# ViennaRNA/RNAcode

Hardware: AMD Instinct MI355X
Metric: alignment-columns x samples scored /sec (higher is better)
Workload: dtype f32; 1 GPU; synthetic MAF 10000 blocks x 120 cols x 6 seqs, n=1000 (BASELINE configs[2]/[3]); exchange=none, fit_exp_mode=fused

## Files before the change

rnacode_amd/csrc/rc_batch.cpp:

```cpp
#include "rc_runtime.h"


extern "C" {

void rc_batch_destroy(rc_batch *b) {
  if (!b) return;
  trace("destroy", b);
  (void)hipSetDevice(b->device);
  const bool ctxAlive = b->ctx && !(b->retiredKeep && b->retiredKeep->ctxGone.load());
  if (b->state == rc_batch::RUNNING) { if (b->evDone.e) (void)hipEventSynchronize(b->evDone); if (ctxAlive) b->ctx->inflight.fetch_sub(1); }
  else if (b->state == rc_batch::READY && b->evPrep.e) (void)hipEventSynchronize(b->evPrep);
  delete b;
  trace("destroyed", b);
}

}


extern "C" void rc_batch_destroy(rc_batch *b);

int batch_prepare(rc_batch *b, const rc_block *blocks, int32_t n_blocks, const rc_params *par, const TableSet *set) {
  rc_ctx *ctx = b->ctx;
  if (par->blosum != 62 && par->blosum != 90) return fail(RC_ERR_ARG, "blosum must be 62 or 90");
  if (par->sampleN < 1) return fail(RC_ERR_ARG, "sampleN must be >= 1");
  if (!set) RC_TRY(table_set(ctx, *par, &set));
  b->tables = set;
  const auto t0 = std::chrono::steady_clock::now();
  b->par = *par; b->n = n_blocks;
  b->state = rc_batch::EMPTY;
  b->meta.assign(n_blocks, BlockMeta());
  b->db.resize(n_blocks);
  b->errs.clear(); b->okBlocks.clear(); b->classes.clear();
  b->maxL = 0; b->maxDraws = 0; b->hssCap = 8;
  b->allExact = !params_in_fast_range(*par);
  const PairTable &pt = set->pt;

  size_t hostSum = 0, devSum = 0;
  for (int i = 0; i < n_blocks; i++) {
    size_t h = 0, d = 0;
    if (blocks[i].n_rows >= 3 && blocks[i].n_rows <= kMaxRows && blocks[i].n_cols >= 3 && blocks[i].n_cols <= RC_MAX_COLS)
      block_footprint(blocks[i].n_rows, blocks[i].n_cols, &h, &d);
    hostSum += h; devSum += d;
  }
  const size_t nn = static_cast<size_t>(std::max(n_blocks, 1));
  const size_t tail = al256(nn * sizeof(DevBlock)) + 2 * al256(nn * sizeof(int)) + al256(nn * sizeof(uint64_t)) + al256((nn + 1) * sizeof(int));
  b->hostCap = al256(hostSum) + tail + 256;
  b->devCap = al256(devSum) + 256;
  HIP_TRY(hipSetDevice(ctx->device));
  HIP_TRY(b->hblob.ensure(b->hostCap));
  BlobArena arena;
  arena.host = b->hblob.as<uint8_t>();
  arena.hostCap = b->hostCap;
  arena.devCap = b->devCap;

  {
    if (!ctx->pool || ctx->pool->size() != ctx->hostThreads) ctx->pool.reset(new Pool(ctx->hostThreads));
    std::mutex errMu;
    ctx->pool->run(n_blocks, [&](int i) {
      std::string err;
      const int st = prepare_block(blocks[i], *par, pt, arena, static_cast<uint32_t>(i), b->db[i], b->meta[i], err);
      if (st != RC_OK && st != RC_ERR_SKIP) {
        std::lock_guard<std::mutex> lk(errMu);
        b->errs[i] = err;
      }
    });
  }

  bool sameL = true;
  const size_t SpadBytes = (static_cast<size_t>(par->sampleN) + kWave - 1) / kWave * kWave * sizeof(uint32_t);
  for (int i = 0; i < n_blocks; i++) {
    BlockMeta &m = b->meta[i];
    if (m.status != RC_OK) continue;
    if (static_cast<double>(b->db[i].nnodes) * m.cols * static_cast<double>(SpadBytes) > static_cast<double>(ctx->totalMem) / 4.0 || SpadBytes >= (1ull << 32)) {
      m.status = RC_ERR_UNSUPPORTED; b->db[i].status = RC_ERR_UNSUPPORTED;
      b->errs[i] = "rows x columns x samples too large for the device: the block's random-number streams (4 bytes x tree nodes x columns x samples) exceed a quarter of its memory; split the block (breakmaf) or lower --num-samples";
      continue;
    }
    b->okBlocks.push_back(i);
    auto &cls = b->classes[block_class(m.N, m.L, b->db[i].omega, ctx->rule)];
    if (!cls.empty() && b->meta[cls.front()].L != m.L) sameL = false;
    cls.push_back(i);
    b->maxL = std::max(b->maxL, m.L);
    b->maxDraws = std::max(b->maxDraws, b->db[i].nnodes * m.cols);
    const size_t smax = static_cast<size_t>(m.L) / 3;
    b->hssCap = std::max(b->hssCap, static_cast<int>(smax) / 3 + 2);
  }
  if (!sameL)
    for (auto &kv : b->classes) std::stable_sort(kv.second.begin(), kv.second.end(), [&](int x, int y) { return b->meta[x].L > b->meta[y].L; });
  for (auto &kv : b->classes)
    if (kv.first > kGenericClass) std::stable_sort(kv.second.begin(), kv.second.end(), [&](int x, int y) { return b->meta[x].NK > b->meta[y].NK; });

  uint8_t *base = arena.host;
  size_t o = al256(arena.hostUsed.load());
  auto take = [&](size_t bytes) { const size_t at = o; o += al256(bytes); return at; };
  b->oDblocks = take(nn * sizeof(DevBlock));
  b->oOk = take(nn * sizeof(int));
  b->oClass = take(nn * sizeof(int));
  b->oPrefix = take((nn + 1) * sizeof(int));
  if (o > b->hostCap) return fail(RC_ERR_ARG, "internal: blob tail does not fit");
  b->hostUsed = o;
  if (n_blocks > 0) std::memcpy(base + b->oDblocks, b->db.data(), sizeof(DevBlock) * n_blocks);
  if (!b->okBlocks.empty()) std::memcpy(base + b->oOk, b->okBlocks.data(), sizeof(int) * b->okBlocks.size());
  {
    int *cl = reinterpret_cast<int *>(base + b->oClass);
    int at = 0;
    std::fill(b->classOff, b->classOff + kClassSlots, 0);
    for (auto &kv : b->classes) {
      b->classOff[kv.first] = at;
      std::memcpy(cl + at, kv.second.data(), sizeof(int) * kv.second.size());
      at += static_cast<int>(kv.second.size());
    }
    int *pf = reinterpret_cast<int *>(base + b->oPrefix);
    int run = 0;
    for (size_t k = 0; k < b->okBlocks.size(); k++) { pf[k] = run; run += 2 * b->meta[b->okBlocks[k]].N; }
    pf[b->okBlocks.size()] = run;
    b->nModels = run;
  }
  b->prepHostMs = std::chrono::duration<double, std::milli>(std::chrono::steady_clock::now() - t0).count();
  return RC_OK;
}

int batch_upload(rc_batch *b) {
  rc_ctx *c = b->ctx;
  HIP_TRY(hipSetDevice(c->device));
  const int n = b->n;
  const size_t nn = static_cast<size_t>(std::max(n, 1));
  HIP_TRY(b->dblob.ensure(b->hostCap + b->devCap));
  if (!b->maximaExternal) { HIP_TRY(b->dmaxima.ensure(nn * b->par.sampleN * sizeof(float))); b->maxPtr = b->dmaxima.as<float>(); }
  HIP_TRY(b->dhss.ensure(nn * 6 * b->hssCap * sizeof(DevHss)));
  HIP_TRY(b->dhssCount.ensure(nn * 6 * sizeof(int)));
  HIP_TRY(b->dhssPacked.ensure(nn * 6 * b->hssCap * sizeof(DevHss)));
  HIP_TRY(b->dhssOffsets.ensure((nn * 6 + 1) * sizeof(int)));
  HIP_TRY(b->dfit.ensure(nn * sizeof(FitOut)));
  HIP_TRY(b->dflags.ensure(nn * sizeof(uint32_t)));
  HIP_TRY(b->dexact.ensure(nn * sizeof(int)));
  HIP_TRY(b->dcounters.ensure(kCntTotal * sizeof(uint32_t)));
  hipStream_t ps = stream_copy(c);
  if (!ps) return fail(RC_ERR_DEVICE, "hipStreamCreate failed");
  HIP_TRY(hipMemcpyAsync(b->dblob.p, b->hblob.p, b->hostUsed, hipMemcpyHostToDevice, ps));
  HIP_TRY(b->evUp.record(ps));
  HIP_TRY(b->evPrep0.record(ps));
  HIP_TRY(hipMemsetAsync(b->dflags.p, 0, nn * sizeof(uint32_t), ps));
  HIP_TRY(hipMemsetAsync(b->dcounters.p, 0, kCntTotal * sizeof(uint32_t), ps));
  if (!b->okBlocks.empty()) {
    const TablePtrs &tp = b->tables->ptrs;
    PrepArgs pa{};
    uint8_t *blob = b->dblob.as<uint8_t>();
    pa.blob = blob;
    pa.dblocks = reinterpret_cast<const DevBlock *>(blob + b->oDblocks);
    pa.blocks = reinterpret_cast<const int *>(blob + b->oOk);
    pa.nBlocks = static_cast<int>(b->okBlocks.size());
    pa.modelPrefix = reinterpret_cast<const int *>(blob + b->oPrefix);
    pa.nModels = b->nModels;
    pa.pep = tp.pep; pa.blosum = tp.blosum; pa.codeInfo = tp.info;
    pa.standardCode = tp.standard; pa.prepOff = tp.prepOff; pa.prepAb = tp.prepAb;
    pa.flags = b->dflags.as<uint32_t>();
    pa.exactList = b->dexact.as<int>();
    pa.exactCount = b->dcounters.as<int>() + kCntExact;
    std::memcpy(pa.classOff, b->classOff, sizeof pa.classOff);
    pa.rule = c->rule;
    launch_prep(pa, ps);
  }
  HIP_TRY(b->evPrep.record(ps));
  HIP_TRY(hipGetLastError());
  b->state = rc_batch::READY;
  b->maximaFetched = false;
  return RC_OK;
}


extern "C" {

int rc_batch_create(rc_ctx *ctx, const rc_block *blocks, int32_t n_blocks, const rc_params *par, rc_batch **out) {
  if (!ctx || (!blocks && n_blocks > 0) || !par || !out || n_blocks < 0) return fail(RC_ERR_ARG, "bad argument");
  *out = nullptr;
  std::unique_ptr<rc_batch, void (*)(rc_batch *)> guard(new rc_batch(), rc_batch_destroy);
  rc_batch *b = guard.get();
  b->adopt(ctx);
  trace("create", b);
  RC_TRY(batch_prepare(b, blocks, n_blocks, par));
  trace("prepared", b);
  RC_TRY(batch_upload(b));
  trace("uploaded", b);
  *out = guard.release();
  return RC_OK;
}


}

bool g_no_stream_cache = false;
extern "C" void rc_set_stream_cache(int enabled) { g_no_stream_cache = !enabled; }


int ensure_mt_stream(rc_ctx *c, rc_batch *b, hipStream_t st, uint32_t seed, int Spad, int D) {
  b->mtLaunched = false;
  if (c->U_valid && c->U_seed == seed && c->U_Spad == Spad && c->U_D >= D) {
    if (c->U_ready.e) HIP_TRY(hipStreamWaitEvent(st, c->U_ready, 0));
    return RC_OK;
  }
  if (c->inflight.load() > 0) HIP_TRY(hipDeviceSynchronize());
  const size_t need = static_cast<size_t>(Spad) * D;
  if (need > c->U_cap) {
    if (c->d_U) (void)hipFree(c->d_U);
    c->d_U = nullptr; c->U_cap = 0;
    HIP_TRY(hipMalloc(&c->d_U, need * sizeof(uint32_t)));
    c->U_cap = need;
  }
  HIP_TRY(b->evMt0.record(st));
  launch_mt_stream(seed, Spad, D, c->d_U, st);
  HIP_TRY(b->evMt1.record(st));
  HIP_TRY(c->U_ready.record(st));
  b->mtLaunched = true;
  c->U_seed = seed; c->U_Spad = Spad; c->U_D = D; c->U_valid = true;
  return RC_OK;
}


int batch_run_async(rc_batch *b, bool streaming) {
  rc_ctx *c = b->ctx;
  if (b->state != rc_batch::READY && b->state != rc_batch::DONE) return fail(RC_ERR_ARG, "batch is not ready to run");
  HIP_TRY(hipSetDevice(c->device));
  std::fill(b->t, b->t + 6, 0.0f);
  std::fill(b->nl, b->nl + 6, 0);
  b->maximaFetched = false;
  b->nullKernel.clear(); b->nullKernelCost = 0.0;
  const int n = b->n, sampleN = b->par.sampleN;
  const int groups = (sampleN + kWave - 1) / kWave, Spad = groups * kWave;
  b->clamped = 0;
  hipStream_t cs = ctx_stream(c, static_cast<int>(c->seq++ % static_cast<unsigned>(c->computeStreams)));
  if (!cs) return fail(RC_ERR_DEVICE, "hipStreamCreate failed");
  const uint8_t *blob = b->dblob.as<uint8_t>();
  bool nativeFirst = c->serialNative != 0, allFat = !b->classes.empty(), wide = false;
  for (auto &kv : b->classes) {
    int maxLc = 0;
    for (int bi : kv.second) maxLc = std::max(maxLc, b->meta[bi].L);
    allFat = allFat && kv.first < kGenericClass && fat_class(b, c, kv.first, maxLc);
    wide = wide || kv.first >= kGenericClass;
  }
  bool fat = allFat && (!streaming || static_cast<long long>(b->okBlocks.size()) * groups >= c->fatStreamMinItems);
  if (fat) nativeFirst = true;
  if (wide) nativeFirst = true;
  const int nativeMode = c->serialNative ? 0 : nativeFirst ? 1 : 0;
  const RunEnv R{b, c, cs, n, sampleN, groups, Spad, n * 6, b->tables->ptrs, blob,
                 reinterpret_cast<const DevBlock *>(blob + b->oDblocks), reinterpret_cast<const int *>(blob + b->oOk),
                 reinterpret_cast<const int *>(blob + b->oClass), streaming, nativeFirst, nativeMode, fat};
  HIP_TRY(hipStreamWaitEvent(cs, b->evPrep, 0));
  HIP_TRY(b->evStart.record(cs));
  if (!b->okBlocks.empty()) {
    RC_TRY(ensure_mt_stream(c, b, cs, b->par.seed_base, Spad, b->maxDraws));
    uint32_t *cnt = b->dcounters.as<uint32_t>();
    HIP_TRY(hipMemsetAsync(cnt + kCntWork, 0, (kCntTotal - kCntWork) * sizeof(uint32_t), cs));
    HIP_TRY(hipMemsetD32Async(reinterpret_cast<hipDeviceptr_t>(b->maxPtr), 0xBF800000u, static_cast<size_t>(n) * sampleN, cs));
    FitArgs fa{};
    fa.dblocks = R.dblocks; fa.blocks = R.okList; fa.maxima = b->maxPtr; fa.hss = b->dhss.as<DevHss>();
    fa.hssCount = b->dhssCount.as<int>(); fa.hssCap = b->hssCap; fa.out = b->dfit.as<FitOut>(); fa.flags = b->dflags.as<uint32_t>();
    fa.sampleN = sampleN; fa.stopEarly = b->par.stopEarly; fa.expMode = c->expMode;
    fa.stopCutoff = static_cast<int>(b->par.cutoff * b->par.sampleN);
    int g1 = groups;
    if (b->par.stopEarly && fa.stopCutoff >= 0 && fa.stopCutoff < sampleN && static_cast<long long>(b->okBlocks.size()) * groups >= c->stopTwoRoundsMinItems)
      g1 = std::min(groups, (fa.stopCutoff + 1 + kWave + kWave - 1) / kWave);
    {
      size_t most = 0;
      int r = 0;
      b->sbufNeed = 0;
      for (int lo = 0, hi = g1; lo < groups; r++) {
        if (r == c->stopRounds - 1) hi = groups;
        size_t sbuf = 0;
        most = std::max(most, null_round_need(R, lo, hi, &sbuf));
        b->sbufNeed = std::max(b->sbufNeed, sbuf);
        lo = hi; hi = std::min(groups, hi * 2);
      }
      HIP_TRY(b->dscratch.ensure(most * sizeof(uint32_t)));
      if (b->sbufNeed) HIP_TRY(b->dsbuf.ensure(b->sbufNeed * sizeof(float)));
      if (c->tailSharing) {
        const size_t bytes = static_cast<size_t>(r) * b->classes.size() * steal_words(c) * sizeof(uint32_t);
        HIP_TRY(b->dsteal.ensure(bytes));
        HIP_TRY(hipMemsetAsync(b->dsteal.p, 0, bytes, cs));
      }
    }
    bool nativeQueued = true;
    if (R.nativeFirst) RC_TRY(launch_native_block(R));
    HIP_TRY(b->evS0.record(cs));
    if (!R.nativeFirst) RC_TRY(launch_native_block(R));
    int round = 0;
    for (int lo = 0, hi = g1; lo < groups; round++) {
      if (round == c->stopRounds - 1) hi = groups;
      if (lo > 0 && !nativeQueued) { RC_TRY(launch_native_block(R)); nativeQueued = true; }
      if (lo > 0) {
        if (!R.nativeFirst && lo == g1) HIP_TRY(hipStreamWaitEvent(cs, b->evN1, 0));
        fa.firstN = std::min(sampleN, lo * kWave);
        launch_stop_mark(fa, static_cast<int>(b->okBlocks.size()), cs);
        HIP_TRY(b->evMid.record(cs));
      }
      RC_TRY(launch_null_groups(R, lo, hi, round, lo > 0 ? kFlagStopped : 0));
      lo = hi;
      hi = std::min(groups, hi * 2);
    }
    HIP_TRY(b->evS1.record(cs));
    if (!nativeQueued) RC_TRY(launch_native_block(R));
    if (!R.nativeFirst) HIP_TRY(hipStreamWaitEvent(cs, b->evN1, 0));
    launch_evd_fit(fa, static_cast<int>(b->okBlocks.size()), c->inflight.load() == 0 && (!streaming || b->okBlocks.size() <= 64), cs); b->nl[4]++;
  }
  HIP_TRY(b->evFit.record(cs));
  {
    const int slots = R.slots;
    const size_t szFit = sizeof(FitOut) * n, szCnt = sizeof(int) * static_cast<size_t>(slots), szOff = sizeof(int) * (static_cast<size_t>(slots) + 1);
    const size_t oFit = 0, oCnt = al256(oFit + szFit), oOff = al256(oCnt + szCnt), oClamp = al256(oOff + szOff), total = oClamp + 16;
    HIP_TRY(b->hstage.ensure(total));
    if (!b->okBlocks.empty()) {
      uint8_t *hs = b->hstage.as<uint8_t>();
      b->packedAhead = std::min(static_cast<size_t>(slots) * b->hssCap, static_cast<size_t>(n) * 16);
      HIP_TRY(b->hpacked.ensure(sizeof(DevHss) * std::max<size_t>(b->packedAhead, 1)));
      void *dStage = nullptr, *dPacked = nullptr;
      static_assert(sizeof(FitOut) % 4 == 0 && sizeof(DevHss) % 4 == 0, "results travel as 32-bit words");
      if (hipHostGetDevicePointer(&dStage, b->hstage.p, 0) == hipSuccess &&
          hipHostGetDevicePointer(&dPacked, b->hpacked.p, 0) == hipSuccess) {
        uint8_t *ds = static_cast<uint8_t *>(dStage);
        ResultsOutArgs ro{};
        auto part = [&](int x, void *dst, const void *src, size_t bytes) {
          ro.dst[x] = static_cast<uint32_t *>(dst); ro.src[x] = static_cast<const uint32_t *>(src); ro.words[x] = bytes / 4;
        };
        part(0, ds + oFit, b->dfit.p, szFit);
        part(1, ds + oCnt, b->dhssCount.p, szCnt);
        part(2, ds + oOff, b->dhssOffsets.p, szOff);
        part(3, ds + oClamp, b->dcounters.as<uint32_t>() + kCntClamp, sizeof(unsigned long long));
        part(4, dPacked, b->dhssPacked.p, sizeof(DevHss) * b->packedAhead);
        launch_results_out(ro, cs);
      } else {
        HIP_TRY(hipMemcpyAsync(hs + oFit, b->dfit.p, szFit, hipMemcpyDeviceToHost, cs));
        HIP_TRY(hipMemcpyAsync(hs + oCnt, b->dhssCount.p, szCnt, hipMemcpyDeviceToHost, cs));
        HIP_TRY(hipMemcpyAsync(hs + oOff, b->dhssOffsets.p, szOff, hipMemcpyDeviceToHost, cs));
        HIP_TRY(hipMemcpyAsync(hs + oClamp, b->dcounters.as<uint32_t>() + kCntClamp, sizeof(unsigned long long), hipMemcpyDeviceToHost, cs));
        HIP_TRY(hipMemcpyAsync(b->hpacked.p, b->dhssPacked.p, sizeof(DevHss) * b->packedAhead, hipMemcpyDeviceToHost, cs));
      }
    }
  }
  HIP_TRY(b->evDone.record(cs));
  HIP_TRY(hipGetLastError());
  b->state = rc_batch::RUNNING;
  c->inflight.fetch_add(1);
  return RC_OK;
}

int batch_wait(rc_batch *b) {
  if (b->state == rc_batch::DONE) return RC_OK;
  if (b->state != rc_batch::RUNNING) return fail(RC_ERR_ARG, "batch is not running");
  rc_ctx *c = b->ctx;
  HIP_TRY(hipSetDevice(c->device));
  hipError_t e = timed_call("wait hipEventSynchronize", 0, [&] { return hipEventSynchronize(b->evDone); });
  if (c->inflight.fetch_sub(1) == 1 || c->retired->held() > c->retiredCapBytes) { if (!c->retired->empty()) c->retired->drain(); }
  b->state = rc_batch::READY;
  if (e != hipSuccess) return fail(RC_ERR_DEVICE, std::string("hipEventSynchronize: ") + hipGetErrorString(e));
  HIP_TRY(hipGetLastError());
  const int n = b->n, slots = n * 6;
  b->fit.assign(n, FitOut{0, 0, -1, 0});
  b->hssCount.assign(static_cast<size_t>(slots), 0);
  b->hssOff.assign(static_cast<size_t>(slots) + 1, 0);
  b->hssRec.clear();
  if (!b->okBlocks.empty()) {
    float ms = 0;
    if (b->mtLaunched) { HIP_TRY(hipEventElapsedTime(&ms, b->evMt0, b->evMt1)); b->t[1] = ms; b->nl[1] = 1; }
    HIP_TRY(hipEventElapsedTime(&ms, b->evN0, b->evN1)); b->t[3] = ms;
    HIP_TRY(hipEventElapsedTime(&ms, b->evS0, b->evS1)); b->t[2] = ms;
    HIP_TRY(hipEventElapsedTime(&ms, b->evS1, b->evFit)); b->t[4] = ms;
    HIP_TRY(hipEventElapsedTime(&ms, b->evStart, b->evFit)); b->t[0] = ms;
    if (b->evPrep0.e && b->evPrep.e) { HIP_TRY(hipEventElapsedTime(&ms, b->evPrep0, b->evPrep)); b->t[5] = ms; b->nl[5] = 2; }
    const size_t szFit = sizeof(FitOut) * n, szCnt = sizeof(int) * static_cast<size_t>(slots), szOff = sizeof(int) * (static_cast<size_t>(slots) + 1);
    const size_t oFit = 0, oCnt = al256(oFit + szFit), oOff = al256(oCnt + szCnt), oClamp = al256(oOff + szOff);
    const uint8_t *hs = b->hstage.as<uint8_t>();
    const FitOut *f = reinterpret_cast<const FitOut *>(hs + oFit);
    for (int bi : b->okBlocks) b->fit[bi] = f[bi];
    std::memcpy(b->hssCount.data(), hs + oCnt, szCnt);
    std::memcpy(b->hssOff.data(), hs + oOff, szOff);
    std::memcpy(&b->clamped, hs + oClamp, sizeof(unsigned long long));
    const size_t nrec = static_cast<size_t>(std::max(b->hssOff[slots], 0));
    if (nrec > b->packedAhead) {
      PinBuf more;
      HIP_TRY(more.ensure(sizeof(DevHss) * nrec));
      RC_STREAM_TRY(aux, stream_aux(c));
      HIP_TRY(hipMemcpyAsync(more.p, b->dhssPacked.p, sizeof(DevHss) * nrec, hipMemcpyDeviceToHost, aux));
      HIP_TRY(hipStreamSynchronize(aux));
      b->hssRec.assign(more.as<DevHss>(), more.as<DevHss>() + nrec);
    } else if (nrec) {
      b->hssRec.assign(b->hpacked.as<DevHss>(), b->hpacked.as<DevHss>() + nrec);
    }
  }
  b->state = rc_batch::DONE;
  return RC_OK;
}

extern "C" {

int rc_batch_run_async(rc_batch *b) {
  if (!b) return fail(RC_ERR_ARG, "null batch");
  if (g_no_stream_cache && b->ctx->inflight.load() == 0) b->ctx->U_valid = false;
  return batch_run_async(b);
}

int rc_batch_wait(rc_batch *b) {
  if (!b) return fail(RC_ERR_ARG, "null batch");
  return batch_wait(b);
}

int rc_batch_run(rc_batch *b) {
  if (!b) return fail(RC_ERR_ARG, "null batch");
  trace("run", b);
  RC_TRY(rc_batch_run_async(b));
  trace("queued", b);
  const int r = batch_wait(b);
  trace("done", b);
  return r;
}

int rc_batch_bind_maxima(rc_batch *b, void *device_ptr) {
  if (!b || !device_ptr) return fail(RC_ERR_ARG, "bad argument");
  if (b->state == rc_batch::RUNNING) return fail(RC_ERR_ARG, "batch is running");
  b->dmaxima.release();
  b->maxPtr = static_cast<float *>(device_ptr);
  b->maximaExternal = true;
  if (b->state == rc_batch::DONE) b->state = rc_batch::READY;
  return RC_OK;
}

}

void trace_device(rc_batch *b) {
  if (!trace_on() || b->okBlocks.empty()) return;
  static Event ref;
  static double refHostUs = 0.0;
  if (!ref.e) {
    hipStream_t aux = stream_aux(b->ctx);
    if (!aux || ref.record(aux) != hipSuccess || hipEventSynchronize(ref) != hipSuccess) return;
    refHostUs = trace_now_us();
    std::fprintf(stderr, "[rc device clock: reference recorded now; a batch finished before it shows negative offsets]\n");
  }
  auto at = [&](const Event &e) { float ms = 0; return (e.e && hipEventElapsedTime(&ms, ref, e) == hipSuccess) ? refHostUs + ms * 1e3 : -1.0; };
  std::fprintf(stderr, "[rc device %p n=%d] now %.1f | prep0 %.1f prep %.1f start %.1f null0 %.1f null1 %.1f native0 %.1f native1 %.1f fit %.1f done %.1f (us on the device-reference clock)\n",
               static_cast<void *>(b), b->n, trace_now_us(), at(b->evPrep0), at(b->evPrep), at(b->evStart), at(b->evS0), at(b->evS1), at(b->evN0), at(b->evN1),
               at(b->evFit), at(b->evDone));
}
```

rnacode_amd/csrc/rc_context.cpp:

```cpp
#include <cstddef>

#include "rc_runtime.h"

extern "C" {

const char *rc_last_error(void) { return g_err.c_str(); }

void rc_default_params(rc_params *p) {
  p->Delta = -10.0f; p->Omega = -4.0f; p->omega = -2.0f;
  p->stopPenalty_0 = -9999.0f; p->stopPenalty_k = -8.0f;
  p->blosum = 62; p->sampleN = 100; p->cutoff = 1.0f; p->stopEarly = 0; p->seed_base = 42;
  std::memset(p->genetic_code, 0, sizeof p->genetic_code);
}

}

void want_hw_queues() { (void)setenv("GPU_MAX_HW_QUEUES", "8", 0); }

int table_set(rc_ctx *c, const rc_params &par, const TableSet **out) {
  char code[64];
  const char *why = nullptr;
  if (!parse_genetic_code(par.genetic_code, code, &why)) return fail(RC_ERR_ARG, why);
  if (par.blosum != 62 && par.blosum != 90) return fail(RC_ERR_ARG, "blosum must be 62 or 90");
  std::lock_guard<std::mutex> lk(c->setMutex);
  for (const auto &t : c->sets)
    if (t->blosum == par.blosum && std::memcmp(t->code, code, 64) == 0) { *out = t.get(); return RC_OK; }
  auto t = std::make_unique<TableSet>(code, par.blosum);
  t->pt.build(t->ct);
  const size_t oPair = 0, oBlosum = al256(4096), oInfo = oBlosum + al256(400 * sizeof(int)), oPep = oInfo + al256(64 * sizeof(CodeInfo)),
               oOff = oPep + al256(64 * sizeof(int)), oAb = oOff + al256(6 * sizeof(int)), total = oAb + al256(4096 * sizeof(uint16_t));
  std::vector<uint8_t> h(total, 0);
  std::memcpy(h.data() + oPair, t->pt.pair, 4096);
  int *bl = reinterpret_cast<int *>(h.data() + oBlosum);
  for (int p = 0; p < 20; p++) for (int q = 0; q < 20; q++) bl[20 * p + q] = t->ct.blosum[p][q];
  std::memcpy(h.data() + oInfo, t->pt.info, 64 * sizeof(CodeInfo));
  int *pep = reinterpret_cast<int *>(h.data() + oPep);
  for (int i = 0; i < 64; i++) pep[i] = t->ct.pep[i];
  int *off = reinterpret_cast<int *>(h.data() + oOff);
  uint16_t *ab = reinterpret_cast<uint16_t *>(h.data() + oAb);
  int n = 0;
  off[0] = 0;
  for (int a = 0; a < 64; a++) for (int b = 0; b < 64; b++) if (pep[a] == -1 || pep[b] == -1) ab[n++] = static_cast<uint16_t>(a << 6 | b);
  for (int hq = 0; hq < 4; hq++) {
    off[1 + hq] = n;
    for (int a = 0; a < 64; a++) for (int b = 0; b < 64; b++) {
      if (pep[a] == -1 || pep[b] == -1) continue;
      const int x = a ^ b;
      if (((x & 48) != 0) + ((x & 12) != 0) + ((x & 3) != 0) == hq) ab[n++] = static_cast<uint16_t>(a << 6 | b);
    }
  }
  off[5] = n;
  t->d.retired = c->retired.get();
  HIP_TRY(hipSetDevice(c->device));
  HIP_TRY(t->d.ensure(total));
  HIP_TRY(hipMemcpy(t->d.p, h.data(), total, hipMemcpyHostToDevice));
  const uint8_t *d = t->d.as<uint8_t>();
  const CodeTables standard(par.blosum);
  t->ptrs = TablePtrs{d + oPair, reinterpret_cast<const int *>(d + oPep), reinterpret_cast<const int *>(d + oBlosum),
                      reinterpret_cast<const CodeInfo *>(d + oInfo), reinterpret_cast<const int *>(d + oOff),
                      reinterpret_cast<const uint16_t *>(d + oAb), std::memcmp(standard.pep, t->ct.pep, sizeof standard.pep) == 0};
  *out = t.get();
  c->sets.push_back(std::move(t));
  return RC_OK;
}

extern "C" {

int rc_device_count(void) {
  want_hw_queues();
  int n = 0;
  if (hipGetDeviceCount(&n) != hipSuccess) return 0;
  return n;
}

int rc_host_cpus(void) { return effective_cpus(); }

void rc_ctx_trim(rc_ctx *c) {
  if (!c) return;
  (void)hipSetDevice(c->device);
  (void)hipDeviceSynchronize();
  c->retired->drain();
  c->bufPool->drain(false);
}

void rc_ctx_destroy(rc_ctx *c) {
  if (!c) return;
  (void)hipSetDevice(c->device);
  (void)hipDeviceSynchronize();
  c->retired->ctxGone.store(true);
  c->retired->drain();
  g_retired.drain();
  c->bufPool->drain(true);
  c->pool.reset();
  if (kProfiling && c->d_cellStats.p) {
    unsigned long long st[6] = {0, 0, 0, 0, 0, 0};
    if (hipMemcpy(st, c->d_cellStats.p, sizeof st, hipMemcpyDeviceToHost) == hipSuccess && st[0])
      std::fprintf(stderr, "[rc cell stats] wavefront-cells %llu, with no positive lane %llu (%.4f %%), positive lane-cells %.2f %%\n", st[0], st[1],
                   100.0 * st[1] / st[0], 100.0 * st[2] / (64.0 * st[0])),
      std::fprintf(stderr, "[rc cell stats] before the row's first event %.1f %%, event codons %.1f %%, after its last event %.1f %%, between events %.1f %%\n",
                   100.0 * st[3] / st[0], 100.0 * st[4] / st[0], 100.0 * st[5] / st[0], 100.0 * (st[0] - st[3] - st[4] - st[5]) / st[0]);
  }
  if (c->d_U) (void)hipFree(c->d_U);
  for (hipStream_t st : c->compute) if (st) (void)hipStreamDestroy(st);
  if (c->native) (void)hipStreamDestroy(c->native);
  if (c->copy) (void)hipStreamDestroy(c->copy);
  if (c->aux) (void)hipStreamDestroy(c->aux);
  if (c->tree) (void)hipStreamDestroy(c->tree);
  if (c->tree2) (void)hipStreamDestroy(c->tree2);
  for (hipStream_t st : c->classStreams) (void)hipStreamDestroy(st);
  delete c;
}

int rc_ctx_create(int device, rc_ctx **out) {
  if (!out) return fail(RC_ERR_ARG, "null out pointer");
  *out = nullptr;
  want_hw_queues();
  int n = 0;
  trace("ctx: start", nullptr);
  if (hipGetDeviceCount(&n) != hipSuccess || n <= 0)
    return fail(RC_ERR_DEVICE, "no HIP device available: the scoring path has no CPU fallback");
  trace("ctx: runtime up", nullptr);
  if (device < 0 || device >= n) return fail(RC_ERR_ARG, "device index out of range");
  HIP_TRY(hipSetDevice(device));
  std::unique_ptr<rc_ctx, void (*)(rc_ctx *)> guard(new rc_ctx(), rc_ctx_destroy);
  rc_ctx *c = guard.get();
  c->device = device;
  hipDeviceProp_t prop;
  HIP_TRY(hipGetDeviceProperties(&prop, device));
  c->numCU = prop.multiProcessorCount;
  c->totalMem = prop.totalGlobalMem;
  c->retiredCapBytes = prop.totalGlobalMem / 16;
  c->bufPool->devCap = prop.totalGlobalMem / 16;
  c->bufPool->device = device;
  static const int hostExp = exp_mode_of_host();
  c->expMode = hostExp;
  if (const char *e = std::getenv("RC_FIT_EXP")) {
    const std::string v(e);
    if (v == "generic" || v == "1") c->expMode = 1;
    else if (v == "fused" || v == "fma" || v == "2") c->expMode = 2;
    else if (v == "device" || v == "0") c->expMode = 0;
    else return fail(RC_ERR_ARG, "RC_FIT_EXP must be generic, fused or device");
  }
  for (DevBuf *d : {&c->treeJobs, &c->treeIn, &c->treeWork, &c->treeRes, &c->d_cellStats}) d->retired = c->retired.get();
  for (PinBuf *h : {&c->treeInPin, &c->treeResPin}) h->retired = c->retired.get();
  c->genericScratchWords = std::max<size_t>(static_cast<size_t>(1) << 30, prop.totalGlobalMem / 12 / sizeof(uint32_t));
  c->togetherWords = std::max<size_t>(static_cast<size_t>(1) << 30, prop.totalGlobalMem / 36 / sizeof(uint32_t));
  if (const char *e = std::getenv("RC_TOGETHER_MAX_MB")) c->togetherWords = static_cast<size_t>(std::max(0ll, std::atoll(e))) * (1u << 20) / sizeof(uint32_t);
  if (const char *e = std::getenv("RC_CLASS_STREAMS")) c->classStreamCount = std::max(1, std::min(16, std::atoi(e)));
  if (const char *e = std::getenv("RC_GRID_CAP_PER_CU")) c->gridCapPerCU = std::max(0, std::atoi(e));
  if (const char *e = std::getenv("RC_SPLIT_FACTOR")) c->splitFactor = std::max(0.0, std::atof(e));
  if (const char *e = std::getenv("RC_NATIVE_WAVES_PER_CU")) c->nativeWavesPerCU = std::max(1, std::min(32, std::atoi(e)));
  if (const char *e = std::getenv("RC_TAIL_SHARING")) c->tailSharing = std::atoi(e) != 0;
  if (const char *e = std::getenv("RC_ROW_SPLIT")) c->rowSplit = std::atoi(e) != 0;
  if (const char *e = std::getenv("RC_DUAL_ROWS")) c->dualRows = std::atoi(e) != 0;
  if (const char *e = std::getenv("RC_HIGH_OCCUPANCY")) c->highOccupancy = std::max(0, std::min(2, std::atoi(e)));
  if (prop.maxSharedMemoryPerMultiProcessor > 0) c->ldsPerCU = prop.maxSharedMemoryPerMultiProcessor;
  if (const char *e = std::getenv("RC_FAT_STREAM_MIN_ITEMS")) c->fatStreamMinItems = std::max(0ll, std::atoll(e));
  if (const char *e = std::getenv("RC_GENERIC_SCRATCH_MB")) c->genericScratchWords = std::max<size_t>(1, static_cast<size_t>(std::atoll(e))) * (1u << 20) / sizeof(uint32_t);
  int prioLow = 0, prioHigh = 0;
  HIP_TRY(hipDeviceGetStreamPriorityRange(&prioLow, &prioHigh));
  c->prioLow = prioLow; c->prioHigh = 0; c->classPrio = prioLow;
  trace("ctx: streams", nullptr);
  c->serialNative = std::getenv("RC_SERIAL_NATIVE") ? 1 : 0;
  c->stopTwoRoundsMinItems = 4LL * c->numCU * 16;
  if (const char *e = std::getenv("RC_STOP_MIN_ITEMS")) c->stopTwoRoundsMinItems = std::atoll(e);
  if (const char *e = std::getenv("RC_GENERIC_MIN_ROWS")) c->rule.genericMinRows = std::max(3, std::min(kTemplRows + 1, std::atoi(e)));
  if (const char *e = std::getenv("RC_TILED_MAX_L")) c->rule.tiledMaxL = std::max(0, std::atoi(e));
  if (const char *e = std::getenv("RC_TILED_MIN_ROWS")) c->rule.tiledMinRows = std::max(kTiledMaxKT + 2, std::min(kTemplRows + 1, std::atoi(e)));
  if (const char *e = std::getenv("RC_TILED_MAX_ROWS")) c->rule.tiledMaxRows = std::max(kTemplRows, std::min(kMaxRows, std::atoi(e)));
  if (const char *e = std::getenv("RC_TILED_WIDE_MAX_L")) c->rule.tiledWideMaxL = std::max(0, std::atoi(e));
  if (const char *e = std::getenv("RC_TILED_ANY_L_MIN_ROWS")) c->rule.tiledAnyLMinRows = std::max(kTemplRows + 1, std::atoi(e));
  if (const char *e = std::getenv("RC_STOP_ROUNDS")) c->stopRounds = std::max(2, std::min(kMaxRounds, std::atoi(e)));
  {
    rc_params std{};
    std.blosum = 62;
    const TableSet *unused = nullptr;
    RC_TRY(table_set(c, std, &unused));
    std.blosum = 90;
    RC_TRY(table_set(c, std, &unused));
  }
  trace("ctx: tables", nullptr);
  c->tieThr = float_threshold_lt(0.0001);
  if (const char *e = std::getenv("RC_LDS_MAX_BYTES")) { c->ldsMaxBytes = c->ldsMaxBytesOneRow = static_cast<size_t>(std::atol(e)); c->stageManyRows = true; }
#ifdef RC_PROFILING
  if (const char *e = std::getenv("RC_DEBUG_SKIP")) c->debugSkip = std::atoi(e);
  if (std::getenv("RC_CELL_STATS")) {
    HIP_TRY(c->d_cellStats.ensure(6 * sizeof(unsigned long long)));
    HIP_TRY(hipMemset(c->d_cellStats.p, 0, 6 * sizeof(unsigned long long)));
  }
#endif
  c->hostThreads = std::min(effective_cpus(), 32);
  if (const char *e = std::getenv("RC_HOST_THREADS")) c->hostThreads = std::max(1, std::atoi(e));
  *out = guard.release();
  return RC_OK;
}

int rc_genetic_code(int32_t ncbi_id, char out[65]) {
  if (!out) return fail(RC_ERR_ARG, "null out pointer");
  const char *aas = ncbi_code(ncbi_id);
  if (!aas) return fail(RC_ERR_ARG, "unknown genetic code id " + std::to_string(ncbi_id) +
                                    " (built in: 1-6, 9-14, 16, 21-26, 29, 30, 33; 27, 28, 31 and 32 are not supported)");
  std::memcpy(out, aas, 64);
  out[64] = '\0';
  return RC_OK;
}

int rc_ctx_set_host_threads(rc_ctx *c, int32_t threads) {
  if (!c || threads < 1) return fail(RC_ERR_ARG, "bad argument");
  if (c->inflight.load() != 0) return fail(RC_ERR_ARG, "batches are in flight");
  c->hostThreads = threads;
  c->pool.reset();
  return RC_OK;
}

int rc_ctx_host_threads(const rc_ctx *c) { return c ? c->hostThreads : 0; }

int rc_ctx_fit_exp_mode(const rc_ctx *c) { return c ? c->expMode : RC_ERR_ARG; }

}

#undef rc_default_params
#undef rc_batch_create
#undef rc_stream_create
static constexpr size_t kParamsV1Bytes = offsetof(rc_params, genetic_code);
static_assert(kParamsV1Bytes == 40, "the members of the older rc_params layout");
static rc_params params_v1(const rc_params *old) {
  rc_params p;
  std::memset(&p, 0, sizeof p);
  std::memcpy(&p, old, kParamsV1Bytes);
  return p;
}

extern "C" {

void rc_default_params(rc_params *p) {
  rc_params q;
  rc_default_params_v2(&q);
  std::memcpy(p, &q, kParamsV1Bytes);
}

int rc_batch_create(rc_ctx *ctx, const rc_block *blocks, int32_t n_blocks, const rc_params *par, rc_batch **out) {
  if (!par) return rc_batch_create_v2(ctx, blocks, n_blocks, par, out);
  const rc_params p = params_v1(par);
  return rc_batch_create_v2(ctx, blocks, n_blocks, &p, out);
}

int rc_stream_create(rc_ctx *ctx, const rc_params *par, int32_t depth, rc_stream **out) {
  if (!par) return rc_stream_create_v2(ctx, par, depth, out);
  const rc_params p = params_v1(par);
  return rc_stream_create_v2(ctx, &p, depth, out);
}

}
```

rnacode_amd/csrc/rc_device.h:

```cpp
#pragma once
#include <cstdint>

namespace rc {

constexpr int kMaxRows = 500;
constexpr int kTemplRows = 64;
constexpr int kFastRows = 32;
constexpr int kGenericDefaultMinRows = 37;
constexpr int kGenericClass = kTemplRows;
constexpr int kTiledMinKT = 12, kTiledMaxKT = 15;
constexpr int kTiledClass0 = kGenericClass + 1;
constexpr int kClassSlots = kTiledClass0 + (kTiledMaxKT - kTiledMinKT + 1);
constexpr int kTiledDefaultMinRows = 32;
constexpr int kTiledDefaultMaxL = 250;
constexpr int tiled_kt(int NK) {
  int best = kTiledMaxKT, bestCost = 1 << 30;
  for (int kt = kTiledMaxKT; kt >= kTiledMinKT; kt--) {
    const int T = (NK + kt - 1) / kt, cost = T * (9 * kt + 20);
    if (cost < bestCost) { bestCost = cost; best = kt; }
  }
  return best;
}
struct ClassRule { int genericMinRows, tiledMinRows, tiledMaxL, tiledMaxRows, tiledWideMaxL, tiledAnyLMinRows; };
constexpr int kTiledDefaultMaxRows = kMaxRows;
constexpr int kTiledDefaultWideMaxL = 200;
constexpr int kTiledDefaultAnyLMinRows = 112;
constexpr ClassRule kDefaultClassRule{kGenericDefaultMinRows, kTiledDefaultMinRows, kTiledDefaultMaxL, kTiledDefaultMaxRows, kTiledDefaultWideMaxL,
                                      kTiledDefaultAnyLMinRows};
constexpr int block_class(int N, int L, float omega, const ClassRule &r) {
  const int maxL = N > kTemplRows ? (N >= r.tiledAnyLMinRows ? (1 << 30) : r.tiledWideMaxL) : N >= kGenericDefaultMinRows ? r.tiledMaxL : r.tiledMaxL * 4 / 5;
  const int maxRows = r.tiledMaxRows > kTemplRows ? r.tiledMaxRows : kTemplRows;
  if (N >= r.tiledMinRows && r.tiledMinRows <= kTemplRows && N <= maxRows && L <= maxL && r.genericMinRows > r.tiledMinRows && omega <= 0.0f) return kTiledClass0 + tiled_kt(N - 1) - kTiledMinKT;
  return N < r.genericMinRows ? N - 1 : kGenericClass;
}
constexpr int kMaxNodes = 2 * kMaxRows;
constexpr int kWave = 64;
constexpr int kLutSize = 64;
constexpr int kFastNodes = 2 * kFastRows;
constexpr int kPhaseALds = kFastNodes * 64 + 64 * 64;

struct alignas(16) U4 { uint32_t x, y, z, w; };

struct alignas(16) NodeRec {
  U4 thr[4];
  uint32_t basepack;
  uint16_t parent;
  int16_t tiprow;
  uint32_t gctrl;
  uint8_t pad[4];
};
constexpr uint32_t node_ctrl(uint32_t q) { return (2u * (q & 7u)) | ((q >> 3) << 7); }
static_assert(sizeof(NodeRec) == 80, "NodeRec layout");

struct alignas(16) ModelRec {
  float P[16];
  float scores[4];
  float probs[4];
  float kappa, dist;
  float freqs[4];
  float pad[2];
};
static_assert(sizeof(ModelRec) == 128, "ModelRec layout");

struct DevBlock {
  int32_t N, NK, cols, L;
  int32_t nnodes, status, ref_start, ref_length;
  float Delta, Omega, omega, nkf;
  float stop0, stopk;
  int32_t code_zero, code_stop0, code_stopk;
  int32_t zw_words;
  int32_t zm_words;
  uint32_t out_index;
  uint64_t off_nodes;
  uint64_t off_qtip;
  uint64_t off_qtip16;
  uint64_t off_chars;
  uint64_t off_models;
  uint64_t off_chars_rev;
  uint64_t off_refcol;
  uint64_t off_zw;
  uint64_t off_mask;
  uint64_t off_zmask;
  uint64_t off_lut;
  uint64_t off_sigma;
  uint64_t off_chain;
};

constexpr int code_words(int NK) { return (NK + 4) / 5; }
constexpr int code_tail_bytes(int NK) { return NK - 5 * (code_words(NK) - 1) == 1 ? 1 : NK - 5 * (code_words(NK) - 1) == 2 ? 2 : 4; }
constexpr int code_pos_words(int NK) { return (code_words(NK) - 1) * kWave + code_tail_bytes(NK) * (kWave / 4); }

constexpr int kDualRowsMaxNK = 5;
constexpr uint32_t kFlagExact = 1u;
constexpr uint32_t kFlagNan = 4u;
constexpr uint32_t kFlagStopped = 2u;

struct CodeInfo { int8_t kind, b, h, pad; };

struct DevHss {
  int32_t strand, frame, startSite, endSite;
  float score;
};

}
```

rnacode_amd/csrc/rc_kernels.hip:

```cpp
#include "rc_null_kernel.h"
#include "rc_null_generic.h"
#include "rc_refexp.h"

namespace rc {

__global__ __launch_bounds__(64) void k_mt_stream(uint32_t seedBase, int Spad, int D, uint32_t *__restrict__ U) {
  __shared__ uint32_t mt[624];
  const int lane = threadIdx.x;
  const int s = blockIdx.x;
  if (lane == 0) {
    uint32_t x = seedBase + static_cast<uint32_t>(s);
    mt[0] = x;
    for (int i = 1; i < 624; i++) {
      x = 1812433253u * (x ^ (x >> 30)) + static_cast<uint32_t>(i);
      mt[i] = x;
    }
  }
  __syncthreads();
  for (int base = 0; base < D; base += 624) {
    for (int c = 0; c < 624; c += 64) {
      const int kk = c + lane;
      uint32_t nv = 0;
      if (kk < 624) {
        const int k1 = (kk + 1 == 624) ? 0 : kk + 1;
        const int km = (kk + 397 >= 624) ? kk + 397 - 624 : kk + 397;
        const uint32_t y = (mt[kk] & 0x80000000u) | (mt[k1] & 0x7fffffffu);
        nv = mt[km] ^ (y >> 1) ^ ((y & 1u) ? 0x9908b0dfu : 0u);
      }
      __syncthreads();
      if (kk < 624) mt[kk] = nv;
      __syncthreads();
    }
    for (int c = 0; c < 624; c += 64) {
      const int kk = c + lane;
      if (kk < 624 && base + kk < D) {
        uint32_t y = mt[kk];
        y ^= (y >> 11);
        y ^= (y << 7) & 0x9d2c5680u;
        y ^= (y << 15) & 0xefc60000u;
        y ^= (y >> 18);
        U[static_cast<size_t>(base + kk) * Spad + s] = y;
      }
    }
    __syncthreads();
  }
}


__device__ constexpr int kPepOf(int c) {
  constexpr char code[] = "KNKNTTTTRSRSIIMIQHQHPPPPRRRRLLLLEDEDAAAAGGGGVVVV*Y*YSSSS*CWCLFLF";
  constexpr char order[] = "ARNDCQEGHILKMFPSTWYV";
  for (int i = 0; i < 20; i++) if (order[i] == code[c]) return i;
  return -1;
}

template <int B, typename F> __device__ __forceinline__ void for_codon_b(F &&f) {
  if constexpr (B < 64) { f(std::integral_constant<int, B>{}); for_codon_b<B + 1>(static_cast<F &&>(f)); }
}

__device__ __forceinline__ ModelRec *prep_model_of(const PrepArgs &A, int t) {
  int hi = A.nBlocks, lo = 0;
  while (hi - lo > 1) {
    const int mid = (lo + hi) >> 1;
    const bool below = A.modelPrefix[mid] <= t;
    hi = below ? hi : mid;
    lo = below ? mid : lo;
  }
  const DevBlock *db = A.dblocks + A.blocks[lo];
  return reinterpret_cast<ModelRec *>(A.blob + db->off_models) + (t - A.modelPrefix[lo]);
}

struct PrepFreq {
  float f0, f1, f2, f3;
  __device__ __forceinline__ float operator()(int x) const { return x == 0 ? f0 : x == 1 ? f1 : x == 2 ? f2 : f3; }
};
__device__ __forceinline__ float prep_term(const float *__restrict__ P, const PrepFreq &freq, int ab) {
  const int a = ab >> 6, b = ab & 63;
  const int a1 = a >> 4, a2 = (a >> 2) & 3, a3 = a & 3;
  const float fa = freq(a1) * freq(a2) * freq(a3);
  float pAB = P[a1 * 4 + (b >> 4)] * P[a2 * 4 + ((b >> 2) & 3)] * P[a3 * 4 + (b & 3)];
  pAB = pAB * fa;
  return pAB;
}
__device__ __forceinline__ void add_in_order(float &acc, float v, int cnt) {
  for (int l = 0; l < cnt; l++) acc = acc + __int_as_float(__builtin_amdgcn_readlane(__float_as_int(v), l));
}

__global__ __launch_bounds__(64) void k_prep_models(PrepArgs A) {
  __builtin_amdgcn_s_setprio(3);
  const int lane = threadIdx.x;
  const int hq = blockIdx.x & 3;
  int t = (blockIdx.x >> 2) * kWave + lane;
  const bool active = t < A.nModels;
  if (!active) t = A.nModels - 1;
  ModelRec *m = prep_model_of(A, t);
  const float *__restrict__ P = m->P;
  const PrepFreq freq{m->freqs[0], m->freqs[1], m->freqs[2], m->freqs[3]};
  const int *__restrict__ blosum = A.blosum;
  float probStop = 0.0f;
  for (int a = 0; a < 64; a++) {
    const int a1 = a >> 4, a2 = (a >> 2) & 3, a3 = a & 3;
    const bool stopA = A.pep[a] == -1;
    const float fa = freq(a1) * freq(a2) * freq(a3);
    float r1[4], r2[4], r3[4];
#pragma unroll
    for (int x = 0; x < 4; x++) { r1[x] = P[a1 * 4 + x]; r2[x] = P[a2 * 4 + x]; r3[x] = P[a3 * 4 + x]; }
    for_codon_b<0>([&](auto bc) {
      constexpr int b = decltype(bc)::value;
      constexpr bool stopB = kPepOf(b) == -1;
      if (stopA || stopB) {
        float pAB = r1[b >> 4] * r2[(b >> 2) & 3] * r3[b & 3];
        pAB = pAB * fa;
        probStop = probStop + pAB;
      }
    });
  }
  float cq = 0.0f, sq = 0.0f;
  const float keep = 1.0f - probStop;
  for (int a = 0; a < 64; a++) {
    const int pa = A.pep[a];
    if (pa == -1) continue;
    const int a1 = a >> 4, a2 = (a >> 2) & 3, a3 = a & 3;
    const float fa = freq(a1) * freq(a2) * freq(a3);
    float r1[4], r2[4], r3[4];
#pragma unroll
    for (int x = 0; x < 4; x++) { r1[x] = P[a1 * 4 + x]; r2[x] = P[a2 * 4 + x]; r3[x] = P[a3 * 4 + x]; }
    for_codon_b<0>([&](auto bc) {
      constexpr int b = decltype(bc)::value;
      constexpr int pb = kPepOf(b);
      if constexpr (pb != -1) {
        const int x = a ^ b;
        const int h = ((x & 48) != 0) + ((x & 12) != 0) + ((x & 3) != 0);
        if (h == hq) {
          float pAB = r1[b >> 4] * r2[(b >> 2) & 3] * r3[b & 3];
          pAB = pAB * fa;
          pAB = pAB / keep;
          const float sc = static_cast<float>(blosum[pa * 20 + pb]);
          cq = cq + pAB;
          sq = sq + sc * pAB;
        }
      }
    });
  }
  if (active) {
    m->scores[hq] = sq / cq;
    m->probs[hq] = cq;
  }
}

struct PrepLists { uint16_t ab[4096]; int off[6]; };
constexpr PrepLists make_prep_lists() {
  PrepLists l{};
  int n = 0;
  l.off[0] = 0;
  for (int a = 0; a < 64; a++) for (int b = 0; b < 64; b++) if (kPepOf(a) == -1 || kPepOf(b) == -1) l.ab[n++] = static_cast<uint16_t>(a << 6 | b);
  for (int h = 0; h < 4; h++) {
    l.off[1 + h] = n;
    for (int a = 0; a < 64; a++) for (int b = 0; b < 64; b++) {
      if (kPepOf(a) == -1 || kPepOf(b) == -1) continue;
      const int x = a ^ b;
      if (((x & 48) != 0) + ((x & 12) != 0) + ((x & 3) != 0) == h) l.ab[n++] = static_cast<uint16_t>(a << 6 | b);
    }
  }
  l.off[5] = n;
  return l;
}
__device__ const PrepLists kPrepLists = make_prep_lists();

__global__ __launch_bounds__(64) void k_prep_models_few(PrepArgs A) {
  __builtin_amdgcn_s_setprio(3);
  const int lane = threadIdx.x;
  const int hq = blockIdx.x & 3, t = blockIdx.x >> 2;
  ModelRec *m = prep_model_of(A, t);
  const float *__restrict__ P = m->P;
  const PrepFreq freq{m->freqs[0], m->freqs[1], m->freqs[2], m->freqs[3]};
  float probStop = 0.0f;
  for (int base = kPrepLists.off[0]; base < kPrepLists.off[1]; base += kWave) {
    const int cnt = kPrepLists.off[1] - base < kWave ? kPrepLists.off[1] - base : kWave;
    const float v = lane < cnt ? prep_term(P, freq, kPrepLists.ab[base + lane]) : 0.0f;
    add_in_order(probStop, v, cnt);
  }
  const float keep = 1.0f - probStop;
  float cq = 0.0f, sq = 0.0f;
  for (int base = kPrepLists.off[1 + hq]; base < kPrepLists.off[2 + hq]; base += kWave) {
    const int cnt = kPrepLists.off[2 + hq] - base < kWave ? kPrepLists.off[2 + hq] - base : kWave;
    float pAB = 0.0f, sp = 0.0f;
    if (lane < cnt) {
      const int ab = kPrepLists.ab[base + lane];
      pAB = prep_term(P, freq, ab);
      pAB = pAB / keep;
      const float sc = static_cast<float>(A.blosum[A.pep[ab >> 6] * 20 + A.pep[ab & 63]]);
      sp = sc * pAB;
    }
    for (int l = 0; l < cnt; l++) {
      cq = cq + __int_as_float(__builtin_amdgcn_readlane(__float_as_int(pAB), l));
      sq = sq + __int_as_float(__builtin_amdgcn_readlane(__float_as_int(sp), l));
    }
  }
  if (lane == 0) {
    m->scores[hq] = sq / cq;
    m->probs[hq] = cq;
  }
}

__global__ __launch_bounds__(64) void k_prep_models_rt(PrepArgs A) {
  __builtin_amdgcn_s_setprio(3);
  const int lane = threadIdx.x;
  const int pepLane = A.pep[lane];
  const int hq = blockIdx.x & 3;
  int t = (blockIdx.x >> 2) * kWave + lane;
  const bool active = t < A.nModels;
  if (!active) t = A.nModels - 1;
  ModelRec *m = prep_model_of(A, t);
  const float *__restrict__ P = m->P;
  const PrepFreq freq{m->freqs[0], m->freqs[1], m->freqs[2], m->freqs[3]};
  const int *__restrict__ blosum = A.blosum;
  float probStop = 0.0f;
  for (int a = 0; a < 64; a++) {
    const int a1 = a >> 4, a2 = (a >> 2) & 3, a3 = a & 3;
    const bool stopA = __builtin_amdgcn_readlane(pepLane, a) == -1;
    const float fa = freq(a1) * freq(a2) * freq(a3);
    float r1[4], r2[4], r3[4];
#pragma unroll
    for (int x = 0; x < 4; x++) { r1[x] = P[a1 * 4 + x]; r2[x] = P[a2 * 4 + x]; r3[x] = P[a3 * 4 + x]; }
    for_codon_b<0>([&](auto bc) {
      constexpr int b = decltype(bc)::value;
      const bool stopB = __builtin_amdgcn_readlane(pepLane, b) == -1;
      if (stopA || stopB) {
        float pAB = r1[b >> 4] * r2[(b >> 2) & 3] * r3[b & 3];
        pAB = pAB * fa;
        probStop = probStop + pAB;
      }
    });
  }
  float cq = 0.0f, sq = 0.0f;
  const float keep = 1.0f - probStop;
  for (int a = 0; a < 64; a++) {
    const int pa = __builtin_amdgcn_readlane(pepLane, a);
    if (pa == -1) continue;
    const int a1 = a >> 4, a2 = (a >> 2) & 3, a3 = a & 3;
    const float fa = freq(a1) * freq(a2) * freq(a3);
    float r1[4], r2[4], r3[4];
#pragma unroll
    for (int x = 0; x < 4; x++) { r1[x] = P[a1 * 4 + x]; r2[x] = P[a2 * 4 + x]; r3[x] = P[a3 * 4 + x]; }
    for_codon_b<0>([&](auto bc) {
      constexpr int b = decltype(bc)::value;
      const int pb = __builtin_amdgcn_readlane(pepLane, b);
      const int x = a ^ b;
      const int h = ((x & 48) != 0) + ((x & 12) != 0) + ((x & 3) != 0);
      if (pb != -1 && h == hq) {
        float pAB = r1[b >> 4] * r2[(b >> 2) & 3] * r3[b & 3];
        pAB = pAB * fa;
        pAB = pAB / keep;
        const float sc = static_cast<float>(blosum[pa * 20 + pb]);
        cq = cq + pAB;
        sq = sq + sc * pAB;
      }
    });
  }
  if (active) {
    m->scores[hq] = sq / cq;
    m->probs[hq] = cq;
  }
}

__global__ __launch_bounds__(64) void k_prep_models_few_rt(PrepArgs A) {
  __builtin_amdgcn_s_setprio(3);
  const int lane = threadIdx.x;
  const int hq = blockIdx.x & 3, t = blockIdx.x >> 2;
  ModelRec *m = prep_model_of(A, t);
  const float *__restrict__ P = m->P;
  const PrepFreq freq{m->freqs[0], m->freqs[1], m->freqs[2], m->freqs[3]};
  const int *__restrict__ off = A.prepOff;
  const uint16_t *__restrict__ abList = A.prepAb;
  const int s0 = off[0], s1 = off[1], c0 = off[1 + hq], c1 = off[2 + hq];
  float probStop = 0.0f;
  for (int base = s0; base < s1; base += kWave) {
    const int cnt = s1 - base < kWave ? s1 - base : kWave;
    const float v = lane < cnt ? prep_term(P, freq, abList[base + lane]) : 0.0f;
    add_in_order(probStop, v, cnt);
  }
  const float keep = 1.0f - probStop;
  float cq = 0.0f, sq = 0.0f;
  for (int base = c0; base < c1; base += kWave) {
    const int cnt = c1 - base < kWave ? c1 - base : kWave;
    float pAB = 0.0f, sp = 0.0f;
    if (lane < cnt) {
      const int ab = abList[base + lane];
      pAB = prep_term(P, freq, ab);
      pAB = pAB / keep;
      const float sc = static_cast<float>(A.blosum[A.pep[ab >> 6] * 20 + A.pep[ab & 63]]);
      sp = sc * pAB;
    }
    for (int l = 0; l < cnt; l++) {
      cq = cq + __int_as_float(__builtin_amdgcn_readlane(__float_as_int(pAB), l));
      sq = sq + __int_as_float(__builtin_amdgcn_readlane(__float_as_int(sp), l));
    }
  }
  if (lane == 0) {
    m->scores[hq] = sq / cq;
    m->probs[hq] = cq;
  }
}

__device__ __forceinline__ bool in_div_range_dev(float v) {
  const float a = fabsf(v);
  return a == 0.0f || (a >= 1.3234889800848443e-23f && a < 1099511627776.0f);
}

__global__ __launch_bounds__(64) void k_prep_lut(PrepArgs A) {
  __builtin_amdgcn_s_setprio(3);
  const int bi = A.blocks[blockIdx.x];
  const DevBlock *db = A.dblocks + bi;
  const int N = db->N, NK = db->NK;
  const ModelRec *models = reinterpret_cast<const ModelRec *>(A.blob + db->off_models);
  float *lut = reinterpret_cast<float *>(A.blob + db->off_lut);
  const int total = 2 * NK * kLutSize;
  bool mine = false, nan = false;
  for (int idx = threadIdx.x; idx < total; idx += kWave) {
    const int code = idx % kLutSize, k = (idx / kLutSize) % NK, s = idx / (kLutSize * NK);
    const CodeInfo ci = A.codeInfo[code];
    float v = 0.0f;
    if (ci.kind == 1) v = static_cast<float>(ci.b) - models[s * N + k + 1].scores[ci.h];
    else if (ci.kind == 3) v = db->stop0;
    else if (ci.kind == 4) v = db->stopk;
    lut[idx] = v;
    mine |= !in_div_range_dev(v);
    nan |= v != v;
  }
  const int cls = block_class(N, db->L, db->omega, A.rule);
  if (cls == kGenericClass && threadIdx.x == 0) {
    float *W = reinterpret_cast<float *>(A.blob + db->off_chain);
    const int nW = db->L / 3 + 40;
    const float omega = db->omega;
    float c = 0.0f;
    for (int i = 0; i < nW; i++) {
      if (i > 3) c = c + omega;
      W[i] = c;
    }
  }
  const bool bad = __ballot(mine) != 0ull, anyNan = __ballot(nan) != 0ull;
  if (threadIdx.x == 0 && bad) {
    A.flags[bi] |= kFlagExact | (anyNan ? kFlagNan : 0u);
    const int at = atomicAdd(A.exactCount + cls, 1);
    A.exactList[A.classOff[cls] + at] = bi;
  }
}


__global__ __launch_bounds__(64) void k_prep_gaps(PrepArgs A) {
  __builtin_amdgcn_s_setprio(3);
  const int bi = A.blocks[blockIdx.x >> 1];
  const int s = blockIdx.x & 1;
  const int lane = threadIdx.x;
  const DevBlock *__restrict__ db = A.dblocks + bi;
  const int N = db->N, NK = db->NK, cols = db->cols, L = db->L, L1 = L + 1;
  const int zww = db->zw_words, ncw = (NK + 4) / 5, zmw = db->zm_words;
  const uint8_t *__restrict__ fwd = A.blob + db->off_chars;
  if (s == 1) {
    uint8_t *rev = A.blob + db->off_chars_rev;
    for (int r = 0; r < N; r++)
      for (int c = lane; c < cols; c += kWave) {
        const uint8_t ch = fwd[static_cast<size_t>(r) * cols + c];
        const uint8_t o = (ch == 'T' || ch == 'U') ? 'A' : ch == 'A' ? 'T' : ch == 'C' ? 'G' : ch == 'G' ? 'C' : ch;
        rev[static_cast<size_t>(r) * cols + (cols - 1 - c)] = o;
      }
  }
  auto is_gap = [&](int r, int c) { return fwd[static_cast<size_t>(r) * cols + (s ? cols - 1 - c : c)] == '-'; };
  uint16_t *refcol = reinterpret_cast<uint16_t *>(A.blob + db->off_refcol) + static_cast<size_t>(s) * L1;
  unsigned long long *zw = reinterpret_cast<unsigned long long *>(A.blob + db->off_zw) + static_cast<size_t>(s) * L1 * zww;
  uint32_t *maskw = reinterpret_cast<uint32_t *>(A.blob + db->off_mask) + static_cast<size_t>(s) * L1 * ncw;
  unsigned long long *zm = reinterpret_cast<unsigned long long *>(A.blob + db->off_zmask) + static_cast<size_t>(s) * 3 * zmw;
  if (lane == 0) refcol[0] = 0;
  int seen = 0;
  for (int c0 = 0; c0 < cols; c0 += kWave) {
    const int c = c0 + lane;
    const bool res = c < cols && !is_gap(0, c);
    const unsigned long long m = __ballot(res);
    const int p = seen + __builtin_popcountll(m & ((1ull << lane) - 1ull)) + 1;
    if (res && p <= L) refcol[p] = static_cast<uint16_t>(c);
    seen += __builtin_popcountll(m);
  }
  if (lane < 3 && lane <= L) {
    for (int w = 0; w < zww; w++) zw[static_cast<size_t>(lane) * zww + w] = 0ull;
    for (int w = 0; w < ncw; w++) maskw[static_cast<size_t>(lane) * ncw + w] = 0u;
  }
  __syncthreads();
  for (int f = 0; f < 3; f++) {
    const int sites = (L - f) / 3;
    for (int j0 = 0; j0 < zmw * kWave; j0 += kWave) {
      const int j = j0 + lane;
      const bool active = j < sites;
      bool any = false;
      if (active) {
        const int i = 3 * j + 3 + f;
        const int c1 = refcol[i - 2], c2 = refcol[i - 1], c3 = refcol[i];
        const int lo = (i > 3) ? refcol[i - 3] + 1 : 0, hi = c3 + 1;
        const int g0 = (hi - lo) - 3;
        unsigned long long zword = 0ull;
        uint32_t mword = 0u;
        for (int k = 0; k < NK; k++) {
          int gk = 0;
          for (int c = lo; c < hi; c++) gk += is_gap(k + 1, c) ? 1 : 0;
          int diff = gk - g0;
          diff = (diff < 0 ? -diff : diff) % 3;
          any |= diff != 0;
          zword |= static_cast<unsigned long long>(diff) << (2 * (k & 31));
          const uint32_t m = (is_gap(k + 1, c1) ? 0u : 0x30u) | (is_gap(k + 1, c2) ? 0u : 0x0Cu) | (is_gap(k + 1, c3) ? 0u : 0x03u);
          mword |= m << (6 * (k % 5));
          if ((k & 31) == 31 || k == NK - 1) { zw[static_cast<size_t>(i) * zww + (k >> 5)] = zword; zword = 0ull; }
          if (k % 5 == 4 || k == NK - 1) { maskw[static_cast<size_t>(i) * ncw + k / 5] = mword; mword = 0u; }
        }
      }
      const unsigned long long bits = __ballot(active && any);
      if (lane == 0) zm[static_cast<size_t>(f) * zmw + (j0 >> 6)] = bits;
    }
  }
}

void launch_prep(const PrepArgs &a, hipStream_t stream) {
  if (a.nBlocks <= 0) return;
  hipLaunchKernelGGL(k_prep_gaps, dim3(2 * a.nBlocks), dim3(kWave), 0, stream, a);
  const bool few = a.nModels <= 2048;
  const dim3 grid(few ? 4 * a.nModels : 4 * ((a.nModels + kWave - 1) / kWave));
  if (a.standardCode) hipLaunchKernelGGL(few ? k_prep_models_few : k_prep_models, grid, dim3(kWave), 0, stream, a);
  else hipLaunchKernelGGL(few ? k_prep_models_few_rt : k_prep_models_rt, grid, dim3(kWave), 0, stream, a);
  hipLaunchKernelGGL(k_prep_lut, dim3(a.nBlocks), dim3(kWave), 0, stream, a);
}

__global__ __launch_bounds__(256) void k_native_sigma(NativeArgs A) {
  __builtin_amdgcn_s_setprio(3);
  const int bi = A.blocks[blockIdx.x];
  const DevBlock *__restrict__ db = A.dblocks + bi;
  const int NK = db->NK, cols = db->cols, L = db->L, L1 = L + 1;
  uint8_t *blob = A.blob;
  const uint16_t *refcol = reinterpret_cast<const uint16_t *>(blob + db->off_refcol);
  const uint8_t *chars = blob + db->off_chars, *charsRev = blob + db->off_chars_rev;
  const float *lut = reinterpret_cast<const float *>(blob + db->off_lut);
  float *sigma = reinterpret_cast<float *>(blob + db->off_sigma);
  const int total = 2 * NK * L1;
  for (int idx = threadIdx.x; idx < total; idx += blockDim.x) {
    const int i = idx % L1, k = (idx / L1) % NK, s = idx / (L1 * NK);
    float sg = 0.0f;
    if (i >= 3) {
      const uint8_t *r0 = (s ? charsRev : chars);
      const uint8_t *rk = (s ? charsRev : chars) + static_cast<size_t>(k + 1) * cols;
      const uint16_t *rc = refcol + s * L1;
      uint32_t a = 0, b = 0;
      bool anyN = false;
#pragma unroll
      for (int t = 2; t >= 0; t--) {
        const int c = rc[i - t];
        const uint8_t ca = r0[c], cb = rk[c];
        anyN |= (ca == 'N') | (cb == 'N');
        const uint32_t xa = (ca == 'C') ? 1u : (ca == 'G') ? 2u : (ca == 'T' || ca == 'U') ? 3u : 0u;
        const uint32_t xb = (cb == 'C') ? 1u : (cb == 'G') ? 2u : (cb == 'T' || cb == 'U') ? 3u : 0u;
        a = (a << 2) | xa;
        b = (b << 2) | xb;
      }
      if (!anyN) sg = lut[(s * NK + k) * kLutSize + A.pair[a * 64 + b]];
    }
    sigma[idx] = sg;
  }
}

}
#define RC_NATIVE_TRACK 0
#include "rc_native_dp.h"
namespace rc {

__global__ __launch_bounds__(64) void k_native_scan(NativeArgs A) {
  const int item = blockIdx.x * kWave + threadIdx.x;
  if (item >= A.nItems) return;
  const int bi = A.blocks[item / 6];
  const int combo = item % 6, s = combo / 3, f = combo % 3;
  const DevBlock *__restrict__ db = A.dblocks + bi;
  const int sites = (db->L - f) / 3;
  const float *__restrict__ S = A.sAll + static_cast<size_t>(item) * A.sAllSites * A.sAllSites;
  DevHss *out = A.hss + (static_cast<size_t>(bi) * 6 + combo) * A.hssCap;
  int n = 0;
  ScanState st{0.0f, -1, -1};
  for (int a = 0; a < sites; a++) {
    const float *__restrict__ row = S + static_cast<size_t>(a) * A.sAllSites;
    for (int j0 = a; j0 < sites; j0 += 8) {
      float v8[8];
#pragma unroll
      for (int t = 0; t < 8; t++) v8[t] = row[j0 + t < sites ? j0 + t : sites - 1];
#pragma unroll
      for (int t = 0; t < 8; t++) {
        const int j = j0 + t;
        const float v = v8[t];
        const bool last = (a == sites - 1) && (j == sites - 1);
        if (j < sites && (v > 0.0f || last))
          scan_step(st, v, a, j, last, A.tieThr, [&](const ScanState &e) {
            if (n < A.hssCap) out[n] = DevHss{s, f, e.ss, e.se, e.cm};
            n++;
          });
      }
    }
  }
  A.hssCount[static_cast<size_t>(bi) * 6 + combo] = n;
}

__global__ __launch_bounds__(64) void k_sk_row(const uint8_t *blob, const DevBlock *dblocks, const uint32_t *flags, int bi, int s, int b, int iMax,
                                               float *out, int stride) {
  const DevBlock *db = dblocks + bi;
  const bool nanSem = flags && (flags[bi] & kFlagNan);
  const int L1 = db->L + 1;
  const unsigned long long *zw = reinterpret_cast<const unsigned long long *>(blob + db->off_zw);
  const float *sigma = reinterpret_cast<const float *>(blob + db->off_sigma);
  for (int k = threadIdx.x; k < db->NK; k += kWave) {
    float s0 = 0.0f, s1 = 0.0f, s2 = 0.0f;
    int t = 0;
    for (int i = b + 2; i <= iMax; i += 3, t++) {
      const int zc = static_cast<int>((zw[static_cast<size_t>(s * L1 + i) * db->zw_words + (k >> 5)] >> (2 * (k & 31))) & 3ull);
      if (nanSem) pair_step<true>(zc, sigma[(static_cast<size_t>(s) * db->NK + k) * L1 + i], db->Delta, db->Omega, db->omega, s0, s1, s2);
      else pair_step(zc, sigma[(static_cast<size_t>(s) * db->NK + k) * L1 + i], db->Delta, db->Omega, db->omega, s0, s1, s2);
      out[(static_cast<size_t>(k) * 3 + 0) * stride + t] = s0;
      out[(static_cast<size_t>(k) * 3 + 1) * stride + t] = s1;
      out[(static_cast<size_t>(k) * 3 + 2) * stride + t] = s2;
    }
  }
}

constexpr unsigned long long kBtMoves = 0x2u | (0x9ull << 4)
                                        | (0x1ull << 8) | (0x5ull << 12)
                                        | (0x5ull << 16) | (0xaull << 20)
                                        | (0x2ull << 24) | (0x5ull << 28)
                                        | (0x6ull << 32) | (0x9ull << 36)
                                        | (0xaull << 40) | (0x1ull << 44);

__device__ __forceinline__ bool bt_near(float x, float y) {
  const float d = (x > y) ? (x - y) : (y - x);
  return static_cast<double>(d) < 0.00001;
}
__device__ __forceinline__ unsigned bt_tests(float s, float first, float second) { return bt_near(s, second) ? 2u : (bt_near(s, first) ? 1u : 0u); }

template <bool SEM>
__device__ __forceinline__ int bt_forward(const unsigned long long *__restrict__ zw, const float *__restrict__ sig, int zww, int k, int i0, int steps,
                                          float Delta, float Omega, float omega, uint8_t *__restrict__ cell) {
  float s0 = 0.0f, s1 = 0.0f, s2 = 0.0f;
  for (int t = 0, i = i0; t < steps; t++, i += 3) {
    const int zc = static_cast<int>((zw[static_cast<size_t>(i) * zww + (k >> 5)] >> (2 * (k & 31))) & 3ull);
    const float p0 = s0, p1 = s1, p2 = s2;
    pair_step<SEM>(zc, sig[i], Delta, Omega, omega, s0, s1, s2);
    unsigned d = static_cast<unsigned>(zc);
    if (zc == 1) {
      d |= bt_tests(s0, p0 + Delta, p2 + Omega) << 2;
      d |= bt_tests(s1, p0 + Omega, p1 + Delta) << 4;
      d |= bt_tests(s2, p1 + Omega, p2 + Delta) << 6;
    } else if (zc != 0) {
      d |= bt_tests(s0, p0 + Delta, p1 + Omega) << 2;
      d |= bt_tests(s1, p1 + Delta, p2 + Omega) << 4;
      d |= bt_tests(s2, p2 + Delta, p0 + Omega) << 6;
    }
    cell[t] = static_cast<uint8_t>(d);
  }
  float opt = -99.0f;
  int curr = -1;
  if (s0 > opt) { opt = s0; curr = 0; }
  if (s1 > opt) { opt = s1; curr = 1; }
  if (s2 > opt) { opt = s2; curr = 2; }
  return curr;
}

__global__ __launch_bounds__(64) void k_backtrack_many(const uint8_t *__restrict__ blob, const DevBlock *__restrict__ dblocks, const uint32_t *__restrict__ flags,
                                                       const BtItem *__restrict__ items, int nItems, uint8_t *__restrict__ cells) {
  const int at = blockIdx.x * kWave + threadIdx.x;
  if (at >= nItems) return;
  const BtItem it = items[at];
  const DevBlock *db = dblocks + it.blk;
  const int L1 = db->L + 1, zww = db->zw_words, k = it.k;
  const unsigned long long *zw = reinterpret_cast<const unsigned long long *>(blob + db->off_zw) + static_cast<size_t>(it.strand) * L1 * zww;
  const float *sig = reinterpret_cast<const float *>(blob + db->off_sigma) + (static_cast<size_t>(it.strand) * db->NK + k) * L1;
  uint8_t *cell = cells + it.off;
  int curr = (flags[it.blk] & kFlagNan) ? bt_forward<true>(zw, sig, zww, k, it.opt_b + 2, it.steps, db->Delta, db->Omega, db->omega, cell)
                                        : bt_forward<false>(zw, sig, zww, k, it.opt_b + 2, it.steps, db->Delta, db->Omega, db->omega, cell);
  int prev = -1;
  unsigned tr = 3u;
  for (int t = it.steps - 1; t >= 0; t--) {
    const unsigned d = cell[t], zc = d & 3u;
    if (zc == 0u) { prev = curr; tr = 0u; }
    else if (curr >= 0) {
      const unsigned test = (d >> (2 + 2 * curr)) & 3u;
      if (test) {
        const unsigned e = static_cast<unsigned>(kBtMoves >> (4 * (((zc == 1u ? 0 : 3) + curr) * 2 + static_cast<int>(test) - 1))) & 15u;
        tr = e & 3u; prev = static_cast<int>(e >> 2);
      }
    }
    const unsigned zenc = zc == 0u ? 1u : (zc == 1u ? 2u : 0u);
    cell[t] = static_cast<uint8_t>(static_cast<unsigned>(curr + 1) | (tr << 2) | (zenc << 4));
    curr = prev;
  }
}

template <int CTRL> __device__ __forceinline__ double dpp_add(double x) {
  const int lo = __builtin_amdgcn_update_dpp(0, __double2loint(x), CTRL, 0xf, 0xf, false);
  const int hi = __builtin_amdgcn_update_dpp(0, __double2hiint(x), CTRL, 0xf, 0xf, false);
  return x + __hiloint2double(hi, lo);
}
__device__ __forceinline__ double row_value(double x, int lane) {
  return __hiloint2double(__builtin_amdgcn_readlane(__double2hiint(x), lane), __builtin_amdgcn_readlane(__double2loint(x), lane));
}
__device__ __forceinline__ double wave_sum(double v) {
  v = dpp_add<0xB1>(v);
  v = dpp_add<0x4E>(v);
  v = dpp_add<0x141>(v);
  v = dpp_add<0x140>(v);
  return (row_value(v, 0) + row_value(v, 16)) + (row_value(v, 32) + row_value(v, 48));
}

template <int THREADS>
__device__ __forceinline__ void fit_sum4(double &a, double &b, double &c, double &d, double *sh) {
  a = wave_sum(a); b = wave_sum(b); c = wave_sum(c); d = wave_sum(d);
  if constexpr (THREADS > kWave) {
    constexpr int NW = THREADS / kWave;
    __syncthreads();
    if ((threadIdx.x & 63) == 0) { double *w = sh + (threadIdx.x >> 6) * 4; w[0] = a; w[1] = b; w[2] = c; w[3] = d; }
    __syncthreads();
    a = b = c = d = 0.0;
#pragma unroll
    for (int w = 0; w < NW; w++) { a += sh[w * 4 + 0]; b += sh[w * 4 + 1]; c += sh[w * 4 + 2]; d += sh[w * 4 + 3]; }
  }
}

__device__ __forceinline__ double fit_exp(int mode, double a) { return mode == 2 ? ref_exp(a, true) : mode == 1 ? ref_exp(a, false) : exp(a); }

template <typename T>
__device__ void lawless416_serial(int mode, const T *x, int n, double lambda, double *f, double *df) {
  const int lane = threadIdx.x & (kWave - 1);
  double e = 0, xe = 0, xxe = 0, xs = 0;
  for (int base = 0; base < n; base += kWave) {
    const int i = base + lane;
    const double xi = i < n ? static_cast<double>(x[i]) : 0.0;
    const double ex = i < n ? fit_exp(mode, -1. * lambda * xi) : 0.0;
    const double t1 = xi * ex, t2 = xi * xi * ex;
    const int cnt = n - base < kWave ? n - base : kWave;
    if (cnt == kWave) {
#pragma unroll
      for (int l = 0; l < kWave; l++) { xs += row_value(xi, l); xe += row_value(t1, l); xxe += row_value(t2, l); e += row_value(ex, l); }
    } else {
      for (int l = 0; l < cnt; l++) { xs += row_value(xi, l); xe += row_value(t1, l); xxe += row_value(t2, l); e += row_value(ex, l); }
    }
  }
  const double total = static_cast<double>(n);
  *f = 1. / lambda - xs / total + xe / e;
  *df = ((xe / e) * (xe / e)) - (xxe / e) - (1. / (lambda * lambda));
}
template <typename T>
__device__ double esum_serial(int mode, const T *x, int n, double lambda) {
  const int lane = threadIdx.x & (kWave - 1);
  double e = 0;
  for (int base = 0; base < n; base += kWave) {
    const int i = base + lane;
    const double ex = i < n ? fit_exp(mode, -1 * lambda * static_cast<double>(x[i])) : 0.0;
    const int cnt = n - base < kWave ? n - base : kWave;
    for (int l = 0; l < cnt; l++) e += row_value(ex, l);
  }
  return e;
}

template <int THREADS, typename T>
__device__ void lawless416(int mode, const T *x, int n, double lambda, double *sh, double *f, double *df) {
  double e = 0, xe = 0, xxe = 0, xs = 0;
  for (int i = threadIdx.x; i < n; i += THREADS) {
    const double xi = static_cast<double>(x[i]);
    const double ex = fit_exp(mode, -1. * lambda * xi);
    xs += xi; xe += xi * ex; xxe += xi * xi * ex; e += ex;
  }
  fit_sum4<THREADS>(e, xe, xxe, xs, sh);
  const double total = static_cast<double>(n);
  *f = 1. / lambda - xs / total + xe / e;
  *df = ((xe / e) * (xe / e)) - (xxe / e) - (1. / (lambda * lambda));
}

constexpr int kFitSerialMaxN = 128;
constexpr int kFitSerialFromStep = 12;

template <int THREADS, typename T>
__device__ int evd_fit_block(int mode, const T *x, int n, double *sh, double *mu_out, double *lambda_out) {
  double lambda = 0.2, fx, dfx;
  const double tol = 1e-5;
  const bool small = n <= kFitSerialMaxN;
  auto eval = [&](double lam, bool careful) {
    if (careful) { lawless416_serial<T>(mode, x, n, lam, &fx, &dfx); return; }
    lawless416<THREADS, T>(mode, x, n, lam, sh, &fx, &dfx);
    if (fabs(fabs(fx) - tol) < 1e-8) lawless416_serial<T>(mode, x, n, lam, &fx, &dfx);
  };
  int it = 0;
  for (int replay = small ? 1 : 0; replay < 2; replay++) {
    const int steps = replay ? 100 : kFitSerialFromStep;
    lambda = 0.2;
    for (it = 0; it < steps; it++) {
      eval(lambda, replay != 0);
      if (fabs(fx) < tol) break;
      lambda = lambda - fx / dfx;
      if (lambda <= 0.) lambda = 0.001;
    }
    if (it < steps) break;
  }
  if (it == 100) {
    double left = 0.2, right = 0.2, mid = 0.2;
    lambda = 0.2;
    eval(lambda, true);
    if (fx < 0.) {
      do {
        left -= 0.1;
        if (left < 0.) return 0;
        eval(left, true);
      } while (fx < 0.);
    } else {
      do {
        right += 0.1;
        eval(right, true);
        if (right > 100.) return 0;
      } while (fx > 0.);
    }
    for (it = 0; it < 100; it++) {
      mid = (left + right) / 2.;
      eval(mid, true);
      if (fabs(fx) < tol) break;
      if (fx > 0.) left = mid; else right = mid;
    }
    if (it == 100) return 0;
    lambda = mid;
  }
  double e = 0, z0 = 0, z1 = 0, z2 = 0;
  if (small) e = esum_serial<T>(mode, x, n, lambda);
  else {
    for (int i = threadIdx.x; i < n; i += THREADS) e += fit_exp(mode, -1 * lambda * static_cast<double>(x[i]));
    fit_sum4<THREADS>(e, z0, z1, z2, sh);
  }
  *mu_out = -1. * log(e / static_cast<double>(n)) / lambda;
  *lambda_out = lambda;
  return 1;
}

__device__ __forceinline__ float best_native(const FitArgs &A, int bi) {
  float m = -1.0f;
  for (int c = 0; c < 6; c++) {
    const int n = min(A.hssCount[static_cast<size_t>(bi) * 6 + c], A.hssCap);
    const DevHss *h = A.hss + (static_cast<size_t>(bi) * 6 + c) * A.hssCap;
    for (int i = 0; i < n; i++) if (h[i].score > 0.0f) m = fmaxf(m, h[i].score);
  }
  return m;
}

__global__ __launch_bounds__(64) void k_stop_mark(FitArgs A) {
  __builtin_amdgcn_s_setprio(3);
  const int bi = A.blocks[blockIdx.x];
  const DevBlock *db = A.dblocks + bi;
  const float *x = A.maxima + static_cast<size_t>(db->out_index) * A.sampleN;
  const float maxNative = best_native(A, bi);
  int better = 0;
  for (int i = threadIdx.x; i < A.firstN; i += kWave) better += (x[i] > maxNative) ? 1 : 0;
  for (int off = 32; off > 0; off >>= 1) better += __shfl_down(better, off, 64);
  if (threadIdx.x == 0) A.flags[bi] = (A.flags[bi] & ~kFlagStopped) | (better > A.stopCutoff ? kFlagStopped : 0u);
}

template <int THREADS>
__global__ __launch_bounds__(THREADS) void k_evd_fit(FitArgs A) {
  __builtin_amdgcn_s_setprio(3);
  __shared__ double sh[THREADS > kWave ? (THREADS / kWave) * 4 : 1];
  const int bi = A.blocks[blockIdx.x];
  const DevBlock *db = A.dblocks + bi;
  const float *x = A.maxima + static_cast<size_t>(db->out_index) * A.sampleN;
  const float maxNative = best_native(A, bi);
  double better = 0, scored = 0, z1 = 0, z2 = 0;
  for (int i = threadIdx.x; i < A.sampleN; i += THREADS) {
    better += (x[i] > maxNative) ? 1.0 : 0.0;
    scored += (x[i] != -1.0f) ? 1.0 : 0.0;
  }
  fit_sum4<THREADS>(better, scored, z1, z2, sh);
  FitOut o;
  o.better = static_cast<int>(better);
  o.rc = -1; o.mu = 0; o.lambda = 0;
  const bool stopped = A.stopEarly && (o.better > A.stopCutoff);
  const bool nothingScored = scored == 0.0;
  if (!stopped && !nothingScored) {
    double mu, lambda;
    if (evd_fit_block<THREADS, float>(A.expMode, x, A.sampleN, sh, &mu, &lambda) == 1) { o.rc = 1; o.mu = mu; o.lambda = lambda; }
  }
  if (threadIdx.x == 0) A.out[db->out_index] = o;
}

__global__ __launch_bounds__(256) void k_evd_fit_f64(const double *x, int n, FitOut *out, int mode) {
  __shared__ double sh[(256 / kWave) * 4];
  double mu = 0, lambda = 0;
  const int rc = evd_fit_block<256, double>(mode, x, n, sh, &mu, &lambda);
  if (threadIdx.x == 0) { out->rc = rc; out->mu = rc ? mu : 0; out->lambda = lambda; out->better = 0; }
}

__global__ __launch_bounds__(64) void k_null_rowscan(NullArgs A, const DevBlock *__restrict__ dblocks, const int *__restrict__ classBlocks,
                                                      const uint32_t *__restrict__ flags, float *__restrict__ maxima) {
  const int lane = threadIdx.x;
  const int groupsHere = A.gHi - A.gLo;
  const int part = blockIdx.x % 6, item = blockIdx.x / 6;
  const int cb = item / groupsHere, grp = A.gLo + item % groupsHere;
  if (cb >= A.nClassBlocks) return;
  const int bi = classBlocks[cb];
  if (A.skipMask && (flags[bi] & A.skipMask)) return;
  const DevBlock *__restrict__ db = dblocks + bi;
  const int f = part % 3, sites = (db->L - f) / 3;
  if (sites <= 0) return;
  const float *__restrict__ src = A.sbuf + (static_cast<size_t>(item) * 6 + part) * A.sbufStride + lane;
  const float negTie = -A.tieThr;
  SampleScan st{0.0f, 0.0f, 0u, 0u};
  float best = -1.0f;
  constexpr int kAhead = 64;
  const int total = sites * (sites + 1) / 2;
  int a = 0, slotsLeft = sites;
  sample_scan_row_begin(st, best, 0u);
  for (int base = 0; base < total; base += kAhead) {
    float v[kAhead];
#pragma unroll
    for (int u = 0; u < kAhead; u++) v[u] = (base + u < total) ? src[static_cast<size_t>(base + u) * kWave] : 0.0f;
#pragma unroll
    for (int u = 0; u < kAhead; u++) {
      if (base + u < total) {
        if (a < sites - 1) sample_scan_step(st, v[u], negTie);
        if (--slotsLeft == 0) {
          sample_scan_row_end(st, static_cast<uint32_t>(a), static_cast<uint32_t>(a < sites - 1 ? sites : sites - 1));
          a++;
          if (a < sites) { sample_scan_row_begin(st, best, static_cast<uint32_t>(a)); slotsLeft = sites - a; }
        }
      }
    }
  }
  sample_scan_last(st, best);
  const int sidx = grp * kWave + lane;
  if (sidx < A.sampleN && best > -1.0f)
    atomicMax(reinterpret_cast<int *>(maxima + static_cast<size_t>(db->out_index) * A.sampleN + sidx), __float_as_int(best));
}

void launch_mt_stream(uint32_t seedBase, int Spad, int D, uint32_t *U, hipStream_t stream) {
  hipLaunchKernelGGL(k_mt_stream, dim3(Spad), dim3(64), 0, stream, seedBase, Spad, D, U);
}

#define RC_NULL_UNIT(S) int null_occupancy_##S(int, NullKind, size_t); bool launch_null_##S(int, NullKind, const NullArgs &, int, size_t, hipStream_t);
RC_NULL_UNIT(a) RC_NULL_UNIT(b) RC_NULL_UNIT(c) RC_NULL_UNIT(d) RC_NULL_UNIT(e) RC_NULL_UNIT(f) RC_NULL_UNIT(g) RC_NULL_UNIT(h)
#undef RC_NULL_UNIT
struct NullUnit { int maxNK; int (*occupancy)(int, NullKind, size_t); bool (*launch)(int, NullKind, const NullArgs &, int, size_t, hipStream_t); };
static const NullUnit *null_unit(int NK) {
  static const NullUnit units[] = {{6, null_occupancy_a, launch_null_a}, {12, null_occupancy_b, launch_null_b}, {21, null_occupancy_c, launch_null_c},
                                   {31, null_occupancy_d, launch_null_d}, {39, null_occupancy_e, launch_null_e}, {47, null_occupancy_f, launch_null_f},
                                   {55, null_occupancy_g, launch_null_g}, {kTemplRows - 1, null_occupancy_h, launch_null_h}};
  if (NK < 2) return nullptr;
  for (const NullUnit &u : units) if (NK <= u.maxNK) return &u;
  return nullptr;
}

int null_occupancy(int NK, NullKind kind, size_t ldsBytes) { const NullUnit *u = null_unit(NK); return u ? u->occupancy(NK, kind, ldsBytes) : 0; }
bool launch_null(int NK, NullKind kind, const NullArgs &a, int grid, size_t ldsBytes, hipStream_t stream) {
  const NullUnit *u = null_unit(NK);
  return u && u->launch(NK, kind, a, grid, ldsBytes, stream);
}

#define RC_FOR_NK(X) \
  X(2) X(3) X(4) X(5) X(6) X(7) X(8) X(9) X(10) X(11) X(12) X(13) X(14) X(15) X(16) X(17) X(18) X(19) X(20) X(21) \
  X(22) X(23) X(24) X(25) X(26) X(27) X(28) X(29) X(30) X(31) X(32) X(33) X(34) X(35) X(36) X(37) X(38) X(39) X(40) X(41) \
  X(42) X(43) X(44) X(45) X(46) X(47) X(48) X(49) X(50) X(51) X(52) X(53) X(54) X(55) X(56) X(57) X(58) X(59) X(60) X(61) X(62) X(63)

void launch_null_rowscan(const NullArgs &a, int items, hipStream_t stream) {
  if (items <= 0) return;
  hipLaunchKernelGGL(k_null_rowscan, dim3(items * 6), dim3(64), 0, stream, a, a.dblocks, a.classBlocks, a.flags, a.maxima);
}

void launch_native_sigma(const NativeArgs &a, int nblocks, hipStream_t stream) {
  hipLaunchKernelGGL(k_native_sigma, dim3(nblocks), dim3(256), 0, stream, a);
}

bool launch_native_dp(int NK, const NativeArgs &a, int grid, hipStream_t stream) {
  switch (NK) {
#define X(n) case n: hipLaunchKernelGGL(k_native_dp<n>, dim3(grid), dim3(64), 0, stream, a); return true;
    RC_FOR_NK(X)
#undef X
    default: return false;
  }
}

void launch_native_scan(const NativeArgs &a, hipStream_t stream) {
  hipLaunchKernelGGL(k_native_scan, dim3((a.nItems + kWave - 1) / kWave), dim3(64), 0, stream, a);
}

__global__ __launch_bounds__(256) void k_hss_pack(const DevHss *__restrict__ hss, const int *__restrict__ count, int cap, int slots,
                                                  DevHss *__restrict__ packed, int *__restrict__ offsets, int *__restrict__ total) {
  const int t = blockIdx.x * blockDim.x + threadIdx.x;
  if (t >= slots) return;
  const int c = min(count[t], cap);
  const int off = c > 0 ? atomicAdd(total, c) : 0;
  offsets[t] = off;
  for (int i = 0; i < c; i++) packed[off + i] = hss[static_cast<size_t>(t) * cap + i];
}

void launch_hss_pack(const DevHss *hss, const int *count, int cap, int slots, DevHss *packed, int *offsets, int *total,
                     hipStream_t stream) {
  if (slots <= 0) return;
  hipLaunchKernelGGL(k_hss_pack, dim3((slots + 255) / 256), dim3(256), 0, stream, hss, count, cap, slots, packed, offsets, total);
}


__global__ __launch_bounds__(64) void k_results_out(ResultsOutArgs a) {
  __builtin_amdgcn_s_setprio(3);
  const size_t t = static_cast<size_t>(blockIdx.x) * blockDim.x + threadIdx.x, step = static_cast<size_t>(gridDim.x) * blockDim.x;
#pragma unroll
  for (int x = 0; x < ResultsOutArgs::kParts; x++)
    for (size_t i = t; i < a.words[x]; i += step) a.dst[x][i] = a.src[x][i];
}

void launch_results_out(const ResultsOutArgs &a, hipStream_t stream) {
  size_t most = 0;
  for (int x = 0; x < ResultsOutArgs::kParts; x++) most = std::max(most, a.words[x]);
  if (!most) return;
  const int grid = static_cast<int>(std::min<size_t>(256, (most + 255) / 256));
  hipLaunchKernelGGL(k_results_out, dim3(grid), dim3(64), 0, stream, a);
}

void launch_sk_row(const uint8_t *blob, const DevBlock *dblocks, const uint32_t *flags, int bi, int s, int b, int iMax, float *out, int stride,
                   hipStream_t stream) {
  hipLaunchKernelGGL(k_sk_row, dim3(1), dim3(64), 0, stream, blob, dblocks, flags, bi, s, b, iMax, out, stride);
}

void launch_backtrack_many(const uint8_t *blob, const DevBlock *dblocks, const uint32_t *flags, const BtItem *items, int nItems, uint8_t *cells,
                           hipStream_t stream) {
  if (nItems <= 0) return;
  hipLaunchKernelGGL(k_backtrack_many, dim3((nItems + kWave - 1) / kWave), dim3(kWave), 0, stream, blob, dblocks, flags, items, nItems, cells);
}

size_t null_generic_lds_bytes(int N, int nnodes) { return generic_lds_bytes(N, nnodes); }

size_t null_generic_codes_bytes(int N, int L, int nnodes) { return generic_codes_bytes(N, L, nnodes); }
size_t null_generic_state_bytes(int N, int L, int nnodes) { return generic_state_bytes(N, L, nnodes); }
int generic_occupancy(NullKind kind, size_t ldsBytes) {
  int nb = 0;
  hipError_t e = hipErrorInvalidValue;
  switch (kind) {
    case NullKind::GenericSim: e = hipOccupancyMaxActiveBlocksPerMultiprocessor(&nb, k_generic_sim<false>, 64, ldsBytes); break;
    case NullKind::TiledSim: e = hipOccupancyMaxActiveBlocksPerMultiprocessor(&nb, k_generic_sim<true>, 64, ldsBytes); break;
    case NullKind::GenericDp: e = hipOccupancyMaxActiveBlocksPerMultiprocessor(&nb, k_generic_dp, 64, ldsBytes); break;
    default: break;
  }
  return e == hipSuccess ? nb : 0;
}
void launch_generic(NullKind kind, const NullArgs &a, int grid, size_t ldsBytes, uint8_t *scratchBytes, hipStream_t stream) {
  if (kind == NullKind::GenericDp)
    hipLaunchKernelGGL(k_generic_dp, dim3(grid), dim3(64), ldsBytes, stream, a, a.blob, a.dblocks, a.classBlocks, a.flags, a.U, a.pair, scratchBytes, a.maxima);
  else if (kind == NullKind::TiledSim)
    hipLaunchKernelGGL(k_generic_sim<true>, dim3(grid), dim3(64), ldsBytes, stream, a, a.blob, a.dblocks, a.classBlocks, a.flags, a.U, a.pair, scratchBytes, a.maxima);
  else
    hipLaunchKernelGGL(k_generic_sim<false>, dim3(grid), dim3(64), ldsBytes, stream, a, a.blob, a.dblocks, a.classBlocks, a.flags, a.U, a.pair, scratchBytes, a.maxima);
}
void launch_native_dp_generic(const NativeArgs &a, int nblocks, float *scratch, size_t scratchStride, hipStream_t stream) {
  hipLaunchKernelGGL(k_native_dp_generic, dim3(nblocks * 6), dim3(64), 0, stream, a, scratch, scratchStride);
}

void launch_stop_mark(const FitArgs &a, int nblocks, hipStream_t stream) {
  hipLaunchKernelGGL(k_stop_mark, dim3(nblocks), dim3(64), 0, stream, a);
}

void launch_evd_fit(const FitArgs &a, int nblocks, bool latency, hipStream_t stream) {
  if (latency && nblocks <= 2048) hipLaunchKernelGGL(k_evd_fit<256>, dim3(nblocks), dim3(256), 0, stream, a);
  else hipLaunchKernelGGL(k_evd_fit<64>, dim3(nblocks), dim3(64), 0, stream, a);
}

void launch_evd_fit_f64(const double *x, int n, FitOut *out, int expMode, hipStream_t stream) {
  hipLaunchKernelGGL(k_evd_fit_f64, dim3(1), dim3(256), 0, stream, x, n, out, expMode);
}

}
```

rnacode_amd/csrc/rc_launch.h:

```cpp
#pragma once
#include <hip/hip_runtime.h>

#include <cstddef>
#include <cstdint>
#include <string>

#include "rc_device.h"

namespace rc {

#ifdef RC_PROFILING
constexpr bool kProfiling = true;
#else
constexpr bool kProfiling = false;
#endif

struct NullArgs {
  const uint8_t *blob;
  const DevBlock *dblocks;
  const int *classBlocks;
  int nClassBlocks;
  const int *nBlocksPtr;
  const uint32_t *flags;
  uint32_t skipMask;
  uint32_t onlyMask;
  int tiledKT;
  int gLo, gHi;
  int sampleN;
  int Spad;
  const uint32_t *U;
  const uint8_t *pair;
  uint32_t *scratch;
  size_t scratchStride;
  float *maxima;
  unsigned long long *clampCount;
  float tieThr;
  int comboSplit;
  unsigned int *workCounter;
  unsigned int *steal;
  uint8_t *codesAll;
  size_t codesStride;
  int cacheSites;
  int reserved[3];
  int stealWait;
  int simParts, simGrid;
  unsigned int *simCounter;
  int rowParts;
  float *sbuf;
  size_t sbufStride;
  int debugSkip;
  unsigned long long *cellStats;
};

struct NativeArgs {
  uint8_t *blob;
  const DevBlock *dblocks;
  const int *blocks;
  const uint8_t *pair;
  float *tile;
  size_t tileStride;
  int nItems;
  float *fullS;
  float *sAll;
  int sAllSites;
  DevHss *hss;
  int *hssCount;
  int hssCap;
  float tieThr;
  const uint32_t *flags;
};

struct PrepArgs {
  uint8_t *blob;
  const DevBlock *dblocks;
  const int *blocks;
  int nBlocks;
  const int *modelPrefix;
  int nModels;
  const int *pep;
  bool standardCode;
  const int *prepOff;
  const uint16_t *prepAb;
  const int *blosum;
  const CodeInfo *codeInfo;
  uint32_t *flags;
  int *exactList;
  int *exactCount;
  int classOff[kClassSlots];
  ClassRule rule;
};

struct FitOut {
  double mu, lambda;
  int rc;
  int better;
};

struct FitArgs {
  const DevBlock *dblocks;
  const int *blocks;
  const float *maxima;
  const DevHss *hss;
  const int *hssCount;
  int hssCap;
  FitOut *out;
  uint32_t *flags;
  int sampleN;
  int firstN;
  int stopEarly;
  int stopCutoff;
  int expMode;
};

struct TreeJob {
  int N, P;
  uint64_t off_mask;
  uint64_t off_w;
  uint64_t off_work;
  uint64_t off_out;
  int mode;
  int pad_;
  uint64_t off_topo;
};
__host__ __device__ inline size_t tree_topo_len_at(int N) { const size_t nn = 2 * static_cast<size_t>(N) - 2; return (sizeof(int) * (1 + 6 * nn) + 7) & ~static_cast<size_t>(7); }
__host__ __device__ inline size_t tree_topo_bytes(int N) { return tree_topo_len_at(N) + sizeof(double) * (2 * static_cast<size_t>(N) - 2); }
#ifdef RC_TREE_PROFILE
constexpr int kTreeProfDoubles = 12;
#else
constexpr int kTreeProfDoubles = 0;
#endif
__host__ __device__ inline size_t tree_result_doubles(int N) { const size_t nn = 2 * static_cast<size_t>(N) - 2; return 2 + nn + (1 + 4 * nn + 1) / 2 + kTreeProfDoubles; }
struct TreeLdsLayout { uint32_t len, coef, e3, D, V, tmpD, len0, opt, ints, w, cols, mask, total; };
constexpr uint32_t kTreeOptDoubles = 32 + kTreeProfDoubles;
__host__ __device__ inline size_t tree_col_doubles(int N, int P) { return (static_cast<size_t>(2) * (N > 3 ? N - 3 : 0) * 4 + 4) * static_cast<size_t>(P); }
__host__ __device__ inline TreeLdsLayout tree_lds_layout(int N, int P, bool big, bool given = false) {
  const uint32_t n = static_cast<uint32_t>(N), nn = 2 * n - 2, p = static_cast<uint32_t>(P);
  TreeLdsLayout l{};
  uint32_t at = 0;
  l.len = at; at += nn;
  l.coef = at; at += 5 * nn;
  l.e3 = at; at += 3 * nn;
  l.D = l.V = l.tmpD = l.len0 = at;
  if (given) {
    l.len0 = at; at += nn;
  } else {
    l.D = at; at += n * n;
    l.V = at; at += n * n;
    l.tmpD = at; at += n;
  }
  l.opt = at; at += kTreeOptDoubles;
  l.ints = at; at += given ? (6 * nn + 1) / 2 : (7 * nn + 2 * n + 1) / 2;
  l.w = l.cols = l.mask = at;
  if (!big) {
    l.w = at; at += p;
    l.cols = at; at += static_cast<uint32_t>(tree_col_doubles(N, P));
    l.mask = at; at += (n * p + 7) / 8;
  }
  l.total = at;
  return l;
}
inline size_t tree_fit_lds_bytes(int N, int P, bool big, bool given = false) {
  const size_t n = static_cast<size_t>(N), nn = 2 * n - 2, p = static_cast<size_t>(P);
  size_t at = given ? 10 * nn + kTreeOptDoubles + (6 * nn + 1) / 2 : 9 * nn + 2 * n * n + n + kTreeOptDoubles + (7 * nn + 2 * n + 1) / 2;
  if (!big) at += p + tree_col_doubles(N, P) + (n * p + 7) / 8;
  return at * sizeof(double);
}
inline size_t tree_work_doubles(int N, int P) { return tree_col_doubles(N, P); }
int tree_fit_max_lds();
int tree_fit_register_occupancy();
bool launch_tree_fit(const TreeJob *jobs, int njobs, bool big, size_t ldsBytes, const uint8_t *in, double *scratch, double *results, hipStream_t stream);

void launch_mt_stream(uint32_t seedBase, int Spad, int D, uint32_t *U, hipStream_t stream);
void launch_prep(const PrepArgs &a, hipStream_t stream);
enum class NullKind {
  Exact,
  Staged,
  StagedTwoRow,
  L2,
  L2Occ,
  L2TwoRow,
  RowSplit,
  GenericSim,
  TiledSim,
  GenericDp,
  TiledDp,
  TiledDpNan,
};
inline std::string null_kernel_name(NullKind kind, int n) {
  const std::string k = std::to_string(n);
  switch (kind) {
    case NullKind::Exact: return "rc::k_null<" + k + ", false, true, false, 0>";
    case NullKind::Staged: return "rc::k_null<" + k + ", true, false, false, 0>";
    case NullKind::StagedTwoRow: return "rc::k_null<" + k + ", true, false, true, 0>";
    case NullKind::L2: return "rc::k_null<" + k + ", false, false, false, 0>";
    case NullKind::L2Occ: return "rc::k_null_occ<" + k + ">";
    case NullKind::L2TwoRow: return "rc::k_null<" + k + ", false, false, true, 0>";
    case NullKind::RowSplit: return "rc::k_null<" + k + ", false, false, false, 1>";
    case NullKind::GenericSim: return "rc::k_generic_sim<false>";
    case NullKind::TiledSim: return "rc::k_generic_sim<true>";
    case NullKind::GenericDp: return "rc::k_generic_dp";
    case NullKind::TiledDp: return "rc::k_tiled_dp<" + k + ", false>";
    case NullKind::TiledDpNan: return "rc::k_tiled_dp<" + k + ", true>";
  }
  return "";
}
int null_occupancy(int NK, NullKind kind, size_t ldsBytes);
bool launch_null(int NK, NullKind kind, const NullArgs &a, int grid, size_t ldsBytes, hipStream_t stream);
void launch_null_rowscan(const NullArgs &a, int items, hipStream_t stream);
void launch_native_sigma(const NativeArgs &a, int nblocks, hipStream_t stream);
bool launch_native_dp(int NK, const NativeArgs &a, int grid, hipStream_t stream);
void launch_native_scan(const NativeArgs &a, hipStream_t stream);
void launch_hss_pack(const DevHss *hss, const int *count, int cap, int slots, DevHss *packed, int *offsets, int *total,
                     hipStream_t stream);
struct ResultsOutArgs {
  static constexpr int kParts = 5;
  uint32_t *dst[kParts];
  const uint32_t *src[kParts];
  size_t words[kParts];
};
void launch_results_out(const ResultsOutArgs &a, hipStream_t stream);
void launch_sk_row(const uint8_t *blob, const DevBlock *dblocks, const uint32_t *flags, int bi, int s, int b, int iMax, float *out, int stride,
                   hipStream_t stream);
struct BtItem {
  int32_t blk, strand, opt_b, steps, k, pad;
  int64_t off;
};
void launch_backtrack_many(const uint8_t *blob, const DevBlock *dblocks, const uint32_t *flags, const BtItem *items, int nItems, uint8_t *cells,
                           hipStream_t stream);
struct SegRange { int32_t blk, strand, opt_b, opt_i; };
struct SegArgs {
  const uint8_t *blob;
  const DevBlock *dblocks;
  const uint32_t *flags;
  const SegRange *ranges;
  const int *prefix;
  int nRanges, nItems;
  float *pairs;
  float *scores;
};
void launch_segment_scores(const SegArgs &a, hipStream_t stream);
struct SegNullArgs {
  const uint8_t *blob;
  const DevBlock *dblocks;
  const uint32_t *flags;
  const int *blocks;
  const int *blkStart;
  const int *rangeIdx;
  const SegRange *ranges;
  const float *scores;
  int *ge;
  float *nullOut;
  const uint8_t *codesAll;
  size_t codesStride;
  int nBlocks, groups, sampleN;
};
constexpr int seg_null_code_words(int L) { return ((L / 3 + 31) >> 2) + 1; }
void launch_segment_null(const SegNullArgs &a, hipStream_t stream);
struct SegPairArgs {
  const int *prefix;
  const float *pairs;
  int *pairGe;
  float *pairNull;
};
void launch_segment_null_pairs(const SegNullArgs &a, const SegPairArgs &pa, hipStream_t stream);
struct DecoyArgs {
  const uint8_t *blob;
  const DevBlock *dblocks;
  const uint32_t *flags;
  const int *blocks;
  const uint8_t *codesAll;
  size_t codesStride;
  uint8_t *sigmaAll;
  size_t sigmaStride;
  DevBlock *vblocks;
  uint32_t *vflags;
  int nDecoys;
};
void launch_decoy_sigma(const DecoyArgs &a, int nBlocks, int maxNK, hipStream_t stream);
struct ShuffleArgs {
  const uint8_t *blob;
  const DevBlock *dblocks;
  const uint32_t *flags;
  const int *blocks;
  const uint8_t *pair;
  const uint16_t *cls16;
  const long long *clsAt;
  uint8_t *permAll;
  size_t permStride;
  uint8_t *sigmaAll;
  size_t sigmaStride;
  DevBlock *vblocks;
  uint32_t *vflags;
  int nDecoys;
  uint32_t seed;
  int ldsCols;
};
constexpr int kShuffleLdsCols = 4096, kShuffleLdsColsMax = 8192;
void launch_shuffle_sigma(const ShuffleArgs &a, int nBlocks, size_t ldsBytes, int sortThreads, hipStream_t stream);
void launch_shuffle_perm(const ShuffleArgs &a, int nBlocks, size_t ldsBytes, int sortThreads, hipStream_t stream);
struct ShuffleNullArgs {
  const uint8_t *blob;
  const DevBlock *dblocks;
  const int *blocks;
  const uint8_t *pair;
  const uint8_t *permAll;
  size_t permStride;
  uint8_t *codesAll;
  size_t codesStride;
  int nBlocks, groups, nShuffles;
};
void launch_shuffle_codes(const ShuffleNullArgs &a, int seqParts, hipStream_t stream);
struct SegShuffleArgs {
  const uint8_t *blob;
  const DevBlock *dblocks;
  const uint32_t *flags;
  const int *blocks;
  const int *blkStart;
  const int *rangeIdx;
  const SegRange *ranges;
  const float *scores;
  const uint8_t *pair;
  int *ge;
  float *nullOut;
  const uint8_t *permAll;
  size_t permStride;
  int nBlocks, groups, nShuffles;
};
void launch_segment_shuffle(const SegShuffleArgs &a, hipStream_t stream);
void launch_segment_shuffle_pairs(const SegShuffleArgs &a, const SegPairArgs &pa, hipStream_t stream);
struct ShuffleNullHeadArgs {
  const uint8_t *blob;
  const DevBlock *dblocks;
  const uint32_t *flags;
  const int *blocks;
  const long long *chainAt;
  float *chainAll;
  DevBlock *vblocks;
  uint32_t *vflags;
  int nBlocks;
};
void launch_shuffle_null_heads(const ShuffleNullHeadArgs &a, hipStream_t stream);
void launch_shuffle_null_ge(const FitArgs &a, int nblocks, int *ge, hipStream_t stream);
size_t null_generic_lds_bytes(int N, int nnodes);
size_t null_generic_codes_bytes(int N, int L, int nnodes);
size_t null_generic_state_bytes(int N, int L, int nnodes);
int generic_occupancy(NullKind kind, size_t ldsBytes);
void launch_generic(NullKind kind, const NullArgs &a, int grid, size_t ldsBytes, uint8_t *scratchBytes, hipStream_t stream);
size_t null_tiled_codes_bytes(int NK, int KT, int L);
size_t null_tiled_state_bytes(int L);
int tiled_dp_occupancy(int KT, NullKind kind, size_t ldsBytes);
bool launch_tiled_dp(int KT, NullKind kind, const NullArgs &a, int grid, size_t ldsBytes, uint8_t *scratchBytes, hipStream_t stream);
void launch_native_dp_generic(const NativeArgs &a, int nblocks, float *scratch, size_t scratchStride, hipStream_t stream);
bool launch_native_track(int NK, const NativeArgs &a, int grid, float *track, const long long *trackOff, hipStream_t stream);
void launch_native_track_generic(const NativeArgs &a, int nblocks, float *scratch, size_t scratchStride, float *track, const long long *trackOff,
                                 hipStream_t stream);
void launch_stop_mark(const FitArgs &a, int nblocks, hipStream_t stream);
void launch_evd_fit(const FitArgs &a, int nblocks, bool latency, hipStream_t stream);
void launch_evd_fit_f64(const double *x, int n, FitOut *out, int expMode, hipStream_t stream);

}
```

rnacode_amd/csrc/rc_native_dp.h:

```cpp
#pragma once
#include "rc_null_kernel.h"

#ifndef RC_NATIVE_TRACK
#error "define RC_NATIVE_TRACK to 0 (the scoring kernels) or 1 (the track kernels) before including rc_native_dp.h"
#endif

namespace rc {

#if RC_NATIVE_TRACK
__device__ __forceinline__ void native_track_rows(float *__restrict__ tile, int a0, int rows, int sites, float *__restrict__ T, int lane) {
  if (lane < rows) {
    float *__restrict__ row = tile + static_cast<size_t>(lane) * sites;
    float run = row[sites - 1];
#pragma unroll 4
    for (int j = sites - 2; j >= a0 + lane; j--) {
      run = fmaxf(run, row[j]);
      row[j] = run;
    }
  }
  __syncthreads();
  for (int c0 = a0; c0 < sites; c0 += kWave) {
    const int c = c0 + lane;
    if (c < sites) {
      const int rmax = c - a0 + 1 < rows ? c - a0 + 1 : rows;
      float m = tile[c];
      for (int r = 1; r < rmax; r++) m = fmaxf(m, tile[static_cast<size_t>(r) * sites + c]);
      T[c] = a0 == 0 ? m : fmaxf(T[c], m);
    }
  }
}

__device__ __forceinline__ float *native_track_of(float *track, const long long *trackOff, int position, int L, int s, int f) {
  const int n0 = L / 3, n1 = (L - 1) / 3, n2 = (L - 2) / 3;
  return track + trackOff[position] + static_cast<size_t>(s) * (n0 + n1 + n2) + (f > 0 ? n0 : 0) + (f > 1 ? n1 : 0);
}
#endif

template <int NK>
#if RC_NATIVE_TRACK
__global__ __launch_bounds__(64) void k_native_track(NativeArgs A, float *__restrict__ track, const long long *__restrict__ trackOff) {
#else
__global__ __launch_bounds__(64) void k_native_dp(NativeArgs A) {
#endif
  __builtin_amdgcn_s_setprio(3);
  const int lane = threadIdx.x;
  float *__restrict__ tile = A.tile + static_cast<size_t>(blockIdx.x) * A.tileStride;
  for (int item = blockIdx.x; item < A.nItems; item += gridDim.x) {
    const int bi = A.blocks[item / 6];
    const int combo = item % 6, s = combo / 3, f = combo % 3;
    const DevBlock *__restrict__ db = A.dblocks + bi;
    const int L = db->L, L1 = L + 1;
    const float Delta = db->Delta, Omega = db->Omega, omega = db->omega, nkf = db->nkf;
    const unsigned long long *zw = reinterpret_cast<const unsigned long long *>(A.blob + db->off_zw);
    const float *sigma = reinterpret_cast<const float *>(A.blob + db->off_sigma);
    const int sites = (L - f) / 3, smax = L / 3;
    float *full = A.fullS ? A.fullS + static_cast<size_t>(combo) * smax * smax : nullptr;
    constexpr bool kOld = NK > 16 && NK <= 32;
    float *__restrict__ all = (!kOld && A.sAll) ? A.sAll + static_cast<size_t>(item) * A.sAllSites * A.sAllSites : nullptr;
#if RC_NATIVE_TRACK
    float *__restrict__ T = native_track_of(track, trackOff, item / 6, L, s, f);
#else
    DevHss *out = A.fullS ? nullptr : A.hss + (static_cast<size_t>(bi) * 6 + combo) * A.hssCap;
    int n = 0;
    ScanState st{0.0f, -1, -1};
#endif
    const bool nanSem = A.flags && (A.flags[bi] & kFlagNan);
    for (int a0 = 0; a0 < sites; a0 += kWave) {
      const int a = a0 + lane;
      float s0[NK], s1[NK], s2[NK];
#pragma unroll
      for (int k = 0; k < NK; k++) s0[k] = s1[k] = s2[k] = 0.0f;
      if constexpr (NK <= 16 || NK > 32) {
      constexpr int ZP = (NK + 15) / 16;
      for (int jc = a0; jc < sites; jc += kWave) {
        const int jl = jc + lane < sites ? jc + lane : sites - 1, il = 3 * jl + 3 + f;
        float sgl[NK];
        uint32_t zl[ZP];
#pragma unroll
        for (int k = 0; k < NK; k++) sgl[k] = sigma[(s * NK + k) * L1 + il];
#pragma unroll
        for (int x = 0; x < ZP; x++) zl[x] = reinterpret_cast<const uint32_t *>(zw)[(static_cast<size_t>(s * L1 + il) * ((NK + 31) / 32)) * 2 + x];
        const int jhi = jc + kWave < sites ? jc + kWave : sites;
        for (int j = jc; j < jhi; j++) {
          const int t = j - jc;
          float sg[NK];
          uint32_t z[ZP];
#pragma unroll
          for (int k = 0; k < NK; k++) sg[k] = __int_as_float(__builtin_amdgcn_readlane(__float_as_int(sgl[k]), t));
#pragma unroll
          for (int x = 0; x < ZP; x++) z[x] = static_cast<uint32_t>(__builtin_amdgcn_readlane(static_cast<int>(zl[x]), t));
          if (a <= j && a < sites) {
            float sum = 0.0f;
            uint32_t zany = 0u;
#pragma unroll
            for (int x = 0; x < ZP; x++) zany |= z[x];
            if (__builtin_expect(nanSem, 0)) {
#pragma unroll
              for (int k = 0; k < NK; k++) {
                pair_step<true>(static_cast<int>((z[k >> 4] >> (2 * (k & 15))) & 3u), sg[k], Delta, Omega, omega, s0[k], s1[k], s2[k]);
                sum = sum + ref_max3<true>(s0[k], s1[k], s2[k]);
              }
            } else if (zany == 0u) {
#pragma unroll
              for (int k = 0; k < NK; k++) {
                s0[k] = s0[k] + sg[k];
                s1[k] = s1[k] + omega;
                s2[k] = s2[k] + omega;
                sum = sum + fmaxf(fmaxf(s0[k], s1[k]), s2[k]);
              }
            } else {
#pragma unroll
              for (int k = 0; k < NK; k++) {
                const uint32_t zc = (z[k >> 4] >> (2 * (k & 15))) & 3u;
                const bool zero = zc == 0u, one = zc == 1u;
                const float d0 = s0[k] + Delta, d1 = s1[k] + Delta, d2 = s2[k] + Delta;
                const float o0 = s0[k] + Omega, o1 = s1[k] + Omega, o2 = s2[k] + Omega;
                const float n0 = fmaxf(d0, one ? o2 : o1), n1 = fmaxf(d1, one ? o0 : o2), n2 = fmaxf(d2, one ? o1 : o0);
                const float p0 = s0[k] + sg[k], p1 = s1[k] + omega, p2 = s2[k] + omega;
                s0[k] = zero ? p0 : n0;
                s1[k] = zero ? p1 : n1;
                s2[k] = zero ? p2 : n2;
                sum = sum + fmaxf(fmaxf(s0[k], s1[k]), s2[k]);
              }
            }
            const float v = fmaxf(sum, Delta) / nkf;
            if (all) all[static_cast<size_t>(a) * A.sAllSites + j] = v;
            else tile[static_cast<size_t>(lane) * sites + j] = v;
            if (full) full[static_cast<size_t>(a) * sites + j] = v;
          }
        }
      }
      } else {
      for (int j = a0; j < sites; j++) {
        const int i = 3 * j + 3 + f;
        constexpr int ZW = (NK + 31) / 32;
        unsigned long long z[ZW];
#pragma unroll
        for (int x = 0; x < ZW; x++) z[x] = zw[static_cast<size_t>(s * L1 + i) * ZW + x];
        if (a <= j && a < sites) {
          float sum = 0.0f;
#pragma unroll
          for (int k = 0; k < NK; k++) {
            const float sig = sigma[(s * NK + k) * L1 + i];
            if (__builtin_expect(nanSem, 0)) {
              pair_step<true>(static_cast<int>((z[k >> 5] >> (2 * (k & 31))) & 3ull), sig, Delta, Omega, omega, s0[k], s1[k], s2[k]);
              sum = sum + ref_max3<true>(s0[k], s1[k], s2[k]);
            } else {
              pair_step(static_cast<int>((z[k >> 5] >> (2 * (k & 31))) & 3ull), sig, Delta, Omega, omega, s0[k], s1[k], s2[k]);
              sum = sum + fmaxf(fmaxf(s0[k], s1[k]), s2[k]);
            }
          }
          const float v = fmaxf(sum, Delta) / nkf;
          tile[static_cast<size_t>(lane) * sites + j] = v;
          if (full) full[static_cast<size_t>(a) * sites + j] = v;
        }
      }
      }
      if constexpr (!kOld) { if (all) continue; }
      __syncthreads();
#if RC_NATIVE_TRACK
      native_track_rows(tile, a0, (a0 + kWave < sites) ? kWave : sites - a0, sites, T, lane);
#else
      native_scan_rows(tile, a0, (a0 + kWave < sites) ? a0 + kWave : sites, sites, s, f, A.tieThr, st, n, out, A.hssCap, lane);
#endif
      __syncthreads();
    }
#if !RC_NATIVE_TRACK
    if (out && lane == 0 && (kOld || !all)) A.hssCount[static_cast<size_t>(bi) * 6 + combo] = n;
#endif
  }
}

#if RC_NATIVE_TRACK
__global__ __launch_bounds__(64) void k_native_track_generic(NativeArgs A, float *__restrict__ scratch, size_t scratchStride, float *__restrict__ track,
                                                             const long long *__restrict__ trackOff) {
#else
__global__ __launch_bounds__(64) void k_native_dp_generic(NativeArgs A, float *__restrict__ scratch, size_t scratchStride) {
#endif
  const int lane = threadIdx.x;
  const int bi = A.blocks[blockIdx.x / 6];
  const int combo = blockIdx.x % 6, s = combo / 3, f = combo % 3;
  const DevBlock *__restrict__ db = A.dblocks + bi;
  const int L = db->L, L1 = L + 1, NK = db->NK, ZW = db->zw_words;
  const float Delta = db->Delta, Omega = db->Omega, omega = db->omega, nkf = db->nkf;
  const unsigned long long *zw = reinterpret_cast<const unsigned long long *>(A.blob + db->off_zw);
  const float *sigma = reinterpret_cast<const float *>(A.blob + db->off_sigma);
  const int sites = (L - f) / 3, smax = L / 3;
  float *dp = scratch + static_cast<size_t>(blockIdx.x) * scratchStride;
  float *tile = dp + static_cast<size_t>(3) * NK * kWave;
  float *full = A.fullS ? A.fullS + static_cast<size_t>(combo) * smax * smax : nullptr;
#if RC_NATIVE_TRACK
  float *__restrict__ T = native_track_of(track, trackOff, blockIdx.x / 6, L, s, f);
#else
  DevHss *out = A.fullS ? nullptr : A.hss + (static_cast<size_t>(bi) * 6 + combo) * A.hssCap;
  int n = 0;
  ScanState st{0.0f, -1, -1};
#endif
  const bool nanSem = A.flags && (A.flags[bi] & kFlagNan);
  for (int a0 = 0; a0 < sites; a0 += kWave) {
    const int a = a0 + lane;
    for (int k = 0; k < 3 * NK; k++) dp[static_cast<size_t>(k) * kWave + lane] = 0.0f;
    for (int j = a0; j < sites; j++) {
      const int i = 3 * j + 3 + f;
      const unsigned long long *z = zw + static_cast<size_t>(s * L1 + i) * ZW;
      if (a <= j && a < sites) {
        float sum = 0.0f;
        for (int k = 0; k < NK; k++) {
          float s0 = dp[(0 * static_cast<size_t>(NK) + k) * kWave + lane], s1 = dp[(1 * static_cast<size_t>(NK) + k) * kWave + lane],
                s2 = dp[(2 * static_cast<size_t>(NK) + k) * kWave + lane];
          if (nanSem) pair_step<true>(static_cast<int>((z[k >> 5] >> (2 * (k & 31))) & 3ull), sigma[(static_cast<size_t>(s) * NK + k) * L1 + i], Delta, Omega, omega, s0, s1, s2);
          else pair_step(static_cast<int>((z[k >> 5] >> (2 * (k & 31))) & 3ull), sigma[(static_cast<size_t>(s) * NK + k) * L1 + i], Delta, Omega, omega, s0, s1, s2);
          dp[(0 * static_cast<size_t>(NK) + k) * kWave + lane] = s0;
          dp[(1 * static_cast<size_t>(NK) + k) * kWave + lane] = s1;
          dp[(2 * static_cast<size_t>(NK) + k) * kWave + lane] = s2;
          sum = sum + (nanSem ? ref_max3<true>(s0, s1, s2) : fmaxf(fmaxf(s0, s1), s2));
        }
        const float v = fmaxf(sum, Delta) / nkf;
        tile[static_cast<size_t>(lane) * sites + j] = v;
        if (full) full[static_cast<size_t>(a) * sites + j] = v;
      }
    }
    __syncthreads();
#if RC_NATIVE_TRACK
    native_track_rows(tile, a0, (a0 + kWave < sites) ? kWave : sites - a0, sites, T, lane);
#else
    native_scan_rows(tile, a0, (a0 + kWave < sites) ? a0 + kWave : sites, sites, s, f, A.tieThr, st, n, out, A.hssCap, lane);
#endif
    __syncthreads();
  }
#if !RC_NATIVE_TRACK
  if (out && lane == 0) A.hssCount[static_cast<size_t>(bi) * 6 + combo] = n;
#endif
}

}
```

rnacode_amd/csrc/rc_native_plan.h:

```cpp
#pragma once
#include <algorithm>
#include <cstddef>
#include <vector>

#include "rc_device.h"

namespace rc {

constexpr bool native_wide(int N, int L, float omega, const ClassRule &rule) {
  return N > kTemplRows || block_class(N, L, omega, rule) == kGenericClass;
}

constexpr int kNativeWideStates = 3;
constexpr size_t native_wide_stride(int maxNK, int smax) {
  return static_cast<size_t>(kNativeWideStates) * maxNK * kWave + static_cast<size_t>(kWave) * smax;
}

constexpr size_t kNativeWideChunk = 256;
constexpr size_t native_wide_chunk(size_t count, size_t at) { return std::min(kNativeWideChunk, count - at); }

constexpr size_t kNativeKeepMinItems = 6 * 64, kNativeKeepMemShare = 16;
constexpr size_t native_all_floats(size_t count, int smax) { return 6 * count * smax * smax; }
constexpr bool native_keep_all(int NK, size_t count, int smax, size_t totalMem) {
  return native_all_floats(count, smax) * sizeof(float) <= totalMem / kNativeKeepMemShare && 6 * count >= kNativeKeepMinItems && (NK <= 16 || NK > 32);
}

struct NativeMember { int NK, L; bool wide; int key; };

struct NativeGroup {
  int NK;
  size_t at, count;
  int smax, maxNK;
  size_t grid;
  bool keepAll;
};

struct NativePlan {
  std::vector<NativeGroup> groups;
  size_t tileFloats = 0, scratchFloats = 0, allFloats = 0;
};

template <typename MemberOf, typename GridOf>
NativePlan native_plan(size_t n, MemberOf memberOf, GridOf gridOf, size_t totalMem) {
  NativePlan pl;
  for (size_t at = 0; at < n;) {
    const NativeMember first = memberOf(at);
    NativeGroup g{first.wide ? 0 : first.NK, at, 0, 1, 0, 0, false};
    for (; at < n; at++, g.count++) {
      const NativeMember m = memberOf(at);
      if (m.wide != first.wide || m.key != first.key || (!m.wide && m.NK != first.NK)) break;
      g.smax = std::max(g.smax, m.L / 3); g.maxNK = std::max(g.maxNK, m.NK);
    }
    if (g.NK) {
      g.grid = gridOf(g.count * 6, g.smax);
      g.keepAll = native_keep_all(g.NK, g.count, g.smax, totalMem);
      pl.tileFloats = std::max(pl.tileFloats, g.grid * kWave * g.smax);
      if (g.keepAll) pl.allFloats = std::max(pl.allFloats, native_all_floats(g.count, g.smax));
    } else {
      pl.scratchFloats = std::max(pl.scratchFloats, native_wide_stride(g.maxNK, g.smax) * 6 * native_wide_chunk(g.count, 0));
    }
    pl.groups.push_back(g);
  }
  return pl;
}

}
```

rnacode_amd/csrc/rc_runtime.h:

```cpp
#pragma once
#include <hip/hip_runtime.h>
#include <sched.h>

#include <algorithm>
#include <atomic>
#include <chrono>
#include <cmath>
#include <condition_variable>
#include <cstdio>
#include <cstdlib>
#include <cstring>
#include <deque>
#include <functional>
#include <initializer_list>
#include <map>
#include <memory>
#include <mutex>
#include <string>
#include <thread>
#include <tuple>
#include <vector>

#include "../../include/rnacode_hip.h"
#include "rc_host.h"
#include "rc_launch.h"
#include "rc_native_plan.h"

using namespace rc;


inline thread_local std::string g_err;
inline int fail(int code, const std::string &msg) { g_err = msg; return code; }

#define HIP_TRY(expr)                                                                         \
  do {                                                                                        \
    hipError_t e_ = (expr);                                                                   \
    if (e_ != hipSuccess) return fail(RC_ERR_DEVICE, std::string(#expr) + ": " + hipGetErrorString(e_)); \
  } while (0)
#define RC_TRY(expr) do { int r_ = (expr); if (r_ != RC_OK) return r_; } while (0)


inline bool trace_on() { static const bool on = std::getenv("RC_TRACE") != nullptr; return on; }
inline double trace_now_us() { return std::chrono::duration<double, std::micro>(std::chrono::steady_clock::now().time_since_epoch()).count(); }
inline void trace(const char *what, const void *obj) {
  if (!trace_on()) return;
  std::fprintf(stderr, "[rc %14.1f us] %-14s %p\n", trace_now_us(), what, obj);
}
template <typename F> auto timed_call(const char *what, size_t bytes, F f) -> decltype(f()) {
  if (!trace_on()) return f();
  const double t0 = trace_now_us();
  auto r = f();
  const double dt = trace_now_us() - t0;
  if (dt > 500.0) std::fprintf(stderr, "[rc %14.1f us] slow call     %s: %.3f ms (%zu bytes)\n", trace_now_us(), what, dt * 1e-3, bytes);
  return r;
}

struct Event {
  hipEvent_t e = nullptr;
  ~Event() { if (e) (void)hipEventDestroy(e); }
  hipError_t record(hipStream_t st) {
    if (!e) { hipError_t r = hipEventCreate(&e); if (r != hipSuccess) return r; }
    return hipEventRecord(e, st);
  }
  operator hipEvent_t() const { return e; }
};

struct Retired {
  std::mutex m;
  std::vector<std::pair<void *, bool>> list;
  size_t bytes = 0;
  std::atomic<bool> ctxGone{false};
  void add(void *p, bool host, size_t n) { std::lock_guard<std::mutex> lk(m); list.emplace_back(p, host); bytes += n; }
  void drain() {
    std::vector<std::pair<void *, bool>> take;
    { std::lock_guard<std::mutex> lk(m); take.swap(list); bytes = 0; }
    for (auto &e : take) { if (e.second) (void)timed_call("retired hipHostFree", 0, [&] { return hipHostFree(e.first); }); else (void)timed_call("retired hipFree", 0, [&] { return hipFree(e.first); }); }
  }
  bool empty() { std::lock_guard<std::mutex> lk(m); return list.empty(); }
  size_t held() { std::lock_guard<std::mutex> lk(m); return bytes; }
};
inline Retired g_retired;

template <typename Alloc> hipError_t alloc_with_retry(Retired *ret, Alloc alloc) {
  hipError_t r = alloc();
  if (r == hipSuccess || (ret->empty() && g_retired.empty())) return r;
  (void)hipGetLastError();
  (void)timed_call("alloc retry hipDeviceSynchronize", 0, [&] { return hipDeviceSynchronize(); });
  ret->drain();
  g_retired.drain();
  return alloc();
}

struct BufPool;
struct PoolRegistry {
  std::mutex m;
  std::vector<BufPool *> pools;
  void add(BufPool *p) { std::lock_guard<std::mutex> lk(m); pools.push_back(p); }
  void remove(BufPool *p) { std::lock_guard<std::mutex> lk(m); pools.erase(std::remove(pools.begin(), pools.end(), p), pools.end()); }
  inline void drain_device(int device);
};
inline PoolRegistry g_pools;

struct BufPool {
  struct Slot { void *p; size_t cap; };
  std::mutex m;
  std::vector<Slot> dev, host;
  size_t devBytes = 0, hostBytes = 0, devCap = static_cast<size_t>(1) << 30, hostCap = static_cast<size_t>(1) << 30;
  bool closed = false;
  int device = -1;
  BufPool() { g_pools.add(this); }
  void *take(bool pinned, size_t want, size_t *got) {
    std::lock_guard<std::mutex> lk(m);
    std::vector<Slot> &v = pinned ? host : dev;
    int best = -1;
    for (size_t i = 0; i < v.size(); i++)
      if (v[i].cap >= want && v[i].cap / 4 <= want && (best < 0 || v[i].cap < v[static_cast<size_t>(best)].cap)) best = static_cast<int>(i);
    if (best < 0) return nullptr;
    Slot s = v[static_cast<size_t>(best)];
    v.erase(v.begin() + best);
    (pinned ? hostBytes : devBytes) -= s.cap;
    *got = s.cap;
    return s.p;
  }
  bool give(bool pinned, void *p, size_t cap) {
    std::lock_guard<std::mutex> lk(m);
    std::vector<Slot> &v = pinned ? host : dev;
    size_t &bytes = pinned ? hostBytes : devBytes;
    if (closed || v.size() >= 256 || bytes + cap > (pinned ? hostCap : devCap)) return false;
    v.push_back(Slot{p, cap});
    bytes += cap;
    return true;
  }
  void drain(bool close) {
    std::vector<Slot> d, h;
    { std::lock_guard<std::mutex> lk(m); d.swap(dev); h.swap(host); devBytes = hostBytes = 0; closed = closed || close; }
    for (auto &s : d) (void)timed_call("pool hipFree", s.cap, [&] { return hipFree(s.p); });
    for (auto &s : h) (void)timed_call("pool hipHostFree", s.cap, [&] { return hipHostFree(s.p); });
  }
  ~BufPool() { g_pools.remove(this); drain(true); }
};
inline void PoolRegistry::drain_device(int device) {
  std::lock_guard<std::mutex> lk(m);
  for (BufPool *p : pools) if (p->device == device) p->drain(false);
}

struct DevBuf {
  void *p = nullptr;
  size_t cap = 0;
  Retired *retired = &g_retired;
  BufPool *pool = nullptr;
  ~DevBuf() { release(); }
  void release() { if (p && !(pool && pool->give(false, p, cap))) (void)timed_call("hipFree", cap, [&] { return hipFree(p); }); p = nullptr; cap = 0; }
  hipError_t ensure(size_t bytes) {
    if (bytes <= cap && p) return hipSuccess;
    if (p) retired->add(p, false, cap);
    p = nullptr; cap = 0;
    const size_t want = std::max<size_t>(bytes + bytes / 8, 256);
    if (pool && (p = pool->take(false, want, &cap))) return hipSuccess;
    hipError_t r = alloc_with_retry(retired, [&] { return timed_call("hipMalloc", want, [&] { return hipMalloc(&p, want); }); });
    if (r != hipSuccess && pool) { pool->drain(false); r = hipMalloc(&p, want); }
    if (r != hipSuccess && pool) { g_pools.drain_device(pool->device); r = hipMalloc(&p, want); }
    if (r == hipSuccess) cap = want; else p = nullptr;
    return r;
  }
  template <typename T> T *as() const { return static_cast<T *>(p); }
};
struct PinBuf {
  void *p = nullptr;
  size_t cap = 0;
  Retired *retired = &g_retired;
  BufPool *pool = nullptr;
  ~PinBuf() { release(); }
  void release() { if (p && !(pool && pool->give(true, p, cap))) (void)timed_call("hipHostFree", cap, [&] { return hipHostFree(p); }); p = nullptr; cap = 0; }
  hipError_t ensure(size_t bytes) {
    if (bytes <= cap && p) return hipSuccess;
    if (p) retired->add(p, true, cap);
    p = nullptr; cap = 0;
    const size_t want = std::max<size_t>(bytes + bytes / 8, 4096);
    if (pool && (p = pool->take(true, want, &cap))) return hipSuccess;
    hipError_t r = alloc_with_retry(retired, [&] { return timed_call("hipHostMalloc", want, [&] { return hipHostMalloc(&p, want, hipHostMallocDefault); }); });
    if (r != hipSuccess && pool) { pool->drain(false); r = hipHostMalloc(&p, want, hipHostMallocDefault); }
    if (r == hipSuccess) cap = want; else p = nullptr;
    return r;
  }
  template <typename T> T *as() const { return static_cast<T *>(p); }
};

inline int effective_cpus() {
  int n = static_cast<int>(std::thread::hardware_concurrency());
  cpu_set_t set;
  if (sched_getaffinity(0, sizeof set, &set) == 0) n = std::min(n, CPU_COUNT(&set));
  if (FILE *f = std::fopen("/sys/fs/cgroup/cpu.max", "r")) {
    char q[64]; long long period = 0;
    if (std::fscanf(f, "%63s %lld", q, &period) == 2 && std::strcmp(q, "max") != 0 && period > 0) {
      const long long quota = std::atoll(q);
      if (quota > 0) n = std::min<long long>(n, std::max<long long>(1, (quota + period - 1) / period));
    }
    std::fclose(f);
  }
  return std::max(1, n);
}

class Pool {
  std::vector<std::thread> th_;
  std::mutex m_;
  std::condition_variable cv_, done_;
  const std::function<void(int)> *job_ = nullptr;
  std::atomic<int> next_{0};
  int total_ = 0, busy_ = 0;
  unsigned long gen_ = 0;
  bool stop_ = false;
  void drain() {
    for (;;) {
      const int i = next_.fetch_add(1);
      if (i >= total_) break;
      (*job_)(i);
    }
  }
  void worker() {
    unsigned long seen = 0;
    for (;;) {
      {
        std::unique_lock<std::mutex> lk(m_);
        cv_.wait(lk, [&] { return stop_ || gen_ != seen; });
        if (stop_) return;
        seen = gen_;
      }
      drain();
      {
        std::lock_guard<std::mutex> lk(m_);
        if (--busy_ == 0) done_.notify_all();
      }
    }
  }

 public:
  explicit Pool(int nthreads) { for (int t = 1; t < nthreads; t++) th_.emplace_back([this] { worker(); }); }
  ~Pool() {
    { std::lock_guard<std::mutex> lk(m_); stop_ = true; }
    cv_.notify_all();
    for (auto &t : th_) t.join();
  }
  int size() const { return static_cast<int>(th_.size()) + 1; }
  void run(int n, const std::function<void(int)> &fn) {
    if (n <= 0) return;
    if (th_.empty() || n < 4) { for (int i = 0; i < n; i++) fn(i); return; }
    {
      std::lock_guard<std::mutex> lk(m_);
      job_ = &fn; total_ = n; next_.store(0); busy_ = static_cast<int>(th_.size()); gen_++;
    }
    cv_.notify_all();
    drain();
    std::unique_lock<std::mutex> lk(m_);
    done_.wait(lk, [&] { return busy_ == 0; });
    job_ = nullptr;
  }
};

template <typename F> void parallel_for(int n, unsigned threads, F &&fn) {
  std::atomic<int> next{0};
  const auto work = [&] { for (int i; (i = next.fetch_add(1)) < n;) fn(i); };
  std::vector<std::thread> th;
  for (unsigned t = 1; t < threads && t < static_cast<unsigned>(std::max(n, 0)); t++) th.emplace_back(work);
  work();
  for (auto &x : th) x.join();
}

inline size_t al256(size_t x) { return (x + 255) & ~static_cast<size_t>(255); }

constexpr size_t kBtMaxBytes = static_cast<size_t>(256) << 20;
constexpr size_t kSegNullMaxBytes = static_cast<size_t>(256) << 20;
constexpr size_t kDecoyMaxBytes = static_cast<size_t>(256) << 20;
constexpr size_t kShuffleNullMaxBytes = static_cast<size_t>(2) << 30;
constexpr size_t kSegShuffleMaxBytes = static_cast<size_t>(256) << 20;


struct TableSet;

struct rc_ctx {
  int device = 0;
  int numCU = 0;
  size_t totalMem = 0;
  size_t togetherWords = static_cast<size_t>(2) << 30;
  DevBuf treeJobs, treeIn, treeWork, treeRes;
  PinBuf treeInPin, treeResPin;
  std::mutex treeMutex;
  int gridCapPerCU = 0;
  double splitFactor = 0.5;
  long long fatStreamMinItems = 16384;
  int tailSharing = 1;
  int nativeWavesPerCU = 8;
  size_t genericScratchWords = static_cast<size_t>(1) << 30;
  static constexpr int kComputeStreams = 3;
  hipStream_t compute[kComputeStreams] = {nullptr, nullptr, nullptr};
  static constexpr int computeStreams = 2;
  hipStream_t native = nullptr;
  hipStream_t copy = nullptr;
  hipStream_t aux = nullptr;
  hipStream_t tree2 = nullptr;
  Event treeFork, treeJoin;
  hipStream_t tree = nullptr;
  int prioLow = 0, prioHigh = 0;
  int classPrio = 0;
  int expMode = 0;
  std::mutex streamMutex;
  std::vector<hipStream_t> classStreams;
  int classStreamCount = 3;
  unsigned seq = 0;
  std::mutex setMutex;
  std::vector<std::unique_ptr<TableSet>> sets;
  uint32_t *d_U = nullptr;
  size_t U_cap = 0;
  uint32_t U_seed = 0;
  int U_Spad = 0, U_D = 0;
  bool U_valid = false;
  Event U_ready;
  float tieThr = 0.0f;
  std::map<std::tuple<NullKind, int, size_t>, int> occ;
  size_t ldsPerCU = 160 * 1024;
  int dualRows = 1;
  int rowSplit = 1;
  int highOccupancy = 1;
  size_t ldsMaxBytes = 13312;
  size_t ldsMaxBytesOneRow = 10752;
  bool stageManyRows = false;
  int debugSkip = 0;
  DevBuf d_cellStats;
  int serialNative = 0;
  ClassRule rule = kDefaultClassRule;
  int stopRounds = 6;
  long long stopTwoRoundsMinItems = 0;
  int hostThreads = 0;
  std::unique_ptr<Pool> pool;
  std::atomic<int> inflight{0};
  std::shared_ptr<Retired> retired = std::make_shared<Retired>();
  std::shared_ptr<BufPool> bufPool = std::make_shared<BufPool>();
  size_t retiredCapBytes = 0;
};

inline void adopt_bufs(rc_ctx *c, std::initializer_list<DevBuf *> bufs) {
  for (DevBuf *d : bufs) { d->retired = c->retired.get(); d->pool = c->bufPool.get(); }
}

inline hipStream_t ctx_stream(rc_ctx *c, int which) {
  hipStream_t *slot = which < rc_ctx::kComputeStreams ? &c->compute[which] : which == 3 ? &c->native : which == 4 ? &c->copy : which == 5 ? &c->aux : which == 6 ? &c->tree : &c->tree2;
  std::lock_guard<std::mutex> lk(c->streamMutex);
  if (!*slot) {
    (void)hipSetDevice(c->device);
    if (hipStreamCreateWithPriority(slot, hipStreamNonBlocking, which < rc_ctx::kComputeStreams ? c->prioLow : c->prioHigh) != hipSuccess) *slot = nullptr;
  }
  return *slot;
}
inline hipStream_t stream_native(rc_ctx *c) { return ctx_stream(c, 3); }
inline hipStream_t stream_copy(rc_ctx *c) { return ctx_stream(c, 4); }
inline hipStream_t stream_aux(rc_ctx *c) { return ctx_stream(c, 5); }
inline hipStream_t stream_tree(rc_ctx *c) { return ctx_stream(c, 6); }
inline hipStream_t stream_tree2(rc_ctx *c) { return ctx_stream(c, 7); }
#define RC_STREAM_TRY(var, expr)                                                               \
  hipStream_t var = (expr);                                                                    \
  if (!var) return fail(RC_ERR_DEVICE, "hipStreamCreateWithPriority failed")

struct TablePtrs {
  const uint8_t *pair; const int *pep; const int *blosum; const CodeInfo *info;
  const int *prepOff; const uint16_t *prepAb;
  bool standard;
};
struct TableSet {
  char code[64];
  int blosum;
  CodeTables ct;
  PairTable pt;
  DevBuf d;
  TablePtrs ptrs{};
  TableSet(const char *c, int which) : blosum(which), ct(which, c) { std::memcpy(code, c, 64); }
};

struct rc_stream;
struct rc_stream;

struct rc_batch {
  std::shared_ptr<Retired> retiredKeep;
  std::shared_ptr<BufPool> poolKeep;
  rc_ctx *ctx = nullptr;
  int device = 0;
  rc_params par{};
  const TableSet *tables = nullptr;
  int n = 0;
  enum State { EMPTY, READY, RUNNING, DONE } state = EMPTY;
  std::vector<BlockMeta> meta;
  std::vector<DevBlock> db;
  std::map<int, std::string> errs;
  std::vector<int> okBlocks;
  std::map<int, std::vector<int>> classes;
  int classOff[kClassSlots] = {0};
  int maxL = 0, maxDraws = 0, hssCap = 8;
  bool allExact = false;
  PinBuf hblob;
  size_t hostCap = 0, hostUsed = 0, devCap = 0;
  size_t oDblocks = 0, oOk = 0, oClass = 0, oPrefix = 0;
  int nModels = 0;
  DevBuf dblob, dmaxima, dhss, dhssCount, dhssPacked, dhssOffsets, dfit, dflags, dexact, dcounters, dscratch, dnativeScratch, dnativeTile, dnativeAll, dsteal, dsbuf;
  size_t sbufNeed = 0;
  float *maxPtr = nullptr;
  bool maximaExternal = false;
  PinBuf hstage, hpacked;
  Event evUp, evPrep0, evPrep, evStart, evMt0, evMt1, evN0, evN1, evS0, evS1, evMid, evFit, evDone;
  std::vector<std::unique_ptr<Event>> classDone;
  bool mtLaunched = false;
  size_t packedAhead = 0;
  std::vector<float> maxima;
  bool maximaFetched = false;
  std::vector<FitOut> fit;
  std::vector<int> hssCount, hssOff;
  std::vector<DevHss> hssRec;
  unsigned long long clamped = 0;
  float t[6] = {0, 0, 0, 0, 0, 0};
  int nl[6] = {0, 0, 0, 0, 0, 0};
  double prepHostMs = 0.0;
  std::string nullKernel;
  double nullKernelCost = 0.0;
  rc_stream *owner = nullptr;
  void adopt(rc_ctx *c) {
    ctx = c; device = c->device; retiredKeep = c->retired; poolKeep = c->bufPool;
    Retired *r = retiredKeep.get();
    for (DevBuf *d : {&dblob, &dmaxima, &dhss, &dhssCount, &dhssPacked, &dhssOffsets, &dfit, &dflags, &dexact, &dcounters, &dscratch, &dnativeScratch,
                      &dnativeTile, &dnativeAll, &dsteal, &dsbuf}) { d->retired = r; d->pool = poolKeep.get(); }
    for (PinBuf *h : {&hblob, &hstage, &hpacked}) { h->retired = r; h->pool = poolKeep.get(); }
  }
};

struct rc_stream {
  rc_ctx *ctx = nullptr;
  rc_params par{};
  const TableSet *tables = nullptr;
  int depth = 2;
  std::deque<rc_batch *> inflight;
  std::vector<rc_batch *> spare;
};

constexpr size_t kCntExact = 0;
constexpr int kMaxRounds = 6;
constexpr size_t kCntWork = kClassSlots + 1;
constexpr size_t kCntClamp = kCntWork + static_cast<size_t>(kMaxRounds) * 3 * kClassSlots * 8;
constexpr size_t kCntTotal = kCntClamp + 2;
static_assert((kCntClamp % 2) == 0, "clamp counter alignment");

struct RunEnv {
  rc_batch *b;
  rc_ctx *c;
  hipStream_t cs;
  int n, sampleN, groups, Spad, slots;
  TablePtrs tp;
  const uint8_t *blob;
  const DevBlock *dblocks;
  const int *okList, *classList;
  bool streaming;
  bool nativeFirst;
  int nativeMode;
  bool fat;
  bool two_rows(int NK) const { return c->dualRows && NK <= kDualRowsMaxNK && (NK == 2 || fat); }
};

void want_hw_queues();
int table_set(rc_ctx *c, const rc_params &par, const TableSet **out);
int batch_prepare(rc_batch *b, const rc_block *blocks, int32_t n_blocks, const rc_params *par, const TableSet *set = nullptr);
int batch_upload(rc_batch *b);
int batch_run_async(rc_batch *b, bool streaming = false);
int batch_wait(rc_batch *b);
void trace_device(rc_batch *b);
extern bool g_no_stream_cache;
int ensure_mt_stream(rc_ctx *c, rc_batch *b, hipStream_t st, uint32_t seed, int Spad, int D);
size_t native_grid(const rc_ctx *c, size_t items, int smax, int mode = 0);
template <typename MemberOf> NativePlan native_plan_on(const rc_ctx *c, size_t n, MemberOf memberOf, int mode) {
  return native_plan(n, memberOf, [&](size_t items, int smax) { return native_grid(c, items, smax, mode); }, c->totalMem);
}
inline int native_query_mode(const rc_ctx *c) { return c->inflight.load() > 0 ? 0 : 1; }
bool fat_class(const rc_batch *b, const rc_ctx *c, int NK, int maxL);
int launch_native_block(const RunEnv &R);
struct NativeBufs { float *tile, *scratch, *all; };
struct NativeTrack { float *out; const long long *off; };
int launch_native_plan(const NativePlan &pl, const NativeArgs &base, const int *list, const NativeBufs &buf, hipStream_t st, const NativeTrack *track = nullptr);
int occupancy(rc_ctx *c, NullKind kind, int n, size_t lds);
int launch_sim_side(rc_ctx *c, const NullArgs &sim, long long items, int maxN, int maxNodes, size_t cntWords, hipStream_t st);
size_t steal_slots(const rc_ctx *c);
size_t steal_words(const rc_ctx *c);
size_t null_round_need(const RunEnv &R, int gLo, int gHi, size_t *sbufFloats);
int launch_null_groups(const RunEnv &R, int gLo, int gHi, int phase, uint32_t extraSkip);
```

rnacode_amd/csrc/rc_schedule.cpp:

```cpp
#include "rc_runtime.h"


size_t native_grid(const rc_ctx *c, size_t items, int smax, int mode) {
  const size_t perGroup = static_cast<size_t>(kWave) * std::max(1, smax) * sizeof(float);
  const size_t byMemory = std::max<size_t>(1, (static_cast<size_t>(2) << 30) / perGroup);
  const size_t perCU = mode == 1 ? 32 : static_cast<size_t>(c->nativeWavesPerCU);
  return std::max<size_t>(1, std::min(std::min(items, perCU * c->numCU), byMemory));
}

bool fat_class(const rc_batch *b, const rc_ctx *c, int NK, int maxL) {
  if (!c->dualRows || NK < 3 || NK > kDualRowsMaxNK || b->allExact) return false;
  const size_t lds = static_cast<size_t>(maxL / 3) * ((NK + 4) / 5) * kWave * sizeof(uint32_t);
  return lds <= c->ldsMaxBytes;
}

int launch_native_block(const RunEnv &R) {
  rc_batch *b = R.b; rc_ctx *c = R.c;
  hipStream_t st = R.nativeFirst ? R.cs : stream_native(c);
  if (!st) return fail(RC_ERR_DEVICE, "hipStreamCreate failed");
  if (!R.nativeFirst) HIP_TRY(hipStreamWaitEvent(st, b->evStart, 0));
  HIP_TRY(b->evN0.record(st));
  NativeArgs na{};
  na.blob = b->dblob.as<uint8_t>(); na.dblocks = R.dblocks; na.blocks = R.okList; na.pair = R.tp.pair;
  na.hss = b->dhss.as<DevHss>(); na.hssCount = b->dhssCount.as<int>(); na.hssCap = b->hssCap; na.tieThr = c->tieThr;
  na.flags = b->dflags.as<uint32_t>();
  HIP_TRY(hipMemsetAsync(b->dhssCount.p, 0, static_cast<size_t>(R.n) * 6 * sizeof(int), st));
  launch_native_sigma(na, static_cast<int>(b->okBlocks.size()), st); b->nl[3]++;
  std::vector<NativeMember> mem;
  mem.reserve(b->okBlocks.size());
  for (const auto &kv : b->classes) {
    const bool generic = kv.first == kGenericClass;
    for (int bi : kv.second) {
      const BlockMeta &m = b->meta[bi];
      mem.push_back(NativeMember{m.NK, m.L, generic || m.N > kTemplRows, generic ? kv.first : kv.first * kMaxRows + m.NK});
    }
  }
  const NativePlan pl = native_plan(mem.size(), [&](size_t i) { return mem[i]; },
                                    [&](size_t items, int smax) { return native_grid(c, items, smax, R.nativeMode); }, c->totalMem);
  HIP_TRY(b->dnativeTile.ensure(std::max<size_t>(pl.tileFloats, 4) * sizeof(float)));
  if (pl.scratchFloats) HIP_TRY(b->dnativeScratch.ensure(pl.scratchFloats * sizeof(float)));
  if (pl.allFloats) HIP_TRY(b->dnativeAll.ensure(std::max<size_t>(pl.allFloats, 4) * sizeof(float)));
  const int launches = launch_native_plan(pl, na, R.classList, NativeBufs{b->dnativeTile.as<float>(), b->dnativeScratch.as<float>(), b->dnativeAll.as<float>()}, st);
  if (launches < 0) return launches;
  b->nl[3] += launches;
  HIP_TRY(hipMemsetAsync(b->dhssOffsets.as<int>() + R.slots, 0, sizeof(int), st));
  launch_hss_pack(b->dhss.as<DevHss>(), b->dhssCount.as<int>(), b->hssCap, R.slots, b->dhssPacked.as<DevHss>(), b->dhssOffsets.as<int>(),
                  b->dhssOffsets.as<int>() + R.slots, st);
  HIP_TRY(b->evN1.record(st));
  return RC_OK;
}

int launch_native_plan(const NativePlan &pl, const NativeArgs &base, const int *list, const NativeBufs &buf, hipStream_t st, const NativeTrack *track) {
  int launches = 0;
  for (const NativeGroup &g : pl.groups) {
    if (g.NK) continue;
    NativeArgs na = base;
    const size_t stride = native_wide_stride(g.maxNK, g.smax);
    for (size_t lo = 0; lo < g.count; lo += kNativeWideChunk, launches++) {
      na.blocks = list + g.at + lo;
      const int blocks = static_cast<int>(native_wide_chunk(g.count, lo));
      if (track) launch_native_track_generic(na, blocks, buf.scratch, stride, track->out, track->off + g.at + lo, st);
      else launch_native_dp_generic(na, blocks, buf.scratch, stride, st);
    }
  }
  for (const NativeGroup &g : pl.groups) {
    if (!g.NK) continue;
    NativeArgs na = base;
    na.blocks = list + g.at; na.nItems = static_cast<int>(g.count) * 6;
    na.tile = buf.tile; na.tileStride = static_cast<size_t>(kWave) * g.smax;
    if (g.keepAll && !track) { na.sAll = buf.all; na.sAllSites = g.smax; }
    if (!(track ? launch_native_track(g.NK, na, static_cast<int>(g.grid), track->out, track->off + g.at, st) : launch_native_dp(g.NK, na, static_cast<int>(g.grid), st)))
      return fail(RC_ERR_UNSUPPORTED, "no native DP kernel for this number of rows");
    launches++;
    if (na.sAll) { launch_native_scan(na, st); launches++; }
  }
  return launches;
}

int launch_sim_side(rc_ctx *c, const NullArgs &sim, long long items, int maxN, int maxNodes, size_t cntWords, hipStream_t st) {
  const size_t lds = null_generic_lds_bytes(maxN, maxNodes);
  const int occ = std::max(1, occupancy(c, NullKind::GenericSim, 0, lds));
  HIP_TRY(hipMemsetAsync(sim.workCounter, 0, cntWords * sizeof(uint32_t), st));
  launch_generic(NullKind::GenericSim, sim, static_cast<int>(std::min<long long>(items, static_cast<long long>(c->numCU) * occ)), lds, sim.codesAll, st);
  HIP_TRY(hipGetLastError());
  return RC_OK;
}

size_t steal_slots(const rc_ctx *c) { return static_cast<size_t>(c->numCU) * 32; }
size_t steal_words(const rc_ctx *c) { return 16 + 4 * steal_slots(c); }

int occupancy(rc_ctx *c, NullKind kind, int n, size_t lds) {
  const auto key = std::make_tuple(kind, n, lds);
  auto it = c->occ.find(key);
  if (it != c->occ.end()) return it->second;
  return c->occ[key] = kind >= NullKind::TiledDp ? tiled_dp_occupancy(n, kind, lds) : kind >= NullKind::GenericSim ? generic_occupancy(kind, lds)
                                                   : null_occupancy(n, kind, lds);
}

struct ClassPlan {
  int cls = 0;
  NullKind kind = NullKind::Exact;
  int n = 0, grid = 0; size_t lds = 0;
  int gridExact = 0;
  NullKind simKind = NullKind::GenericSim; int simGrid = 0; size_t simLds = 0;
  int comboSplit = 0, rowParts = 0, simParts = 0, cacheSites = 0;
  size_t stride = 0, sbufStride = 0, sbufFloats = 0;
  size_t codesBytes = 0, stateBytes = 0; int roundBlocks = 0;
  double itemCost = 0.0; size_t need = 0;
  bool tailShare = false;
  size_t slot = 0, scratchOff = 0, sbufOff = 0;
};

struct RoundIn { const RunEnv &R; int groups; bool together, splitAll; };

static bool few_items(const RoundIn &in, double items, int occ) { return in.together ? in.splitAll : items <= in.R.c->splitFactor * in.R.c->numCU * occ; }

struct Extent { int maxL = 0, maxNK = 0, maxN = 0, maxNodes = 0; };
static ClassPlan class_base(const rc_batch *b, int cls, const std::vector<int> &mem, Extent *x) {
  for (int bi : mem) {
    x->maxL = std::max(x->maxL, b->meta[bi].L); x->maxNK = std::max(x->maxNK, b->meta[bi].NK);
    x->maxN = std::max(x->maxN, b->meta[bi].N); x->maxNodes = std::max(x->maxNodes, b->db[bi].nnodes);
  }
  ClassPlan p;
  p.cls = cls; p.itemCost = static_cast<double>(x->maxNK) * x->maxL * x->maxL;
  return p;
}

struct PlainPlan { int occ; size_t lds; NullKind kind; };
static PlainPlan plain_plan(rc_ctx *c, int NK, int maxNodes, NullKind want) {
  for (NullKind k : {want, NullKind::L2}) {
    const size_t minLds = k == NullKind::L2 ? static_cast<size_t>(kPhaseALds) : al256(static_cast<size_t>(maxNodes) * 64 + 64 * 64);
    const int occ = occupancy(c, k, NK, minLds);
    if (occ <= 0) continue;
    size_t budget = (c->ldsPerCU / static_cast<size_t>(occ)) & ~static_cast<size_t>(255);
    while (budget > minLds && occupancy(c, k, NK, budget) < occ) budget -= 256;
    return PlainPlan{occ, std::max(budget, minLds), k};
  }
  return PlainPlan{0, static_cast<size_t>(kPhaseALds), NullKind::L2};
}

static ClassPlan plan_rows(const RoundIn &in, int NK, const std::vector<int> &mem) {
  const RunEnv &R = in.R; rc_batch *b = R.b; rc_ctx *c = R.c;
  Extent x;
  ClassPlan p = class_base(b, NK, mem, &x);
  p.n = NK; p.rowParts = 1; p.simParts = 1;
  p.stride = static_cast<size_t>(2) * (x.maxL + 1) * code_pos_words(NK);
  const bool exactOnly = b->allExact || NK >= kFastRows;
  if (c->rowSplit && !exactOnly && !R.streaming) {
    const long long slots = static_cast<long long>(c->numCU) * 16;
    const long long partsAll = static_cast<long long>(in.together ? b->okBlocks.size() : mem.size()) * in.groups * 6;
    if ((!in.together || in.splitAll) && partsAll * 2 <= slots) {
      const size_t smax = static_cast<size_t>(x.maxL) / 3;
      p.rowParts = static_cast<int>(std::min<long long>(8, slots / partsAll));
      p.sbufStride = smax * (smax + 1) / 2 * kWave;
      p.sbufFloats = p.sbufStride * 6 * mem.size() * static_cast<size_t>(in.groups);
      if (p.sbufFloats * sizeof(float) > (static_cast<size_t>(256) << 20) || smax < 45) { p.rowParts = 1; p.sbufStride = p.sbufFloats = 0; }
    }
  }
  const bool twoRows = R.two_rows(NK);
  const size_t staged = static_cast<size_t>(x.maxL / 3) * ((NK + 4) / 5) * kWave * sizeof(uint32_t);
  const bool dualL2 = p.rowParts == 1 && !exactOnly && NK >= 3 && twoRows && staged <= c->ldsMaxBytes &&
                      c->ldsPerCU / std::max<size_t>(staged, kPhaseALds) <= 12;
  const bool stage = !exactOnly && !dualL2 && p.rowParts == 1 && (NK <= kDualRowsMaxNK || c->stageManyRows) &&
                     staged <= (twoRows ? c->ldsMaxBytes : std::min(c->ldsMaxBytes, c->ldsMaxBytesOneRow));
  int occ = 0;
  if (exactOnly) {
    p.kind = NullKind::Exact;
    occ = NK < kFastRows ? occupancy(c, NullKind::L2, NK, kPhaseALds) : occupancy(c, NullKind::Exact, NK, 0);
  } else if (stage) {
    p.lds = std::max<size_t>(staged, kPhaseALds);
    p.kind = twoRows && p.lds <= 48 * 1024 ? NullKind::StagedTwoRow : NullKind::Staged;
    occ = occupancy(c, NullKind::Staged, NK, p.lds);
  }
  if (!exactOnly && occ <= 0) {
    const NullKind want = dualL2 ? NullKind::L2TwoRow : (c->highOccupancy == 2 || (c->highOccupancy == 1 && b->classes.size() == 1)) ? NullKind::L2Occ : NullKind::L2;
    const PlainPlan pp = plain_plan(c, NK, x.maxNodes, want);
    occ = pp.occ; p.lds = pp.lds;
    p.kind = p.rowParts > 1 ? NullKind::RowSplit : pp.kind;
    const size_t tables = static_cast<size_t>(NK) * kWave * sizeof(float);
    if (pp.occ > 0 && pp.lds > tables) p.cacheSites = static_cast<int>((pp.lds - tables) / (static_cast<size_t>(code_pos_words(NK)) * sizeof(uint32_t)));
  }
  occ = std::max(1, occ);
  if (c->gridCapPerCU > 0) occ = std::min(occ, c->gridCapPerCU);
  int items = static_cast<int>(mem.size()) * in.groups;
  p.comboSplit = (p.rowParts > 1 || few_items(in, static_cast<double>(items), occ)) ? 1 : 0;
  if (p.rowParts > 1) {
    const long long its = static_cast<long long>(mem.size()) * in.groups;
    p.simParts = static_cast<int>(std::max<long long>(1, std::min<long long>({16, x.maxL / 16, static_cast<long long>(c->numCU) * 4 / std::max<long long>(its, 1)})));
    p.simGrid = static_cast<int>(std::min<long long>(its * p.simParts, static_cast<long long>(c->numCU) * occ));
  }
  if (p.comboSplit) items *= 6 * p.rowParts;
  p.grid = std::min(items, c->numCU * occ);
  p.grid = static_cast<int>(std::max<size_t>(1, std::min<size_t>(p.grid, (static_cast<size_t>(1) << 30) / std::max<size_t>(p.stride, 1))));
  p.gridExact = exactOnly ? 0 : std::min(p.grid, c->numCU);
  p.need = p.rowParts > 1 ? p.stride * std::max<size_t>(mem.size() * static_cast<size_t>(in.groups), static_cast<size_t>(p.gridExact))
                          : p.stride * std::max(p.grid, p.gridExact);
  p.tailShare = !exactOnly && c->tailSharing && !p.comboSplit && static_cast<size_t>(p.grid) <= steal_slots(c);
  return p;
}

static void size_two_launches(const RoundIn &in, ClassPlan &p, size_t blocks, int occD, int occS) {
  const rc_ctx *c = in.R.c;
  occD = std::max(1, occD); occS = std::max(1, occS);
  const long long slotsD = static_cast<long long>(c->numCU) * occD;
  const long long items = static_cast<long long>(blocks) * in.groups;
  const long long budgetBlocks = std::max<long long>(1, static_cast<long long>(c->genericScratchWords * sizeof(uint32_t) / p.codesBytes) / in.groups);
  const long long nBlocks = static_cast<long long>(blocks);
  const long long rounds = (nBlocks + budgetBlocks - 1) / budgetBlocks;
  p.roundBlocks = static_cast<int>((nBlocks + rounds - 1) / rounds);
  const long long roundItems = static_cast<long long>(p.roundBlocks) * in.groups;
  p.comboSplit = (few_items(in, static_cast<double>(items), occD) || roundItems < 8 * slotsD) ? 1 : 0;
  p.grid = static_cast<int>(std::min<long long>(roundItems * (p.comboSplit ? 6 : 1), slotsD));
  p.simGrid = static_cast<int>(std::min<long long>(roundItems, static_cast<long long>(c->numCU) * occS));
  p.need = (static_cast<size_t>(roundItems) * p.codesBytes + static_cast<size_t>(p.grid) * p.stateBytes + 3) / 4 + 64;
}

static ClassPlan plan_generic(const RoundIn &in, const std::vector<int> &mem) {
  rc_ctx *c = in.R.c;
  Extent x;
  ClassPlan p = class_base(in.R.b, kGenericClass, mem, &x);
  p.kind = NullKind::GenericDp; p.simKind = NullKind::GenericSim;
  p.lds = p.simLds = null_generic_lds_bytes(x.maxN, x.maxNodes);
  p.codesBytes = null_generic_codes_bytes(x.maxN, x.maxL, x.maxNodes);
  p.stateBytes = null_generic_state_bytes(x.maxN, x.maxL, x.maxNodes);
  size_two_launches(in, p, mem.size(), occupancy(c, NullKind::GenericDp, 0, p.lds), occupancy(c, NullKind::GenericSim, 0, p.simLds));
  return p;
}

static ClassPlan plan_tiled(const RoundIn &in, int cls, const std::vector<int> &mem) {
  rc_batch *b = in.R.b; rc_ctx *c = in.R.c;
  Extent x;
  ClassPlan p = class_base(b, cls, mem, &x);
  p.n = kTiledMinKT + (cls - kTiledClass0);
  p.kind = b->allExact ? NullKind::TiledDpNan : NullKind::TiledDp; p.simKind = NullKind::TiledSim;
  p.lds = 0;
  p.simLds = null_generic_lds_bytes(x.maxN, x.maxNodes);
  for (int bi : mem) p.codesBytes = std::max(p.codesBytes, null_tiled_codes_bytes(b->meta[bi].NK, p.n, b->meta[bi].L));
  p.stateBytes = null_tiled_state_bytes(x.maxL);
  size_two_launches(in, p, mem.size(), occupancy(c, NullKind::TiledDp, p.n, 0), occupancy(c, NullKind::GenericSim, 0, p.simLds));
  p.gridExact = p.kind == NullKind::TiledDp ? std::min(p.grid, c->numCU) : 0;
  return p;
}

struct RoundPlan { std::vector<ClassPlan> classes; bool concurrent = false; size_t need = 0, sbufFloats = 0; };

static RoundPlan plan_classes(const RunEnv &R, int groups, bool together) {
  const rc_batch *b = R.b; const rc_ctx *c = R.c;
  const RoundIn in{R, groups, together, static_cast<double>(b->okBlocks.size()) * groups <= c->splitFactor * c->numCU * 16};
  RoundPlan rp{{}, together, 0, 0};
  size_t needSum = 0, needMax = 0;
  for (const auto &kv : b->classes) {
    rp.classes.push_back(kv.first < kGenericClass ? plan_rows(in, kv.first, kv.second)
                         : kv.first == kGenericClass ? plan_generic(in, kv.second) : plan_tiled(in, kv.first, kv.second));
    needSum += rp.classes.back().need; needMax = std::max(needMax, rp.classes.back().need);
    rp.sbufFloats += rp.classes.back().sbufFloats;
  }
  std::stable_sort(rp.classes.begin(), rp.classes.end(), [](const ClassPlan &x, const ClassPlan &y) { return x.itemCost > y.itemCost; });
  rp.need = together ? needSum : needMax;
  return rp;
}

static RoundPlan plan_round(const RunEnv &R, int gLo, int gHi) {
  rc_batch *b = R.b; rc_ctx *c = R.c;
  trace("null: plan", b);
  const bool together = b->classes.size() > 1 && !c->serialNative;
  RoundPlan rp = plan_classes(R, gHi - gLo, together);
  if (together && rp.need > c->togetherWords) rp = plan_classes(R, gHi - gLo, false);
  const size_t streams = std::min(rp.classes.size(), static_cast<size_t>(c->classStreamCount));
  size_t scratchOff = 0, sbufOff = 0;
  for (size_t pi = 0; pi < rp.classes.size(); pi++) {
    ClassPlan &p = rp.classes[pi];
    if (rp.concurrent) { p.slot = pi % streams; p.scratchOff = scratchOff; scratchOff += p.need; }
    p.sbufOff = sbufOff; sbufOff += p.sbufFloats;
  }
  return rp;
}

size_t null_round_need(const RunEnv &R, int gLo, int gHi, size_t *sbufFloats) { const RoundPlan rp = plan_round(R, gLo, gHi); *sbufFloats = rp.sbufFloats; return rp.need; }

static void trace_launch(const RunEnv &R, const ClassPlan &p, int phase, int gLo, int gHi) {
  if (!trace_on()) return;
  std::fprintf(stderr, "[rc %14.1f us] null: launch   %p class=%d kernel=%s grid=%d exactGrid=%d simGrid=%d lds=%zu slot=%zu comboSplit=%d rowParts=%d simParts=%d cacheSites=%d scratch=%zu round=%d groups=%d..%d\n",
               trace_now_us(), static_cast<const void *>(R.b), p.cls, null_kernel_name(p.kind, p.n).c_str(), p.grid, p.gridExact, p.simGrid, p.lds, p.slot,
               p.comboSplit, p.rowParts, p.simParts, p.cacheSites, p.need, phase, gLo, gHi);
}

static int launch_rows(const RunEnv &R, const ClassPlan &p, NullArgs a, unsigned int *work, size_t stealIdx, uint32_t extraSkip, hipStream_t st) {
  rc_batch *b = R.b; rc_ctx *c = R.c;
  if (p.kind == NullKind::Exact) {
    a.skipMask = extraSkip; a.workCounter = work + kClassSlots * 8 + p.cls * 8;
    if (!launch_null(p.n, p.kind, a, p.grid, p.lds, st)) return fail(RC_ERR_UNSUPPORTED, "no null kernel for this number of rows");
    b->nl[2]++;
    return RC_OK;
  }
  a.skipMask = kFlagExact | extraSkip; a.workCounter = work + p.cls * 8; a.cacheSites = p.cacheSites;
  if (p.rowParts > 1) {
    if (!b->dsbuf.p || (p.sbufOff + p.sbufFloats) * sizeof(float) > b->dsbuf.cap) return fail(RC_ERR_ARG, "internal: the row buffer was not sized for this round");
    a.rowParts = p.rowParts; a.sbuf = b->dsbuf.as<float>() + p.sbufOff; a.sbufStride = p.sbufStride;
    a.simParts = p.simParts; a.simGrid = p.simGrid; a.simCounter = work + 2 * kClassSlots * 8 + p.cls * 8;
  }
  if (p.tailShare && b->dsteal.p) {
    if ((stealIdx + 1) * steal_words(c) * sizeof(uint32_t) <= b->dsteal.cap) a.steal = b->dsteal.as<unsigned int>() + stealIdx * steal_words(c);
    a.stealWait = R.streaming ? 0 : 1;
  }
  if (!launch_null(p.n, p.kind, a, p.grid, p.lds, st)) return fail(RC_ERR_UNSUPPORTED, "no null kernel for this number of rows");
  b->nl[2]++;
  if (p.rowParts > 1) launch_null_rowscan(a, a.nClassBlocks * (a.gHi - a.gLo), st);
  NullArgs e = a;
  e.classBlocks = b->dexact.as<int>() + b->classOff[p.cls];
  e.nBlocksPtr = b->dcounters.as<int>() + kCntExact + p.cls;
  e.nClassBlocks = 0; e.skipMask = extraSkip; e.comboSplit = 0; e.steal = nullptr;
  e.cacheSites = 0; e.rowParts = 0; e.sbuf = nullptr; e.simParts = 0; e.simGrid = 0; e.simCounter = nullptr;
  e.workCounter = work + kClassSlots * 8 + p.cls * 8;
  if (!launch_null(p.n, NullKind::Exact, e, p.gridExact, 0, st)) return fail(RC_ERR_UNSUPPORTED, "no null kernel for this number of rows");
  return RC_OK;
}

static int launch_two(const RunEnv &R, const ClassPlan &p, NullArgs a, unsigned int *work, uint32_t extraSkip, hipStream_t st) {
  rc_batch *b = R.b;
  const bool tiled = p.cls > kGenericClass;
  const size_t members = static_cast<size_t>(a.nClassBlocks);
  a.skipMask = extraSkip; a.tiledKT = p.n; a.workCounter = work + p.cls * 8;
  uint8_t *base = reinterpret_cast<uint8_t *>(a.scratch);
  const size_t codesAllBytes = (static_cast<size_t>(p.roundBlocks) * (a.gHi - a.gLo) * p.codesBytes + 255) & ~static_cast<size_t>(255);
  a.codesAll = base; a.codesStride = p.codesBytes;
  a.scratchStride = p.stateBytes;
  unsigned int *simWork = work + kClassSlots * 8 + p.cls * 8;
  unsigned int *nanWork = work + 2 * kClassSlots * 8 + p.cls * 8;
  for (size_t at = 0; at < members; at += static_cast<size_t>(p.roundBlocks)) {
    if (at) {
      HIP_TRY(hipMemsetAsync(a.workCounter, 0, 8 * sizeof(unsigned int), st));
      HIP_TRY(hipMemsetAsync(simWork, 0, 8 * sizeof(unsigned int), st));
      if (tiled) HIP_TRY(hipMemsetAsync(nanWork, 0, 8 * sizeof(unsigned int), st));
    }
    NullArgs r = a;
    r.classBlocks = a.classBlocks + at;
    r.nClassBlocks = static_cast<int>(std::min<size_t>(static_cast<size_t>(p.roundBlocks), members - at));
    NullArgs sim = r; sim.workCounter = simWork;
    launch_generic(p.simKind, sim, p.simGrid, p.simLds, nullptr, st);
    if (!tiled) {
      launch_generic(p.kind, r, p.grid, p.lds, base + codesAllBytes, st);
      b->nl[2] += 2;
      continue;
    }
    r.skipMask = extraSkip | (p.kind == NullKind::TiledDp ? kFlagNan : 0u);
    if (!launch_tiled_dp(p.n, p.kind, r, p.grid, p.lds, base + codesAllBytes, st)) return fail(RC_ERR_UNSUPPORTED, "no tiled kernel for this tile size");
    b->nl[2] += 2;
    if (p.kind == NullKind::TiledDp) {
      NullArgs e = r;
      e.skipMask = extraSkip; e.onlyMask = kFlagNan; e.workCounter = nanWork;
      e.nBlocksPtr = b->dcounters.as<int>() + kCntExact + p.cls;
      (void)launch_tiled_dp(p.n, NullKind::TiledDpNan, e, p.gridExact, p.lds, base + codesAllBytes, st);
      b->nl[2]++;
    }
  }
  return RC_OK;
}

int launch_null_groups(const RunEnv &R, int gLo, int gHi, int phase, uint32_t extraSkip) {
  rc_batch *b = R.b; rc_ctx *c = R.c;
  const RoundPlan rp = plan_round(R, gLo, gHi);
  if (rp.need * sizeof(uint32_t) > b->dscratch.cap) return fail(RC_ERR_ARG, "internal: staging scratch was not sized for this round");
  Event &fork = phase ? b->evMid : b->evS0;
  if (rp.concurrent) while (b->classDone.size() < static_cast<size_t>(kMaxRounds) * rp.classes.size()) b->classDone.emplace_back(new Event());
  trace("null: planned", b);
  std::vector<Event *> joins;
  for (size_t pi = 0; pi < rp.classes.size(); pi++) {
    const ClassPlan &p = rp.classes[pi];
    hipStream_t st = R.cs;
    if (rp.concurrent) {
      if (p.slot > 0) {
        while (c->classStreams.size() < p.slot) {
          hipStream_t ns = nullptr;
          HIP_TRY(hipStreamCreateWithPriority(&ns, hipStreamNonBlocking, c->classPrio));
          c->classStreams.push_back(ns);
        }
        st = c->classStreams[p.slot - 1];
      }
      if (pi == 0) trace("null: streams", b);
      if (st != R.cs) HIP_TRY(hipStreamWaitEvent(st, fork, 0));
    }
    trace_launch(R, p, phase, gLo, gHi);
    const size_t members = b->classes[p.cls].size();
    const double cost = p.itemCost * static_cast<double>(members) * (gHi - gLo);
    if (cost > b->nullKernelCost) { b->nullKernelCost = cost; b->nullKernel = null_kernel_name(p.kind, p.n); }
    NullArgs a{};
    a.blob = R.blob; a.dblocks = R.dblocks; a.classBlocks = R.classList + b->classOff[p.cls]; a.nClassBlocks = static_cast<int>(members);
    a.flags = b->dflags.as<uint32_t>();
    a.gLo = gLo; a.gHi = gHi; a.sampleN = R.sampleN; a.Spad = R.Spad;
    a.U = c->d_U; a.pair = R.tp.pair; a.scratch = b->dscratch.as<uint32_t>() + p.scratchOff; a.scratchStride = p.stride;
    a.maxima = b->maxPtr; a.clampCount = reinterpret_cast<unsigned long long *>(b->dcounters.as<uint32_t>() + kCntClamp);
    a.tieThr = c->tieThr; a.debugSkip = c->debugSkip; a.comboSplit = p.comboSplit;
    a.cellStats = c->d_cellStats.as<unsigned long long>();
    unsigned int *work = b->dcounters.as<unsigned int>() + kCntWork + static_cast<size_t>(phase) * 3 * kClassSlots * 8;
    if (p.cls < kGenericClass) RC_TRY(launch_rows(R, p, a, work, static_cast<size_t>(phase) * b->classes.size() + pi, extraSkip, st));
    else RC_TRY(launch_two(R, p, a, work, extraSkip, st));
    if (pi == 0) trace("null: first class", b);
    if (rp.concurrent && st != R.cs) {
      Event &done = *b->classDone[static_cast<size_t>(phase) * rp.classes.size() + pi];
      HIP_TRY(done.record(st));
      joins.push_back(&done);
    }
  }
  for (Event *done : joins) HIP_TRY(hipStreamWaitEvent(R.cs, *done, 0));
  return RC_OK;
}
```

Before: 30.17 billion alignment-columns*samples/s.

## Merge memsets into one reset kernel, fold result copy into fit, pack triangular scores

Several separate memsets (counters, maxima, hss counts, offsets, steal buffer) are replaced by one multi-part reset kernel. The mapped-memory result copy is folded into extra workgroups of the EVD fit kernel, which also writes fit results straight to host memory, and the packed-record copy is trimmed to the used count. The kept per-item score matrix now uses triangular storage to halve memory and allow keep-all in more cases. The host-side result vectors become pointers into pinned buffers, which avoids copies but ties result lifetime to the staging buffers.

```diff
diff --git a/rnacode_amd/csrc/rc_batch.cpp b/rnacode_amd/csrc/rc_batch.cpp
--- a/rnacode_amd/csrc/rc_batch.cpp
+++ b/rnacode_amd/csrc/rc_batch.cpp
@@ -247,11 +247,19 @@
                  reinterpret_cast<const int *>(blob + b->oClass), streaming, nativeFirst, nativeMode, fat};
   HIP_TRY(hipStreamWaitEvent(cs, b->evPrep, 0));
   HIP_TRY(b->evStart.record(cs));
+  const int slots = R.slots;
+  const size_t szFit = sizeof(FitOut) * n, szCnt = sizeof(int) * static_cast<size_t>(slots), szOff = sizeof(int) * (static_cast<size_t>(slots) + 1);
+  const size_t oFit = 0, oCnt = al256(oFit + szFit), oOff = al256(oCnt + szCnt), oClamp = al256(oOff + szOff);
+  HIP_TRY(b->hstage.ensure(oClamp + 16));
+  bool mapped = false;
   if (!b->okBlocks.empty()) {
     RC_TRY(ensure_mt_stream(c, b, cs, b->par.seed_base, Spad, b->maxDraws));
-    uint32_t *cnt = b->dcounters.as<uint32_t>();
-    HIP_TRY(hipMemsetAsync(cnt + kCntWork, 0, (kCntTotal - kCntWork) * sizeof(uint32_t), cs));
-    HIP_TRY(hipMemsetD32Async(reinterpret_cast<hipDeviceptr_t>(b->maxPtr), 0xBF800000u, static_cast<size_t>(n) * sampleN, cs));
+    RunResetArgs rs{};
+    auto preset = [&](int x, void *dst, size_t words, uint32_t value) { rs.dst[x] = static_cast<uint32_t *>(dst); rs.words[x] = words; rs.value[x] = value; };
+    preset(0, b->dcounters.as<uint32_t>() + kCntWork, kCntTotal - kCntWork, 0u);
+    preset(1, b->maxPtr, static_cast<size_t>(n) * sampleN, 0xBF800000u);
+    preset(3, b->dhssCount.p, static_cast<size_t>(n) * 6, 0u);
+    preset(4, b->dhssOffsets.as<int>() + R.slots, 1, 0u);
     FitArgs fa{};
     fa.dblocks = R.dblocks; fa.blocks = R.okList; fa.maxima = b->maxPtr; fa.hss = b->dhss.as<DevHss>();
     fa.hssCount = b->dhssCount.as<int>(); fa.hssCap = b->hssCap; fa.out = b->dfit.as<FitOut>(); fa.flags = b->dflags.as<uint32_t>();
@@ -260,24 +268,28 @@
     int g1 = groups;
     if (b->par.stopEarly && fa.stopCutoff >= 0 && fa.stopCutoff < sampleN && static_cast<long long>(b->okBlocks.size()) * groups >= c->stopTwoRoundsMinItems)
       g1 = std::min(groups, (fa.stopCutoff + 1 + kWave + kWave - 1) / kWave);
+    std::vector<std::pair<int, int>> rounds;
+    for (int lo = 0, hi = g1; lo < groups;) {
+      if (static_cast<int>(rounds.size()) == c->stopRounds - 1) hi = groups;
+      rounds.emplace_back(lo, hi);
+      lo = hi; hi = std::min(groups, hi * 2);
+    }
+    if (c->tailSharing) {
+      const size_t bytes = rounds.size() * b->classes.size() * steal_words(c) * sizeof(uint32_t);
+      HIP_TRY(b->dsteal.ensure(bytes));
+      preset(2, b->dsteal.p, bytes / sizeof(uint32_t), 0u);
+    }
+    launch_run_reset(rs, cs);
     {
       size_t most = 0;
-      int r = 0;
       b->sbufNeed = 0;
-      for (int lo = 0, hi = g1; lo < groups; r++) {
-        if (r == c->stopRounds - 1) hi = groups;
+      for (const auto &lh : rounds) {
         size_t sbuf = 0;
-        most = std::max(most, null_round_need(R, lo, hi, &sbuf));
+        most = std::max(most, null_round_need(R, lh.first, lh.second, &sbuf));
         b->sbufNeed = std::max(b->sbufNeed, sbuf);
-        lo = hi; hi = std::min(groups, hi * 2);
       }
       HIP_TRY(b->dscratch.ensure(most * sizeof(uint32_t)));
       if (b->sbufNeed) HIP_TRY(b->dsbuf.ensure(b->sbufNeed * sizeof(float)));
-      if (c->tailSharing) {
-        const size_t bytes = static_cast<size_t>(r) * b->classes.size() * steal_words(c) * sizeof(uint32_t);
-        HIP_TRY(b->dsteal.ensure(bytes));
-        HIP_TRY(hipMemsetAsync(b->dsteal.p, 0, bytes, cs));
-      }
     }
     bool nativeQueued = true;
     if (R.nativeFirst) RC_TRY(launch_native_block(R));
@@ -300,41 +312,36 @@
     HIP_TRY(b->evS1.record(cs));
     if (!nativeQueued) RC_TRY(launch_native_block(R));
     if (!R.nativeFirst) HIP_TRY(hipStreamWaitEvent(cs, b->evN1, 0));
+    b->packedAhead = std::min(static_cast<size_t>(slots) * b->hssCap, static_cast<size_t>(n) * 16);
+    HIP_TRY(b->hpacked.ensure(sizeof(DevHss) * std::max<size_t>(b->packedAhead, 1)));
+    void *dStage = nullptr, *dPacked = nullptr;
+    static_assert(sizeof(FitOut) % 4 == 0 && sizeof(DevHss) % 4 == 0, "results travel as 32-bit words");
+    mapped = c->mappedResults && hipHostGetDevicePointer(&dStage, b->hstage.p, 0) == hipSuccess && hipHostGetDevicePointer(&dPacked, b->hpacked.p, 0) == hipSuccess;
+    if (mapped) {
+      uint8_t *ds = static_cast<uint8_t *>(dStage);
+      ResultsOutArgs &ro = fa.send;
+      size_t most = 0;
+      auto part = [&](int x, void *dst, const void *src, size_t bytes) {
+        ro.dst[x] = static_cast<uint32_t *>(dst); ro.src[x] = static_cast<const uint32_t *>(src); ro.words[x] = bytes / 4; most = std::max(most, bytes / 4);
+      };
+      part(1, ds + oCnt, b->dhssCount.p, szCnt);
+      part(2, ds + oOff, b->dhssOffsets.p, szOff);
+      part(3, ds + oClamp, b->dcounters.as<uint32_t>() + kCntClamp, sizeof(unsigned long long));
+      part(4, dPacked, b->dhssPacked.p, sizeof(DevHss) * b->packedAhead);
+      ro.lastUsed = b->dhssOffsets.as<int>() + slots; ro.lastUnitWords = static_cast<int>(sizeof(DevHss) / 4);
+      fa.outHost = reinterpret_cast<FitOut *>(ds + oFit);
+      fa.sendGroups = static_cast<int>(std::min<size_t>(256, (most + 255) / 256));
+    }
     launch_evd_fit(fa, static_cast<int>(b->okBlocks.size()), c->inflight.load() == 0 && (!streaming || b->okBlocks.size() <= 64), cs); b->nl[4]++;
   }
   HIP_TRY(b->evFit.record(cs));
-  {
-    const int slots = R.slots;
-    const size_t szFit = sizeof(FitOut) * n, szCnt = sizeof(int) * static_cast<size_t>(slots), szOff = sizeof(int) * (static_cast<size_t>(slots) + 1);
-    const size_t oFit = 0, oCnt = al256(oFit + szFit), oOff = al256(oCnt + szCnt), oClamp = al256(oOff + szOff), total = oClamp + 16;
-    HIP_TRY(b->hstage.ensure(total));
-    if (!b->okBlocks.empty()) {
-      uint8_t *hs = b->hstage.as<uint8_t>();
-      b->packedAhead = std::min(static_cast<size_t>(slots) * b->hssCap, static_cast<size_t>(n) * 16);
-      HIP_TRY(b->hpacked.ensure(sizeof(DevHss) * std::max<size_t>(b->packedAhead, 1)));
-      void *dStage = nullptr, *dPacked = nullptr;
-      static_assert(sizeof(FitOut) % 4 == 0 && sizeof(DevHss) % 4 == 0, "results travel as 32-bit words");
-      if (hipHostGetDevicePointer(&dStage, b->hstage.p, 0) == hipSuccess &&
-          hipHostGetDevicePointer(&dPacked, b->hpacked.p, 0) == hipSuccess) {
-        uint8_t *ds = static_cast<uint8_t *>(dStage);
-        ResultsOutArgs ro{};
-        auto part = [&](int x, void *dst, const void *src, size_t bytes) {
-          ro.dst[x] = static_cast<uint32_t *>(dst); ro.src[x] = static_cast<const uint32_t *>(src); ro.words[x] = bytes / 4;
-        };
-        part(0, ds + oFit, b->dfit.p, szFit);
-        part(1, ds + oCnt, b->dhssCount.p, szCnt);
-        part(2, ds + oOff, b->dhssOffsets.p, szOff);
-        part(3, ds + oClamp, b->dcounters.as<uint32_t>() + kCntClamp, sizeof(unsigned long long));
-        part(4, dPacked, b->dhssPacked.p, sizeof(DevHss) * b->packedAhead);
-        launch_results_out(ro, cs);
-      } else {
-        HIP_TRY(hipMemcpyAsync(hs + oFit, b->dfit.p, szFit, hipMemcpyDeviceToHost, cs));
-        HIP_TRY(hipMemcpyAsync(hs + oCnt, b->dhssCount.p, szCnt, hipMemcpyDeviceToHost, cs));
-        HIP_TRY(hipMemcpyAsync(hs + oOff, b->dhssOffsets.p, szOff, hipMemcpyDeviceToHost, cs));
-        HIP_TRY(hipMemcpyAsync(hs + oClamp, b->dcounters.as<uint32_t>() + kCntClamp, sizeof(unsigned long long), hipMemcpyDeviceToHost, cs));
-        HIP_TRY(hipMemcpyAsync(b->hpacked.p, b->dhssPacked.p, sizeof(DevHss) * b->packedAhead, hipMemcpyDeviceToHost, cs));
-      }
-    }
+  if (!b->okBlocks.empty() && !mapped) {
+    uint8_t *hs = b->hstage.as<uint8_t>();
+    HIP_TRY(hipMemcpyAsync(hs + oFit, b->dfit.p, szFit, hipMemcpyDeviceToHost, cs));
+    HIP_TRY(hipMemcpyAsync(hs + oCnt, b->dhssCount.p, szCnt, hipMemcpyDeviceToHost, cs));
+    HIP_TRY(hipMemcpyAsync(hs + oOff, b->dhssOffsets.p, szOff, hipMemcpyDeviceToHost, cs));
+    HIP_TRY(hipMemcpyAsync(hs + oClamp, b->dcounters.as<uint32_t>() + kCntClamp, sizeof(unsigned long long), hipMemcpyDeviceToHost, cs));
+    HIP_TRY(hipMemcpyAsync(b->hpacked.p, b->dhssPacked.p, sizeof(DevHss) * b->packedAhead, hipMemcpyDeviceToHost, cs));
   }
   HIP_TRY(b->evDone.record(cs));
   HIP_TRY(hipGetLastError());
@@ -355,10 +362,11 @@
   HIP_TRY(hipGetLastError());
   const int n = b->n, slots = n * 6;
   b->fit.assign(n, FitOut{0, 0, -1, 0});
-  b->hssCount.assign(static_cast<size_t>(slots), 0);
-  b->hssOff.assign(static_cast<size_t>(slots) + 1, 0);
-  b->hssRec.clear();
-  if (!b->okBlocks.empty()) {
+  b->hssRec = nullptr;
+  if (b->okBlocks.empty()) {
+    b->hssNone.assign(static_cast<size_t>(slots) + 1, 0);
+    b->hssCount = b->hssOff = b->hssNone.data();
+  } else {
     float ms = 0;
     if (b->mtLaunched) { HIP_TRY(hipEventElapsedTime(&ms, b->evMt0, b->evMt1)); b->t[1] = ms; b->nl[1] = 1; }
     HIP_TRY(hipEventElapsedTime(&ms, b->evN0, b->evN1)); b->t[3] = ms;
@@ -371,19 +379,17 @@
     const uint8_t *hs = b->hstage.as<uint8_t>();
     const FitOut *f = reinterpret_cast<const FitOut *>(hs + oFit);
     for (int bi : b->okBlocks) b->fit[bi] = f[bi];
-    std::memcpy(b->hssCount.data(), hs + oCnt, szCnt);
-    std::memcpy(b->hssOff.data(), hs + oOff, szOff);
+    b->hssCount = reinterpret_cast<const int *>(hs + oCnt);
+    b->hssOff = reinterpret_cast<const int *>(hs + oOff);
     std::memcpy(&b->clamped, hs + oClamp, sizeof(unsigned long long));
     const size_t nrec = static_cast<size_t>(std::max(b->hssOff[slots], 0));
+    b->hssRec = b->hpacked.as<DevHss>();
     if (nrec > b->packedAhead) {
-      PinBuf more;
-      HIP_TRY(more.ensure(sizeof(DevHss) * nrec));
+      HIP_TRY(b->hmore.ensure(sizeof(DevHss) * nrec));
       RC_STREAM_TRY(aux, stream_aux(c));
-      HIP_TRY(hipMemcpyAsync(more.p, b->dhssPacked.p, sizeof(DevHss) * nrec, hipMemcpyDeviceToHost, aux));
+      HIP_TRY(hipMemcpyAsync(b->hmore.p, b->dhssPacked.p, sizeof(DevHss) * nrec, hipMemcpyDeviceToHost, aux));
       HIP_TRY(hipStreamSynchronize(aux));
-      b->hssRec.assign(more.as<DevHss>(), more.as<DevHss>() + nrec);
-    } else if (nrec) {
-      b->hssRec.assign(b->hpacked.as<DevHss>(), b->hpacked.as<DevHss>() + nrec);
+      b->hssRec = b->hmore.as<DevHss>();
     }
   }
   b->state = rc_batch::DONE;
diff --git a/rnacode_amd/csrc/rc_context.cpp b/rnacode_amd/csrc/rc_context.cpp
--- a/rnacode_amd/csrc/rc_context.cpp
+++ b/rnacode_amd/csrc/rc_context.cpp
@@ -151,6 +151,7 @@
   if (const char *e = std::getenv("RC_SPLIT_FACTOR")) c->splitFactor = std::max(0.0, std::atof(e));
   if (const char *e = std::getenv("RC_NATIVE_WAVES_PER_CU")) c->nativeWavesPerCU = std::max(1, std::min(32, std::atoi(e)));
   if (const char *e = std::getenv("RC_TAIL_SHARING")) c->tailSharing = std::atoi(e) != 0;
+  if (const char *e = std::getenv("RC_MAPPED_RESULTS")) c->mappedResults = std::atoi(e) != 0;
   if (const char *e = std::getenv("RC_ROW_SPLIT")) c->rowSplit = std::atoi(e) != 0;
   if (const char *e = std::getenv("RC_DUAL_ROWS")) c->dualRows = std::atoi(e) != 0;
   if (const char *e = std::getenv("RC_HIGH_OCCUPANCY")) c->highOccupancy = std::max(0, std::min(2, std::atoi(e)));
diff --git a/rnacode_amd/csrc/rc_device.h b/rnacode_amd/csrc/rc_device.h
--- a/rnacode_amd/csrc/rc_device.h
+++ b/rnacode_amd/csrc/rc_device.h
@@ -1,4 +1,5 @@
 #pragma once
+#include <cstddef>
 #include <cstdint>
 
 namespace rc {
@@ -90,6 +91,9 @@
 constexpr int code_tail_bytes(int NK) { return NK - 5 * (code_words(NK) - 1) == 1 ? 1 : NK - 5 * (code_words(NK) - 1) == 2 ? 2 : 4; }
 constexpr int code_pos_words(int NK) { return (code_words(NK) - 1) * kWave + code_tail_bytes(NK) * (kWave / 4); }
 
+constexpr size_t native_tri_floats(int smax) { return static_cast<size_t>(smax) * (static_cast<size_t>(smax) + 1) / 2; }
+constexpr size_t native_tri_at(int a, int j, int smax) { return static_cast<size_t>(a) * smax - (static_cast<size_t>(a) * (a + 1) / 2 - a) + (j - a); }
+
 constexpr int kDualRowsMaxNK = 5;
 constexpr uint32_t kFlagExact = 1u;
 constexpr uint32_t kFlagNan = 4u;
diff --git a/rnacode_amd/csrc/rc_kernels.hip b/rnacode_amd/csrc/rc_kernels.hip
--- a/rnacode_amd/csrc/rc_kernels.hip
+++ b/rnacode_amd/csrc/rc_kernels.hip
@@ -476,12 +476,12 @@
   const int combo = item % 6, s = combo / 3, f = combo % 3;
   const DevBlock *__restrict__ db = A.dblocks + bi;
   const int sites = (db->L - f) / 3;
-  const float *__restrict__ S = A.sAll + static_cast<size_t>(item) * A.sAllSites * A.sAllSites;
+  const float *__restrict__ S = A.sAll + static_cast<size_t>(item) * native_tri_floats(A.sAllSites);
   DevHss *out = A.hss + (static_cast<size_t>(bi) * 6 + combo) * A.hssCap;
   int n = 0;
   ScanState st{0.0f, -1, -1};
   for (int a = 0; a < sites; a++) {
-    const float *__restrict__ row = S + static_cast<size_t>(a) * A.sAllSites;
+    const float *__restrict__ row = S + native_tri_at(a, a, A.sAllSites) - a;
     for (int j0 = a; j0 < sites; j0 += 8) {
       float v8[8];
 #pragma unroll
@@ -758,11 +758,27 @@
   if (threadIdx.x == 0) A.flags[bi] = (A.flags[bi] & ~kFlagStopped) | (better > A.stopCutoff ? kFlagStopped : 0u);
 }
 
+__device__ __forceinline__ void results_copy(const ResultsOutArgs &a, size_t t, size_t threads) {
+#pragma unroll
+  for (int x = 0; x < ResultsOutArgs::kParts; x++) {
+    size_t words = a.words[x];
+    if (x == ResultsOutArgs::kParts - 1 && a.lastUsed) {
+      const size_t used = static_cast<size_t>(*a.lastUsed > 0 ? *a.lastUsed : 0) * a.lastUnitWords;
+      words = used < words ? used : words;
+    }
+    for (size_t i = t; i < words; i += threads) a.dst[x][i] = a.src[x][i];
+  }
+}
+
 template <int THREADS>
 __global__ __launch_bounds__(THREADS) void k_evd_fit(FitArgs A) {
   __builtin_amdgcn_s_setprio(3);
   __shared__ double sh[THREADS > kWave ? (THREADS / kWave) * 4 : 1];
-  const int bi = A.blocks[blockIdx.x];
+  if (static_cast<int>(blockIdx.x) < A.sendGroups) {
+    results_copy(A.send, static_cast<size_t>(blockIdx.x) * THREADS + threadIdx.x, static_cast<size_t>(A.sendGroups) * THREADS);
+    return;
+  }
+  const int bi = A.blocks[blockIdx.x - A.sendGroups];
   const DevBlock *db = A.dblocks + bi;
   const float *x = A.maxima + static_cast<size_t>(db->out_index) * A.sampleN;
   const float maxNative = best_native(A, bi);
@@ -781,7 +797,10 @@
     double mu, lambda;
     if (evd_fit_block<THREADS, float>(A.expMode, x, A.sampleN, sh, &mu, &lambda) == 1) { o.rc = 1; o.mu = mu; o.lambda = lambda; }
   }
-  if (threadIdx.x == 0) A.out[db->out_index] = o;
+  if (threadIdx.x == 0) {
+    A.out[db->out_index] = o;
+    if (A.outHost) A.outHost[db->out_index] = o;
+  }
 }
 
 __global__ __launch_bounds__(256) void k_evd_fit_f64(const double *x, int n, FitOut *out, int mode) {
@@ -899,21 +918,19 @@
   hipLaunchKernelGGL(k_hss_pack, dim3((slots + 255) / 256), dim3(256), 0, stream, hss, count, cap, slots, packed, offsets, total);
 }
 
-
-__global__ __launch_bounds__(64) void k_results_out(ResultsOutArgs a) {
-  __builtin_amdgcn_s_setprio(3);
+__global__ __launch_bounds__(256) void k_run_reset(RunResetArgs a) {
   const size_t t = static_cast<size_t>(blockIdx.x) * blockDim.x + threadIdx.x, step = static_cast<size_t>(gridDim.x) * blockDim.x;
 #pragma unroll
-  for (int x = 0; x < ResultsOutArgs::kParts; x++)
-    for (size_t i = t; i < a.words[x]; i += step) a.dst[x][i] = a.src[x][i];
-}
-
-void launch_results_out(const ResultsOutArgs &a, hipStream_t stream) {
+  for (int x = 0; x < RunResetArgs::kParts; x++)
+    for (size_t i = t; i < a.words[x]; i += step) a.dst[x][i] = a.value[x];
+}
+
+void launch_run_reset(const RunResetArgs &a, hipStream_t stream) {
   size_t most = 0;
-  for (int x = 0; x < ResultsOutArgs::kParts; x++) most = std::max(most, a.words[x]);
+  for (int x = 0; x < RunResetArgs::kParts; x++) most = std::max(most, a.words[x]);
   if (!most) return;
-  const int grid = static_cast<int>(std::min<size_t>(256, (most + 255) / 256));
-  hipLaunchKernelGGL(k_results_out, dim3(grid), dim3(64), 0, stream, a);
+  const int grid = static_cast<int>(std::min<size_t>(2048, (most + 1023) / 1024));
+  hipLaunchKernelGGL(k_run_reset, dim3(grid), dim3(256), 0, stream, a);
 }
 
 void launch_sk_row(const uint8_t *blob, const DevBlock *dblocks, const uint32_t *flags, int bi, int s, int b, int iMax, float *out, int stride,
@@ -959,8 +976,8 @@
 }
 
 void launch_evd_fit(const FitArgs &a, int nblocks, bool latency, hipStream_t stream) {
-  if (latency && nblocks <= 2048) hipLaunchKernelGGL(k_evd_fit<256>, dim3(nblocks), dim3(256), 0, stream, a);
-  else hipLaunchKernelGGL(k_evd_fit<64>, dim3(nblocks), dim3(64), 0, stream, a);
+  if (latency && nblocks <= 2048) hipLaunchKernelGGL(k_evd_fit<256>, dim3(nblocks + a.sendGroups), dim3(256), 0, stream, a);
+  else hipLaunchKernelGGL(k_evd_fit<64>, dim3(nblocks + a.sendGroups), dim3(64), 0, stream, a);
 }
 
 void launch_evd_fit_f64(const double *x, int n, FitOut *out, int expMode, hipStream_t stream) {
diff --git a/rnacode_amd/csrc/rc_launch.h b/rnacode_amd/csrc/rc_launch.h
--- a/rnacode_amd/csrc/rc_launch.h
+++ b/rnacode_amd/csrc/rc_launch.h
@@ -96,6 +96,15 @@
   int better;
 };
 
+struct ResultsOutArgs {
+  static constexpr int kParts = 5;
+  uint32_t *dst[kParts];
+  const uint32_t *src[kParts];
+  size_t words[kParts];
+  const int *lastUsed;
+  int lastUnitWords;
+};
+
 struct FitArgs {
   const DevBlock *dblocks;
   const int *blocks;
@@ -110,6 +119,9 @@
   int stopEarly;
   int stopCutoff;
   int expMode;
+  FitOut *outHost;
+  int sendGroups;
+  ResultsOutArgs send;
 };
 
 struct TreeJob {
@@ -212,13 +224,13 @@
 void launch_native_scan(const NativeArgs &a, hipStream_t stream);
 void launch_hss_pack(const DevHss *hss, const int *count, int cap, int slots, DevHss *packed, int *offsets, int *total,
                      hipStream_t stream);
-struct ResultsOutArgs {
+struct RunResetArgs {
   static constexpr int kParts = 5;
   uint32_t *dst[kParts];
-  const uint32_t *src[kParts];
   size_t words[kParts];
-};
-void launch_results_out(const ResultsOutArgs &a, hipStream_t stream);
+  uint32_t value[kParts];
+};
+void launch_run_reset(const RunResetArgs &a, hipStream_t stream);
 void launch_sk_row(const uint8_t *blob, const DevBlock *dblocks, const uint32_t *flags, int bi, int s, int b, int iMax, float *out, int stride,
                    hipStream_t stream);
 struct BtItem {
diff --git a/rnacode_amd/csrc/rc_native_dp.h b/rnacode_amd/csrc/rc_native_dp.h
--- a/rnacode_amd/csrc/rc_native_dp.h
+++ b/rnacode_amd/csrc/rc_native_dp.h
@@ -56,7 +56,7 @@
     const int sites = (L - f) / 3, smax = L / 3;
     float *full = A.fullS ? A.fullS + static_cast<size_t>(combo) * smax * smax : nullptr;
     constexpr bool kOld = NK > 16 && NK <= 32;
-    float *__restrict__ all = (!kOld && A.sAll) ? A.sAll + static_cast<size_t>(item) * A.sAllSites * A.sAllSites : nullptr;
+    float *__restrict__ all = (!kOld && A.sAll) ? A.sAll + static_cast<size_t>(item) * native_tri_floats(A.sAllSites) : nullptr;
 #if RC_NATIVE_TRACK
     float *__restrict__ T = native_track_of(track, trackOff, item / 6, L, s, f);
 #else
@@ -124,7 +124,7 @@
               }
             }
             const float v = fmaxf(sum, Delta) / nkf;
-            if (all) all[static_cast<size_t>(a) * A.sAllSites + j] = v;
+            if (all) all[native_tri_at(a, j, A.sAllSites)] = v;
             else tile[static_cast<size_t>(lane) * sites + j] = v;
             if (full) full[static_cast<size_t>(a) * sites + j] = v;
           }
diff --git a/rnacode_amd/csrc/rc_native_plan.h b/rnacode_amd/csrc/rc_native_plan.h
--- a/rnacode_amd/csrc/rc_native_plan.h
+++ b/rnacode_amd/csrc/rc_native_plan.h
@@ -20,7 +20,7 @@
 constexpr size_t native_wide_chunk(size_t count, size_t at) { return std::min(kNativeWideChunk, count - at); }
 
 constexpr size_t kNativeKeepMinItems = 6 * 64, kNativeKeepMemShare = 16;
-constexpr size_t native_all_floats(size_t count, int smax) { return 6 * count * smax * smax; }
+constexpr size_t native_all_floats(size_t count, int smax) { return 6 * count * native_tri_floats(smax); }
 constexpr bool native_keep_all(int NK, size_t count, int smax, size_t totalMem) {
   return native_all_floats(count, smax) * sizeof(float) <= totalMem / kNativeKeepMemShare && 6 * count >= kNativeKeepMinItems && (NK <= 16 || NK > 32);
 }
diff --git a/rnacode_amd/csrc/rc_runtime.h b/rnacode_amd/csrc/rc_runtime.h
--- a/rnacode_amd/csrc/rc_runtime.h
+++ b/rnacode_amd/csrc/rc_runtime.h
@@ -288,6 +288,7 @@
   int gridCapPerCU = 0;
   double splitFactor = 0.5;
   long long fatStreamMinItems = 16384;
+  int mappedResults = 1;
   int tailSharing = 1;
   int nativeWavesPerCU = 8;
   size_t genericScratchWords = static_cast<size_t>(1) << 30;
@@ -411,8 +412,10 @@
   std::vector<float> maxima;
   bool maximaFetched = false;
   std::vector<FitOut> fit;
-  std::vector<int> hssCount, hssOff;
-  std::vector<DevHss> hssRec;
+  const int *hssCount = nullptr, *hssOff = nullptr;
+  const DevHss *hssRec = nullptr;
+  std::vector<int> hssNone;
+  PinBuf hmore;
   unsigned long long clamped = 0;
   float t[6] = {0, 0, 0, 0, 0, 0};
   int nl[6] = {0, 0, 0, 0, 0, 0};
@@ -425,7 +428,7 @@
     Retired *r = retiredKeep.get();
     for (DevBuf *d : {&dblob, &dmaxima, &dhss, &dhssCount, &dhssPacked, &dhssOffsets, &dfit, &dflags, &dexact, &dcounters, &dscratch, &dnativeScratch,
                       &dnativeTile, &dnativeAll, &dsteal, &dsbuf}) { d->retired = r; d->pool = poolKeep.get(); }
-    for (PinBuf *h : {&hblob, &hstage, &hpacked}) { h->retired = r; h->pool = poolKeep.get(); }
+    for (PinBuf *h : {&hblob, &hstage, &hpacked, &hmore}) { h->retired = r; h->pool = poolKeep.get(); }
   }
 };
 
diff --git a/rnacode_amd/csrc/rc_schedule.cpp b/rnacode_amd/csrc/rc_schedule.cpp
--- a/rnacode_amd/csrc/rc_schedule.cpp
+++ b/rnacode_amd/csrc/rc_schedule.cpp
@@ -18,13 +18,12 @@
   rc_batch *b = R.b; rc_ctx *c = R.c;
   hipStream_t st = R.nativeFirst ? R.cs : stream_native(c);
   if (!st) return fail(RC_ERR_DEVICE, "hipStreamCreate failed");
-  if (!R.nativeFirst) HIP_TRY(hipStreamWaitEvent(st, b->evStart, 0));
+  if (!R.nativeFirst) HIP_TRY(hipStreamWaitEvent(st, b->evS0, 0));
   HIP_TRY(b->evN0.record(st));
   NativeArgs na{};
   na.blob = b->dblob.as<uint8_t>(); na.dblocks = R.dblocks; na.blocks = R.okList; na.pair = R.tp.pair;
   na.hss = b->dhss.as<DevHss>(); na.hssCount = b->dhssCount.as<int>(); na.hssCap = b->hssCap; na.tieThr = c->tieThr;
   na.flags = b->dflags.as<uint32_t>();
-  HIP_TRY(hipMemsetAsync(b->dhssCount.p, 0, static_cast<size_t>(R.n) * 6 * sizeof(int), st));
   launch_native_sigma(na, static_cast<int>(b->okBlocks.size()), st); b->nl[3]++;
   std::vector<NativeMember> mem;
   mem.reserve(b->okBlocks.size());
@@ -43,7 +42,6 @@
   const int launches = launch_native_plan(pl, na, R.classList, NativeBufs{b->dnativeTile.as<float>(), b->dnativeScratch.as<float>(), b->dnativeAll.as<float>()}, st);
   if (launches < 0) return launches;
   b->nl[3] += launches;
-  HIP_TRY(hipMemsetAsync(b->dhssOffsets.as<int>() + R.slots, 0, sizeof(int), st));
   launch_hss_pack(b->dhss.as<DevHss>(), b->dhssCount.as<int>(), b->hssCap, R.slots, b->dhssPacked.as<DevHss>(), b->dhssOffsets.as<int>(),
                   b->dhssOffsets.as<int>() + R.slots, st);
   HIP_TRY(b->evN1.record(st));
```

Result: no change. 30.25 billion alignment-columns*samples/s, median of 6 (+0.3%).
